# traveller59/spconv

Hardware: AMD Instinct MI355X
Metric: active-voxels/sec fwd+bwd, 3x3x3 SubMConv3d C=64, ~100k voxels/scene (higher is better)
Workload: dtype f16; 1 GPU; SubMConv3d 3x3x3 C=64->64 f16, 100000 uniform voxels/scene in 1600x1280x40 (BASELINE configs[1]), 8 distinct scenes per GPU visited round-robin, rulebook reused via indice_key; voxels_per_gpu=100000, launch=hipgraph, steps_per_replay=8, scenes_rotated=8, mask_sort=False, prewarm_steps=0, parallelism=dp1, ranks_seen=1, tree=unknown

## Files before the change

include/spconv_amd.h:

```cpp
#ifndef SPCONV_AMD_H_
#define SPCONV_AMD_H_

#include <stddef.h>
#include <stdint.h>

#ifdef __cplusplus
extern "C" {
#endif

#define SPX_MAX_NDIM 4
#define SPX_UNION_MAX_OPERANDS 8

typedef void *spx_stream_t;

enum spx_dtype { SPX_F32 = 0, SPX_F16 = 1, SPX_BF16 = 2, SPX_I8 = 3, SPX_F64 = 4 };

enum spx_act { SPX_ACT_NONE = 0, SPX_ACT_RELU = 1, SPX_ACT_SIGMOID = 2, SPX_ACT_LEAKY_RELU = 3 };
#define SPX_OUT_CACHED 0x100
#define SPX_TILE_ORDER 0x200

const char *spx_last_error(void);

int spx_version(void);

int spx_set_option(const char *name_h, int value);

long long spx_launch_count(const char *family_h);

int spx_pad_rows(const void *src, void *dst, long long rows, int src_row_bytes, int dst_row_bytes,
                 spx_stream_t stream);

int spx_conv_out_shape(int ndim, const int *in_shape, const int *ksize, const int *stride,
                       const int *padding, const int *dilation, const int *out_padding,
                       int transposed, int *out_shape);


size_t spx_subm_rulebook_ws_bytes(int n, int kv);

int spx_subm_rulebook(const int32_t *indices, int n, int ndim, int batch_size,
                      const int *spatial_shape, const int *ksize, const int *dilation,
                      int32_t *pair_fwd, int32_t *pair_bwd, uint32_t *mask,
                      int32_t *pair_native, int32_t *num_per_loc,
                      void *ws, size_t ws_bytes, spx_stream_t stream);

size_t spx_conv_rulebook_ws_bytes(int n_in, int ndim, const int *ksize, const int *stride,
                                  const int *dilation, int transposed);

int spx_conv_rulebook_count(const int32_t *indices, int n_in, int ndim, int batch_size,
                            const int *in_shape, const int *out_shape, const int *ksize,
                            const int *stride, const int *padding, const int *dilation,
                            int transposed, void *ws, size_t ws_bytes, int *n_out_h,
                            spx_stream_t stream);

int spx_conv_rulebook_fill(const int32_t *indices, int n_in, int ndim, int batch_size,
                           const int *in_shape, const int *out_shape, const int *ksize,
                           const int *stride, const int *padding, const int *dilation,
                           int transposed, int n_out, int32_t *out_indices,
                           int32_t *pair_fwd, int32_t *pair_bwd, uint32_t *mask_fwd,
                           uint32_t *mask_bwd, int32_t *pair_native, int32_t *num_per_loc,
                           void *ws, size_t ws_bytes, spx_stream_t stream);

int spx_conv_rulebook_static(const int32_t *indices, int n_in, int ndim, int batch_size,
                             const int *in_shape, const int *out_shape, const int *ksize,
                             const int *stride, const int *padding, const int *dilation,
                             int transposed, int n_out_cap, int32_t *out_indices,
                             int32_t *pair_fwd, int32_t *pair_bwd, uint32_t *mask_fwd,
                             uint32_t *mask_bwd, int32_t *pair_native, int32_t *num_per_loc,
                             int32_t *n_out_dev, void *ws, size_t ws_bytes, spx_stream_t stream);

size_t spx_rankmap_bytes(int ndim, int batch_size, const int *shape);
int spx_conv_sorted_ok(int ndim, int batch_size, const int *in_shape, const int *out_shape, const int *ksize,
                       const int *stride, const int *padding, const int *dilation, int transposed);
size_t spx_conv_rulebook_sorted_ws_bytes(int n_in, int ndim, int batch_size, const int *out_shape,
                                         const int *ksize);
int spx_conv_rulebook_count_sorted(const int32_t *indices, int n_in, int ndim, int batch_size,
                                   const int *in_shape, const int *out_shape, const int *ksize,
                                   const int *stride, const int *padding, const int *dilation,
                                   void *rankmap, size_t rankmap_bytes, void *ws, size_t ws_bytes,
                                   int *n_out_h, spx_stream_t stream);
int spx_conv_rulebook_fill_sorted(const int32_t *indices, int n_in, int ndim, int batch_size,
                                  const int *in_shape, const int *out_shape, const int *ksize,
                                  const int *stride, const int *padding, const int *dilation, int n_out,
                                  int32_t *out_indices, int32_t *pair_fwd, int32_t *pair_bwd,
                                  uint32_t *mask_fwd, uint32_t *mask_bwd, int32_t *pair_native,
                                  int32_t *num_per_loc, void *rankmap, size_t rankmap_bytes, void *ws,
                                  size_t ws_bytes, spx_stream_t stream);
int spx_conv_rulebook_static_sorted(const int32_t *indices, int n_in, int ndim, int batch_size,
                                    const int *in_shape, const int *out_shape, const int *ksize,
                                    const int *stride, const int *padding, const int *dilation,
                                    int n_out_cap, int32_t *out_indices, int32_t *pair_fwd,
                                    int32_t *pair_bwd, uint32_t *mask_fwd, uint32_t *mask_bwd,
                                    int32_t *pair_native, int32_t *num_per_loc, int32_t *n_out_dev,
                                    void *rankmap, size_t rankmap_bytes, void *ws, size_t ws_bytes,
                                    spx_stream_t stream);
int spx_rankmap_from_sorted(const int32_t *indices, int n, int ndim, int batch_size, const int *spatial_shape,
                            void *rankmap, size_t rankmap_bytes, int32_t *violation, spx_stream_t stream);
size_t spx_key_argsort_ws_bytes(int n);
int spx_key_argsort(const int32_t *indices, int n, int ndim, int batch_size, const int *spatial_shape, int32_t *order,
                    int32_t *indices_sorted, void *rankmap, size_t rankmap_bytes, int32_t *violation, const void *rows,
                    void *rows_sorted, int row_bytes, void *ws, size_t ws_bytes, spx_stream_t stream);
size_t spx_subm_rulebook_ranked_ws_bytes(int n, int kv);
int spx_subm_rulebook_ranked(const int32_t *indices, int n, int ndim, int batch_size,
                             const int *spatial_shape, const int *ksize, const int *dilation,
                             int32_t *pair_fwd, int32_t *pair_bwd, uint32_t *mask,
                             int32_t *pair_native, int32_t *num_per_loc, const void *rankmap,
                             size_t rankmap_bytes, void *ws, size_t ws_bytes, spx_stream_t stream);

size_t spx_mask_argsort_ws_bytes(int n);
int spx_mask_argsort(const uint32_t *mask, int n, int words, int32_t *argsort,
                     void *ws, size_t ws_bytes, spx_stream_t stream);
int spx_mask_argsort_kv(const uint32_t *mask, int n, int kv, int32_t *argsort, void *ws, size_t ws_bytes,
                        spx_stream_t stream);

int spx_native_to_table(const int32_t *pair_native, const int32_t *num_per_loc, int n_in,
                        int n_dst, int kv, int subm, int inverse, int32_t *table,
                        uint32_t *mask, spx_stream_t stream);
size_t spx_table_to_native_ws_bytes(int n, int kv);
int spx_table_to_native(const int32_t *table, int subm, int kv, int n, int32_t *pair_native,
                        int32_t *num_per_loc, void *ws, size_t ws_bytes, spx_stream_t stream);


size_t spx_igemm_acc_bytes(int n_dst, int cout, int kv);

int spx_igemm_fwd(const void *feat, const void *weight, void *out, const int32_t *pair,
                  const uint32_t *mask, const int32_t *argsort, int tile_order, int n_in, int n_out,
                  int C, int K, int kv, int dtype, int identity_k, const void *bias,
                  int act, float act_alpha, void *ws, size_t ws_bytes,
                  spx_stream_t stream);

int spx_igemm_fwd_stats_slots(int n_out);
int spx_igemm_fwd_stats(const void *feat, const void *weight, void *out, const int32_t *pair,
                        const uint32_t *mask, const int32_t *argsort, int tile_order, int n_in, int n_out, int C,
                        int K, int kv, int dtype, int identity_k, const void *bias, int act,
                        float act_alpha, void *ws, size_t ws_bytes, float *stats, int stats_slots,
                        const int32_t *n_live, int *slots_used_h, spx_stream_t stream);

int spx_igemm_fwd_int8(const void *feat, const void *weight, void *out, const int32_t *pair,
                       const uint32_t *mask, const int32_t *argsort, int n_in, int n_out, int C,
                       int K, int kv, int identity_k, const float *scale, const float *bias,
                       const void *add, float add_scale, int out_dtype, int act, float act_alpha,
                       spx_stream_t stream);

int spx_permute_tables(const int32_t *pair, const uint32_t *mask, const int32_t *order, int kv, int n,
                       int words, int32_t *pair_t, uint32_t *mask_t, spx_stream_t stream);

size_t spx_subm_layout_mcap(int n);
#define SPX_ROWS_LAYOUT 2
#define SPX_DENSE_HINT 0x100
#define SPX_ROWS_LAYOUT_ACT 0x400
#define SPX_SPARSE_HINT 0x800
#define SPX_LAYOUT_HEADER 64
size_t spx_subm_layout_bytes(int n, int kv);
size_t spx_subm_layout_ws_bytes(int n);
int spx_subm_layout(const int32_t *pair_fwd, const uint32_t *mask, int n, int kv, int32_t *layout,
                    void *ws, size_t ws_bytes, spx_stream_t stream);

size_t spx_igemm_dgrad_ws_bytes(int C, int K, int kv, int dtype);

int spx_igemm_dgrad(const void *dout, const void *weight, void *din, const int32_t *pair,
                    const uint32_t *mask, const int32_t *argsort, int tile_order, int n_out, int n_in,
                    int C, int K, int kv, int dtype, int subm, void *ws, size_t ws_bytes,
                    spx_stream_t stream);

size_t spx_igemm_wgrad_ws_bytes(int n_in, int C, int K, int kv);
size_t spx_igemm_wgrad_ws_bytes_dtype(int n_in, int C, int K, int kv, int dtype);

size_t spx_wgrad_plan_bytes(int n_in, int kv);
int spx_wgrad_plan(const int32_t *num_per_loc, int n_in, int kv, int subm, int32_t *plan,
                   spx_stream_t stream);

int spx_igemm_wgrad(const void *feat, const void *dout, void *dw, const int32_t *pair_native,
                    const int32_t *num_per_loc, const int32_t *plan, int n_in, int n_out, int C,
                    int K, int kv, int dtype, int subm, void *ws, size_t ws_bytes,
                    spx_stream_t stream);

size_t spx_igemm_bwd_rows_ws_bytes(int n_in, int C, int K, int kv);
int spx_igemm_bwd_rows(const void *feat, const void *dout, const void *weight_t, void *din, void *dw,
                       const int32_t *table, const uint32_t *mask, int n_in, int n_out, int C, int K,
                       int kv, int mirror, int dtype, void *ws, size_t ws_bytes, spx_stream_t stream);

int spx_igemm_bwd(const void *feat, const void *dout, const void *weight, void *din, void *dw,
                  const int32_t *pair, const uint32_t *mask, const int32_t *argsort, int tile_order,
                  const int32_t *pair_native, const int32_t *num_per_loc, const int32_t *plan,
                  int n_in, int n_out, int C, int K, int kv, int dtype, int subm, void *ws,
                  size_t ws_bytes, spx_stream_t stream);

#define SPX_STAGE2_JOB_BYTES 64
int spx_igemm_bwd_deferred(const void *feat, const void *dout, const void *weight, void *din, void *dw,
                           const int32_t *pair, const uint32_t *mask, const int32_t *argsort, int tile_order,
                           const int32_t *pair_native, const int32_t *num_per_loc, const int32_t *plan,
                           int n_in, int n_out, int C, int K, int kv, int dtype, int subm, void *ws,
                           size_t ws_bytes, spx_stream_t stream, void *stage2_job);
int spx_igemm_wgrad_deferred(const void *feat, const void *dout, void *dw, const int32_t *pair_native,
                             const int32_t *num_per_loc, const int32_t *plan, int n_in, int n_out, int C,
                             int K, int kv, int dtype, int subm, void *ws, size_t ws_bytes,
                             spx_stream_t stream, void *stage2_job);
int spx_wgrad_stage2_batch(const void *jobs, int njobs, spx_stream_t stream);
int spx_stage2_job_retarget(void *stage2_job, void *dw);

int spx_bias_act_inplace(void *out, const void *bias, int n, int K, int dtype, int act,
                         float act_alpha, spx_stream_t stream);


int spx_maxpool_fwd(const void *feat, void *out, const int32_t *pair_fwd, const uint32_t *mask,
                    int n_out, int C, int kv, int dtype, int init_zero, spx_stream_t stream);
int spx_maxpool_bwd(const void *feat, const void *out, const void *dout, void *din,
                    const int32_t *pair_bwd, const uint32_t *mask_bwd, int n_in, int C, int kv,
                    int dtype, spx_stream_t stream);
int spx_avgpool_fwd(const void *feat, void *out, int32_t *count_out, const int32_t *pair_fwd,
                    const uint32_t *mask, int n_out, int C, int kv, int dtype,
                    spx_stream_t stream);
int spx_avgpool_bwd(const void *dout, void *din, const int32_t *count, const int32_t *pair_bwd,
                    const uint32_t *mask_bwd, int n_in, int C, int kv, int dtype,
                    spx_stream_t stream);


size_t spx_point2voxel_ws_bytes(int n_points, int max_voxels);
int spx_point2voxel(const float *points, int n, int nfeat, int ndim, const float *vsize,
                    const float *coors_range, const int *grid_size, int max_voxels, int max_points,
                    int empty_mean, int clear_voxels, float *voxels, int32_t *indices,
                    int32_t *num_per_voxel, long long *pc_voxel_id, int *n_voxels_h, void *ws,
                    size_t ws_bytes, spx_stream_t stream);

size_t spx_point2voxel_static_ws_bytes(int n_cap, int max_voxels, int ndim, int batch_size, const int *grid_size,
                                       int key_order);
int spx_point2voxel_static(const float *points, const int32_t *point_batch, int n_cap, const int32_t *n_points_dev,
                           int nfeat, int ndim, const float *vsize, const float *coors_range, const int *grid_size,
                           int batch_size, int max_voxels, int max_points, int empty_mean, int key_order,
                           float *voxels, int32_t *indices, int32_t *num_per_voxel, long long *pc_voxel_id,
                           int32_t *n_voxels_dev, void *mean_out, int mean_dtype, void *rankmap, size_t rankmap_bytes,
                           void *ws, size_t ws_bytes, spx_stream_t stream);


size_t spx_hash_ws_bytes(int capacity);
int spx_hash_clear(void *table_keys, int capacity, int key_bytes, spx_stream_t stream);
int spx_hash_insert(void *table_keys, void *table_vals, int capacity, int key_bytes, int val_bytes,
                    const void *keys, const void *values, int n, spx_stream_t stream);
int spx_hash_query(void *table_keys, void *table_vals, int capacity, int key_bytes, int val_bytes,
                   const void *keys, void *values_out, unsigned char *is_empty, int n,
                   spx_stream_t stream);
int spx_hash_insert_exist(void *table_keys, void *table_vals, int capacity, int key_bytes,
                          int val_bytes, const void *keys, const void *values,
                          unsigned char *is_empty, int n, spx_stream_t stream);
int spx_hash_assign_arange(void *table_keys, void *table_vals, int capacity, int key_bytes,
                           int val_bytes, void *count_out, void *ws, size_t ws_bytes,
                           spx_stream_t stream);
int spx_hash_items(void *table_keys, void *table_vals, int capacity, int key_bytes, int val_bytes,
                   void *keys_out, void *vals_out, int max_out, void *count_out, void *ws,
                   size_t ws_bytes, spx_stream_t stream);

size_t spx_batchnorm_ws_bytes(int n, int C);
int spx_batchnorm_fwd(const void *x, void *y, int n, int C, int dtype, const void *weight,
                      const void *bias, void *running_mean, void *running_var,
                      long long *num_batches_tracked, int param_dtype, int training, float momentum,
                      float eps, int relu, float *save_mean, float *save_invstd, void *ws,
                      size_t ws_bytes, const int32_t *n_live, spx_stream_t stream);
int spx_batchnorm_fwd_stats(const void *x, void *y, int n, int C, int dtype, const void *weight,
                            const void *bias, void *running_mean, void *running_var,
                            long long *num_batches_tracked, int param_dtype, float momentum, float eps,
                            int relu, float *save_mean, float *save_invstd, const float *stats,
                            int stats_records, const int32_t *n_live, spx_stream_t stream);
int spx_batchnorm_bwd(const void *x, const void *dy, void *dx, int n, int C, int dtype,
                      const void *weight, const void *bias, int param_dtype, const float *mean,
                      const float *invstd, int use_batch_stats, int relu, void *dweight, void *dbias,
                      void *ws, size_t ws_bytes, const int32_t *n_live, spx_stream_t stream);

int spx_batchnorm_local_stats(const void *x, int n, int C, int dtype, const float *stats_in,
                              int stats_in_records, float *record_out, void *ws, size_t ws_bytes,
                              const int32_t *n_live, spx_stream_t stream);
int spx_batchnorm_bwd_sums(const void *x, const void *dy, int n, int C, int dtype, const void *weight,
                           const void *bias, int param_dtype, const float *mean, const float *invstd,
                           int relu, float *sums, void *dweight, void *dbias, void *ws, size_t ws_bytes,
                           const int32_t *n_live, spx_stream_t stream);
int spx_batchnorm_bwd_apply(const void *x, const void *dy, void *dx, int n, int C, int dtype,
                            const void *weight, const void *bias, int param_dtype, const float *mean,
                            const float *invstd, int relu, const float *sums, const float *total_rows,
                            const int32_t *n_live, spx_stream_t stream);

size_t spx_dense_ws_bytes(int ndim, int batch, const int *spatial_h);
int spx_dense_map(const int32_t *indices, int n, const int32_t *n_live, int ndim, int batch,
                  const int *spatial_h, int32_t *map, spx_stream_t stream);
int spx_to_dense(const void *rows, int n, long long row_stride, const int32_t *map, void *out, int C,
                 int elem_bytes, int channels_first, long long fill_bits, int ndim, int batch,
                 const int *spatial_h, spx_stream_t stream);
int spx_dense_gather(const void *dense, const int32_t *map, void *rows, int n, int C, int elem_bytes,
                     int channels_first, int ndim, int batch, const int *spatial_h,
                     spx_stream_t stream);
size_t spx_from_dense_ws_bytes(int ndim, int batch, const int *spatial_h);
int spx_from_dense_count(const void *dense, int C, int elem_bytes, int is_float, int ndim, int batch,
                         const int *spatial_h, void *ws, size_t ws_bytes, int *n_active_h,
                         spx_stream_t stream);
int spx_from_dense_fill(const void *dense, int C, int elem_bytes, int ndim, int batch,
                        const int *spatial_h, const void *ws, size_t ws_bytes, int32_t *indices,
                        void *rows, int32_t *map, spx_stream_t stream);

size_t spx_union_ws_bytes(int ndim, int batch, const int *spatial_h, int T, long long n_total);
int spx_union_count(const int32_t *const *indices_h, const int *n_h, const int32_t *const *n_live_h, int T,
                    int ndim, int batch, const int *spatial_h, void *rankmap, size_t rankmap_bytes, void *ws,
                    size_t ws_bytes, int *result_h, spx_stream_t stream);
int spx_union_fill(const int32_t *const *indices_h, const int *n_h, const int32_t *const *n_live_h, int T,
                   int ndim, int batch, const int *spatial_h, int n_out, int base, int32_t *out_indices,
// ... 16 lines not shown
```

spconv_amd/csrc/common.cpp:

```cpp
#include "common.h"

#include <string.h>

#include <mutex>
#include <string>

namespace spx {
namespace {
thread_local std::string g_error;
}

void set_error(const char *fmt, ...) {
  char buf[1024];
  va_list ap;
  va_start(ap, fmt);
  vsnprintf(buf, sizeof(buf), fmt, ap);
  va_end(ap);
  g_error = buf;
}

namespace {
struct Option {
  char name[48];
  int value;
// ... 27 lines not shown
    v = v * 10 + (*t - '0');
  }
  return v;
}

int instance_slot(const char *key) {
  char buf[96];
  if (strlen(key) >= sizeof(buf)) return -1;
  strcpy(buf, key);
  const char *tok[8];
  int n = 0;
  for (char *c = buf, *start = buf;; ++c) {
    if (*c == '/' || *c == 0) {
      if (n == 8) return -1;
      const bool end = *c == 0;
      *c = 0;
      tok[n++] = start;
      start = c + 1;
      if (end) break;
    }
  }
  const char *fam = tok[0];
  auto is = [&](const char *name, int ntok) { return strcmp(fam, name) == 0 && n == ntok; };
  auto cout_ok = [](int c) { return inst::cout_slot(c) >= 0; };
  if (is("igemm_v4", 7)) {
    const int cout = parse_int(tok[1]), mb = parse_int(tok[2]), dt = parse_dt(tok[3]);
    const int bt = strcmp(tok[4], "bt") == 0 ? 1 : (strcmp(tok[4], "fwd") == 0 ? 0 : -1);
    const int nks = parse_int(tok[5]), pk = parse_int(tok[6]);
    if (!cout_ok(cout) || (mb != 1 && mb != 2) || dt < 0 || bt < 0 || (nks != 1 && nks != 2) || inst::pk_slot(pk) < 0)
      return -1;
    return inst::v4(cout, mb, dt, bt == 1, nks, pk);
  }
  if (is("igemm_v4w", 6)) {
    const int nt = parse_int(tok[1]), dt = parse_dt(tok[2]);
    const int bt = strcmp(tok[3], "bt") == 0 ? 1 : (strcmp(tok[3], "fwd") == 0 ? 0 : -1);
    const int nks = parse_int(tok[4]), pk = parse_int(tok[5]);
    if (nt != 128 || bt < 0 || !inst::v4w_exists(dt, bt == 1, nks, pk)) return -1;
    return inst::v4w(dt, bt == 1, nks, pk);
  }
  if (is("igemm_bwd", 6)) {
    const int cout = parse_int(tok[1]), mb = parse_int(tok[2]), dt = parse_dt(tok[3]);
    const int nks = parse_int(tok[4]), pk = parse_int(tok[5]);
    if (!cout_ok(cout) || (mb != 1 && mb != 2) || dt < 0 || (nks != 1 && nks != 2) || inst::pk_slot(pk) < 0) return -1;
    return inst::bwd(cout, mb, dt, nks, pk);
  }
  if (is("igemm_ws", 2)) return parse_dt(tok[1]) < 0 ? -1 : inst::ws(parse_dt(tok[1]));
  if (is("igemm_bwd_rows", 5)) {
    const int c = parse_int(tok[1]), k = parse_int(tok[2]), dt = parse_dt(tok[3]), w8 = parse_int(tok[4]);
    if ((c != 16 && c != 32) || (k != 16 && k != 32) || dt < 0 || (w8 != 0 && w8 != 1)) return -1;
    return inst::bwd_rows(c, k, dt, w8 == 1);
  }
  if (is("wgrad_tr", 3)) {
    const int dt = parse_dt(tok[1]), sl = parse_int(tok[2]);
    return dt < 0 || inst::sl_slot(sl) < 0 ? -1 : inst::wgrad_tr(dt, sl);
  }
  if (is("wgrad_f32", 1)) return inst::kWgradF32;
  if (is("wgrad_mfma", 2)) return parse_dt(tok[1]) < 0 ? -1 : inst::wgrad_mfma(parse_dt(tok[1]));
  if (is("wgrad_generic", 2)) return parse_dt(tok[1]) < 0 ? -1 : inst::wgrad_generic(parse_dt(tok[1]));
  if (is("generic", 2)) return parse_dt(tok[1]) < 0 ? -1 : inst::generic(parse_dt(tok[1]));
  if (is("gen1", 3)) {
    const int cout = parse_int(tok[1]), dt = parse_dt(tok[2]);
    return !cout_ok(cout) || dt < 0 ? -1 : inst::gen1(cout, dt);
  }
  return -1;
}

std::atomic<long long> *f64_counter(const char *key) {
  if (strcmp(key, "igemm_f64/fwd") == 0) return &g_f64_launches[kF64Fwd];
  if (strcmp(key, "igemm_f64/dgrad") == 0) return &g_f64_launches[kF64Dgrad];
  if (strcmp(key, "wgrad_f64") == 0) return &g_f64_launches[kF64Wgrad];
  if (strcmp(key, "pool/f64") == 0) return &g_f64_launches[kF64Pool];
  return nullptr;
}

std::atomic<long long> *dense_counter(const char *key) {
  static const char *names[kDenseCount] = {"dense/map", "dense/scatter_cl", "dense/scatter_cf", "dense/gather_cl",
                                           "dense/gather_cf", "dense/compact"};
  for (int i = 0; i < kDenseCount; ++i)
    if (strcmp(key, names[i]) == 0) return &g_dense_launches[i];
  return nullptr;
}

std::atomic<long long> *union_counter(const char *key) {
  static const char *names[kUnionCount] = {"union/mark", "union/prefix", "union/claim", "union/fill", "union/add_fwd",
                                           "union/add_bwd"};
  for (int i = 0; i < kUnionCount; ++i)
    if (strcmp(key, names[i]) == 0) return &g_union_launches[i];
  return nullptr;
}

std::atomic<long long> *rulebook_counter(const char *key) {
  static const char *names[kRbCount] = {"subm_probe3", "subm_probe4", "subm_probe5", "subm_mask_pass", "subm_lists",
                                        "native_lists_v1", "conv3/1", "conv3/2", "conv3/4", "conv3/8", "conv_generic",
                                        "conv_lists_v1", "conv_shrunk", "conv_retry", "conv3_shares/1", "conv3_shares/2",
                                        "conv3_shares/4", "conv3_shares/8"};
  if (strncmp(key, "rulebook/", 9) != 0) return nullptr;
  for (int i = 0; i < kRbCount; ++i)
    if (strcmp(key + 9, names[i]) == 0) return &g_rulebook_launches[i];
  return nullptr;
}

std::atomic<long long> *pool_counter(const char *key) {
  static const char *ops[kPoolOps] = {"max_fwd", "max_bwd", "avg_fwd", "avg_bwd"};
  static const char *dts[kPoolDts] = {"f16", "bf16", "f32", "f64", "i8"};
  if (strncmp(key, "pool/", 5) != 0) return nullptr;
  key += 5;
  for (int op = 0; op < kPoolOps; ++op) {
    const size_t n = strlen(ops[op]);
    if (strncmp(key, ops[op], n) != 0 || key[n] != '/') continue;
    const char *rest = key + n + 1;
    for (int dt = 0; dt < kPoolDts; ++dt) {
      const size_t m = strlen(dts[dt]);
      if (strncmp(rest, dts[dt], m) != 0 || rest[m] != '/') continue;
      const char *piece = rest + m + 1;
      if (strcmp(piece, "v") == 0) return &g_pool_launches[pool_slot(op, dt, false)];
      if (strcmp(piece, "s") == 0) return &g_pool_launches[pool_slot(op, dt, true)];
    }
  }
  return nullptr;
}
}

int option_int(const char *name, int dflt) {
  {
    std::lock_guard<std::mutex> lock(g_option_mutex);
    for (int i = 0; i < g_noptions; ++i)
      if (strcmp(g_options[i].name, name) == 0) return g_options[i].value;
  }
  return env_int(name, dflt);
}
}

extern "C" {

int spx_set_option(const char *name_h, int value) {
  SPX_CHECK(name_h && strlen(name_h) < sizeof(spx::Option::name), "bad option name");
  std::lock_guard<std::mutex> lock(spx::g_option_mutex);
  for (int i = 0; i < spx::g_noptions; ++i)
    if (strcmp(spx::g_options[i].name, name_h) == 0) {
      spx::g_options[i].value = value;
      return 0;
    }
  SPX_CHECK(spx::g_noptions < 32, "too many options");
  strcpy(spx::g_options[spx::g_noptions].name, name_h);
  spx::g_options[spx::g_noptions++].value = value;
  return 0;
}

const char *spx_last_error(void) { return spx::g_error.c_str(); }

long long spx_launch_count(const char *family_h) {
  static const char *names[spx::kFamCount] = {"igemm_v4", "igemm_ws", "igemm_bwd", "igemm_bwd_rows", "igemm_i8_stream",
                                              "generic", "wgrad_stage2", "wgrad_stage2_batch", "igemm_f64",
                                              "igemm_v4w"};
  if (!family_h) return -1;
  for (int i = 0; i < spx::kFamCount; ++i)
    if (strcmp(names[i], family_h) == 0) return spx::g_launches[i].load(std::memory_order_relaxed);
  if (std::atomic<long long> *c = spx::f64_counter(family_h)) return c->load(std::memory_order_relaxed);
  if (std::atomic<long long> *c = spx::dense_counter(family_h)) return c->load(std::memory_order_relaxed);
  if (std::atomic<long long> *c = spx::union_counter(family_h)) return c->load(std::memory_order_relaxed);
  if (std::atomic<long long> *c = spx::pool_counter(family_h)) return c->load(std::memory_order_relaxed);
  if (std::atomic<long long> *c = spx::rulebook_counter(family_h)) return c->load(std::memory_order_relaxed);
  const int slot = spx::instance_slot(family_h);
  return slot < 0 ? -1 : spx::g_inst_launches[slot].load(std::memory_order_relaxed);
}

int spx_version(void) { return 1000; }

int spx_conv_out_shape(int ndim, const int *in_shape, const int *ksize, const int *stride,
                       const int *padding, const int *dilation, const int *out_padding,
                       int transposed, int *out_shape) {
  SPX_CHECK(ndim >= 1 && ndim <= SPX_MAX_NDIM, "ndim must be in [1,4], got %d", ndim);
  for (int i = 0; i < ndim; ++i) {
    SPX_CHECK(stride[i] > 0, "stride must be positive");
    if (transposed) {
      SPX_CHECK(ksize[i] != -1, "deconv don't support kernel_size < 0");
      out_shape[i] = (in_shape[i] - 1) * stride[i] - 2 * padding[i] + ksize[i] +
                     (out_padding ? out_padding[i] : 0);
    } else if (ksize[i] == -1) {
      out_shape[i] = 1;
    } else {
      const int num = in_shape[i] + 2 * padding[i] - dilation[i] * (ksize[i] - 1) - 1;
      int q = num / stride[i];
      if (num % stride[i] != 0 && num < 0) --q;
      out_shape[i] = q + 1;
    }
  }
  return 0;
}

}
```

spconv_amd/csrc/common.h:

```cpp
#pragma once
#include <hip/hip_runtime.h>
#include <stdint.h>
#include <stdio.h>
#include <stdarg.h>
#include <stdlib.h>

#include <atomic>

#include "../../include/spconv_amd.h"

namespace spx {

constexpr int kWave = 64;
constexpr int kMaxNdim = SPX_MAX_NDIM;

void set_error(const char *fmt, ...);

inline int env_int(const char *name, int dflt) {
  const char *v = getenv(name);
  return v ? atoi(v) : dflt;
}

int option_int(const char *name, int dflt);

inline size_t align_up(size_t v, size_t a) { return (v + a - 1) / a * a; }
inline int div_up(int a, int b) { return (a + b - 1) / b; }

struct Carver {
  char *base;
  size_t off = 0;
  explicit Carver(void *p) : base(static_cast<char *>(p)) {}
  template <typename T> T *take(size_t count) {
    T *r = reinterpret_cast<T *>(base + off);
    off += align_up(count * sizeof(T), 256);
    return r;
  }
};

#define SPX_CHECK(cond, ...)                 \
  do {                                       \
    if (!(cond)) {                           \
      ::spx::set_error(__VA_ARGS__);         \
      return -1;                             \
    }                                        \
  } while (0)

#define SPX_HIP(expr)                                                         \
  do {                                                                        \
    hipError_t e_ = (expr);                                                   \
    if (e_ != hipSuccess) {                                                   \
      ::spx::set_error("%s failed: %s (%s:%d)", #expr, hipGetErrorString(e_), \
                       __FILE__, __LINE__);                                   \
      return -2;                                                              \
    }                                                                         \
  } while (0)

#define SPX_LAUNCH_CHECK() SPX_HIP(hipGetLastError())

inline hipError_t ensure_dynamic_lds(const void *fn, int bytes, std::atomic<uint64_t> &done) {
  int dev = 0;
  hipError_t e = hipGetDevice(&dev);
  if (e != hipSuccess) return e;
  const uint64_t bit = 1ull << (dev & 63);
  if (done.load(std::memory_order_acquire) & bit) return hipSuccess;
  e = hipFuncSetAttribute(fn, hipFuncAttributeMaxDynamicSharedMemorySize, bytes);
  if (e == hipSuccess) done.fetch_or(bit, std::memory_order_release);
  return e;
}

struct Geom {
  int ndim;
  int batch;
  int in_dims[4];
  int out_dims[4];
  int ksize[4], stride[4], padding[4], dilation[4];
  int kv;
};

inline Geom make_geom(int ndim, int batch, const int *in_dims, const int *out_dims,
                      const int *ksize, const int *stride, const int *padding,
                      const int *dilation) {
  Geom g;
  g.ndim = ndim;
  g.batch = batch;
  const int lead = 4 - ndim;
  g.kv = 1;
  for (int i = 0; i < 4; ++i) {
    const bool pad = i < lead;
    const int j = i - lead;
    g.in_dims[i] = pad ? 1 : in_dims[j];
    g.out_dims[i] = pad ? 1 : out_dims[j];
    g.ksize[i] = pad ? 1 : ksize[j];
    g.stride[i] = pad ? 1 : (stride ? stride[j] : 1);
    g.padding[i] = pad ? 0 : (padding ? padding[j] : 0);
    g.dilation[i] = pad ? 1 : (dilation ? dilation[j] : 1);
    g.kv *= g.ksize[i];
  }
  return g;
}

}

namespace spx {
enum LaunchFamily { kFamV4 = 0, kFamWs, kFamBwdFused, kFamBwdRows, kFamI8Stream, kFamGeneric, kFamStage2, kFamStage2Batch,
                    kFamF64, kFamV4w, kFamCount };
extern std::atomic<long long> g_launches[kFamCount];
inline void count_launch(LaunchFamily f) { g_launches[f].fetch_add(1, std::memory_order_relaxed); }

namespace inst {
constexpr int cout_slot(int c) { return c == 16 ? 0 : c == 32 ? 1 : c == 64 ? 2 : c == 128 ? 3 : c == 256 ? 4 : -1; }
constexpr int pk_slot(int pk) {
  return pk == 1 ? 0 : pk == 2 ? 1 : pk == 4 ? 2 : pk == 8 ? 3 : pk == 16 ? 4 : pk == 32 ? 5 : -1;
}
constexpr int sl_slot(int sl) { return sl == 2 ? 0 : sl == 4 ? 1 : sl == 8 ? 2 : -1; }
constexpr int kCouts = 5, kDts = 4, kPks = 6;
constexpr int kV4 = 0;
constexpr int kBwd = kV4 + kCouts * 2 * kDts * 2 * 2 * kPks;
constexpr int kWs = kBwd + kCouts * 2 * kDts * 2 * kPks;
constexpr int kBwdRows = kWs + kDts;
constexpr int kWgradTr = kBwdRows + 2 * 2 * kDts * 2;
constexpr int kWgradF32 = kWgradTr + kDts * 3;
constexpr int kWgradMfma = kWgradF32 + 1;
constexpr int kWgradGeneric = kWgradMfma + kDts;
constexpr int kGeneric = kWgradGeneric + kDts;
constexpr int kGen1 = kGeneric + kDts;
constexpr int kV4w = kGen1 + kCouts * kDts;
constexpr int kWidePks = 3;
constexpr int kCount = kV4w + kDts * 2 * 2 * kWidePks;

constexpr int v4(int cout, int mb, int dt, bool bt, int nks, int pk) {
  return kV4 + ((((cout_slot(cout) * 2 + (mb - 1)) * kDts + dt) * 2 + (bt ? 1 : 0)) * 2 + (nks - 1)) * kPks + pk_slot(pk);
}
constexpr int bwd(int cout, int mb, int dt, int nks, int pk) {
  return kBwd + (((cout_slot(cout) * 2 + (mb - 1)) * kDts + dt) * 2 + (nks - 1)) * kPks + pk_slot(pk);
}
constexpr int ws(int dt) { return kWs + dt; }
constexpr int bwd_rows(int c, int k, int dt, bool w8) {
  return kBwdRows + (((c == 32 ? 1 : 0) * 2 + (k == 32 ? 1 : 0)) * kDts + dt) * 2 + (w8 ? 1 : 0);
}
constexpr int wgrad_tr(int dt, int sl) { return kWgradTr + dt * 3 + sl_slot(sl); }
constexpr int wgrad_mfma(int dt) { return kWgradMfma + dt; }
constexpr int wgrad_generic(int dt) { return kWgradGeneric + dt; }
constexpr int generic(int dt) { return kGeneric + dt; }
constexpr int gen1(int cout, int dt) { return kGen1 + cout_slot(cout) * kDts + dt; }
constexpr bool v4w_exists(int dt, bool bt, int nks, int pk) {
  return dt >= 0 && dt < kDts && (nks == 1 || nks == 2) && (pk == 1 || ((pk == 2 || pk == 4) && nks == 1 && dt <= 1)) &&
         !(dt == 2 && bt);
}
constexpr int v4w(int dt, bool bt, int nks, int pk) {
  return kV4w + ((dt * 2 + (bt ? 1 : 0)) * 2 + (nks - 1)) * kWidePks + pk_slot(pk);
}
}

extern std::atomic<long long> g_inst_launches[inst::kCount];
template <int I>
inline void count_inst() {
  static_assert(I >= 0 && I < inst::kCount, "instance counter slot");
  g_inst_launches[I].fetch_add(1, std::memory_order_relaxed);
}

enum F64Inst { kF64Fwd = 0, kF64Dgrad, kF64Wgrad, kF64Pool, kF64Count };
extern std::atomic<long long> g_f64_launches[kF64Count];
inline void count_f64(F64Inst i) { g_f64_launches[i].fetch_add(1, std::memory_order_relaxed); }

enum DenseInst { kDenseMap = 0, kDenseScatterCl, kDenseScatterCf, kDenseGatherCl, kDenseGatherCf, kDenseCompact, kDenseCount };
extern std::atomic<long long> g_dense_launches[kDenseCount];
inline void count_dense(DenseInst i) { g_dense_launches[i].fetch_add(1, std::memory_order_relaxed); }

enum UnionInst { kUnionMark = 0, kUnionPrefix, kUnionClaim, kUnionFill, kUnionAddFwd, kUnionAddBwd, kUnionCount };
extern std::atomic<long long> g_union_launches[kUnionCount];
inline void count_union(UnionInst i) { g_union_launches[i].fetch_add(1, std::memory_order_relaxed); }

enum PoolDt { kPoolF16 = 0, kPoolBf16, kPoolF32, kPoolF64, kPoolI8, kPoolDts };
constexpr int kPoolOps = 4, kPoolCount = kPoolOps * kPoolDts * 2;
extern std::atomic<long long> g_pool_launches[kPoolCount];
constexpr int pool_slot(int op, int dt, bool scalar) { return (op * kPoolDts + dt) * 2 + (scalar ? 1 : 0); }
inline void count_pool(int op, int dt, bool scalar) {
  g_pool_launches[pool_slot(op, dt, scalar)].fetch_add(1, std::memory_order_relaxed);
}

enum RulebookPass { kRbSubmProbe3 = 0, kRbSubmProbe4, kRbSubmProbe5, kRbSubmMaskPass, kRbSubmLists, kRbNativeListsV1,
                    kRbConv3_1, kRbConv3_2, kRbConv3_4, kRbConv3_8, kRbConvGeneric, kRbConvListsV1, kRbConvShrunk,
                    kRbConvRetry, kRbShares1, kRbShares2, kRbShares4, kRbShares8, kRbCount };
extern std::atomic<long long> g_rulebook_launches[kRbCount];
inline void count_rulebook(RulebookPass p) { g_rulebook_launches[p].fetch_add(1, std::memory_order_relaxed); }
}

namespace spx {
size_t radix_argsort_ws_bytes(int n);
int radix_argsort(const uint32_t *keys, int n, int nbits, int32_t *order_out, void *ws, hipStream_t s);

}
```

spconv_amd/csrc/igemm.hip:

```cpp
#include <cstring>
#include "igemm_bwd.h"

namespace spx {
namespace {

template <typename T>
__global__ void __launch_bounds__(kThreads)
gather_gemm_generic_kernel(GemmParams p) {
  const long long gid = static_cast<long long>(blockIdx.x) * kThreads + threadIdx.x;
  const long long total = static_cast<long long>(p.n_dst) * p.COUT;
  if (gid >= total) return;
  const int d = static_cast<int>(gid / p.COUT), n = static_cast<int>(gid % p.COUT);
  const T *A = static_cast<const T *>(p.A);
  const T *B = static_cast<const T *>(p.B);
  const int words = (p.kv + 31) / 32;
  float acc = 0.f;
  for (int k = 0; k < p.kv; ++k) {
    if (p.mask && !((p.mask[static_cast<size_t>(d) * words + (k >> 5)] >> (k & 31)) & 1u)) continue;
    const int idx = (k == p.identity_k) ? d : p.pair[static_cast<size_t>(k) * p.n_dst + d];
    if (idx < 0) continue;
    const int kb = p.b_reverse ? p.kv - 1 - k : k;
    const T *a = A + static_cast<size_t>(idx) * p.CIN;
    const T *b = B + static_cast<size_t>(kb) * p.strideK + static_cast<size_t>(n) * p.strideN;
    for (int c = 0; c < p.CIN; ++c) acc = fmaf(load_f(a + c), load_f(b + c * p.strideD), acc);
// ... 10 lines not shown
  const long long gid = static_cast<long long>(blockIdx.x) * kThreads + threadIdx.x;
  if (gid >= total) return;
  float v = load_f(out + gid);
  if (bias) v += load_f(bias + gid % K);
  store_f(out + gid, apply_act(v, act, alpha));
}

bool mfma_ok(int dtype, int cin, int cout, int kv) {
  if (dtype != SPX_F16 && dtype != SPX_BF16 && dtype != SPX_F32) return false;
  if (cin % (dtype == SPX_F32 ? 4 : 8) != 0) return false;
  if (kv > 128) return false;
  if (cout == 16 || cout == 32 || cout == 64 || cout == 128 || cout == 256) return true;
  return wide_cout(cout) && option_int("SPX_WIDE", 1) != 0;
}

int run_gather_gemm_single(const GemmParams &p, int dtype, hipStream_t s);

int run_gather_gemm(const GemmParams &p, int dtype, hipStream_t s) {
  if (p.n_dst == 0) return 0;
  if (p.kv <= 32 || !mfma_ok(dtype, p.CIN, p.COUT, p.kv) || !p.pair) return run_gather_gemm_single(p, dtype, s);
  const int words = div_up(p.kv, 32);
  const bool fits = fits32(p.n_dst, words, 4) &&
                    fits32(p.n_dst, p.COUT, 4) &&
                    v4_ok(p, dtype == SPX_F32 ? 4 : 2, dtype == SPX_F32 ? 4 : 2) && !p.argsort;
  if (!fits || !p.acc) {
    GemmParams q = p;
    q.acc = nullptr;
    return run_gather_gemm_single(q, dtype, s);
  }
  for (int g = 0; g < words; ++g) {
    GemmParams q = p;
    q.kbase = 32 * g;
    q.pair = p.pair + static_cast<size_t>(32 * g) * p.n_dst;
    q.mask = p.mask ? p.mask + g : nullptr;
    q.mask_words = p.mask ? words : 1;
    q.identity_k = (p.identity_k >= 32 * g && p.identity_k < 32 * g + 32) ? p.identity_k - 32 * g : -1;
    q.acc_mode = (g > 0 ? 1 : 0) | (g < words - 1 ? 2 : 0);
    if (int rc = run_gather_gemm_single(q, dtype, s)) return rc;
  }
  return 0;
}

int run_gather_gemm_single(const GemmParams &p, int dtype, hipStream_t s) {
  if (p.n_dst == 0) return 0;
  const bool grouped = p.acc_mode != 0;
  if (dtype == SPX_F32 && mfma_ok(dtype, p.CIN, p.COUT, p.kv) && v4_ok(p, 4, 4) &&
      (p.kv <= 32 || grouped))
    return dispatch_gather_gemm_f32(p, s);
  if (dtype != SPX_F32 && mfma_ok(dtype, p.CIN, p.COUT, p.kv) && (p.kv <= 32 || grouped) &&
      (!wide_cout(p.COUT) || v4_ok(p)))
    return dtype == SPX_BF16 ? dispatch_gather_gemm_bf16(p, s) : dispatch_gather_gemm<false>(p, s);
  if (p.cls) {
    GemmParams q = p;
    drop_rows_layout(q);
    return run_gather_gemm_single(q, dtype, s);
  }
  if (p.tile_order) {
    set_error("tables in tile order are supported by the MFMA kernels only (channel counts / kernel volume)");
    return -1;
  }
  const long long total = static_cast<long long>(p.n_dst) * p.COUT;
  const dim3 grid(static_cast<unsigned>((total + kThreads - 1) / kThreads));
  count_launch(kFamGeneric);
  if (int rc = with_elem_type(dtype, [&](auto t, auto slot) {
        count_inst<inst::generic(decltype(slot)::value)>();
        hipLaunchKernelGGL(gather_gemm_generic_kernel<decltype(t)>, grid, dim3(kThreads), 0, s, p);
      }))
    return rc;
  SPX_LAUNCH_CHECK();
  return 0;
}

GemmParams dgrad_params(const void *dout, const void *weight, void *din, const int32_t *pair,
                        const uint32_t *mask, const int32_t *argsort, int n_out, int n_in, int C,
                        int K, int kv, int subm) {
  GemmParams p{};
  p.A = dout;
  p.B = weight;
  p.out = din;
  p.pair = pair;
  p.mask = mask;
  p.argsort = argsort;
  p.bias = nullptr;
  p.strideK = C;
  p.strideN = 1;
  p.strideD = static_cast<long long>(kv) * C;
  p.n_src = n_out;
  p.n_dst = n_in;
  p.CIN = K;
  p.COUT = C;
  p.kv = kv;
  p.identity_k = subm ? kv / 2 : -1;
  p.b_reverse = subm ? 1 : 0;
  p.act = SPX_ACT_NONE;
  p.act_alpha = 0.f;
  return p;
}

GemmParams fwd_params(const void *feat, const void *weight, void *out, const int32_t *pair, const uint32_t *mask,
                      const int32_t *argsort, const void *bias, int n_in, int n_out, int C, int K, int kv,
                      int identity_k) {
  GemmParams p{};
  p.A = feat;
  p.B = weight;
  p.out = out;
  p.pair = pair;
  p.mask = mask;
  p.argsort = argsort;
  p.bias = bias;
  p.strideK = C;
  p.strideN = static_cast<long long>(kv) * C;
  p.strideD = 1;
  p.n_src = n_in;
  p.n_dst = n_out;
  p.CIN = C;
  p.COUT = K;
  p.kv = kv;
  p.identity_k = identity_k;
  p.b_reverse = 0;
  return p;
}

__global__ void __launch_bounds__(kThreads)
pad_rows_kernel(const uint16_t *__restrict__ src, uint16_t *__restrict__ dst, long long total, int sw, int dw) {
  const long long i = static_cast<long long>(blockIdx.x) * kThreads + threadIdx.x;
  if (i >= total) return;
  const long long r = i / dw;
  const int c = static_cast<int>(i - r * dw);
  dst[i] = c < sw ? src[r * sw + c] : static_cast<uint16_t>(0);
}
}
}

using namespace spx;

extern "C" {

size_t spx_igemm_acc_bytes(int n_dst, int cout, int kv) {
  return kv > 32 ? align_up(static_cast<size_t>(n_dst > 0 ? n_dst : 1) * cout * sizeof(float), 256) : 0;
}

static int igemm_fwd_impl(const void *feat, const void *weight, void *out, const int32_t *pair,
                          const uint32_t *mask, const int32_t *argsort, int tile_order, int n_in, int n_out, int C,
                          int K, int kv, int dtype, int identity_k, const void *bias, int act,
                          float act_alpha, void *ws, size_t ws_bytes, spx_stream_t stream, float *stats,
                          const int32_t *n_live, int *slots_used_h) {
  if (slots_used_h) *slots_used_h = 0;
  SPX_CHECK(C > 0 && K > 0 && kv > 0 && n_in >= 0 && n_out >= 0, "bad sizes");
  if (n_out == 0) return 0;
  SPX_CHECK((feat || n_in == 0) && weight && out, "null tensor pointer");
  SPX_CHECK(pair || kv == 1, "pair table required");
  GemmParams p = fwd_params(feat, weight, out, pair, mask, argsort, bias, n_in, n_out, C, K, kv, identity_k);
  p.dense_hint = (tile_order & SPX_DENSE_HINT) ? 1 : 0;
  apply_rows_layout(p, tile_order & ~SPX_DENSE_HINT);
  p.act = act & 0xff;
  if (act & SPX_OUT_CACHED) p.dbg = 0x400;
  p.act_alpha = act_alpha;
  if (dtype == SPX_F64) return run_gather_gemm_f64(p, false, static_cast<hipStream_t>(stream));
  if (ws && ws_bytes >= spx_igemm_acc_bytes(n_out, K, kv) && kv > 32) p.acc = static_cast<float *>(ws);
  if (stats && kv <= 32 && !bias && p.act == SPX_ACT_NONE) {
    p.stats = stats;
    p.n_live = n_live;
    p.grid_out = slots_used_h;
  }
  return run_gather_gemm(p, dtype, static_cast<hipStream_t>(stream));
}

int spx_igemm_fwd(const void *feat, const void *weight, void *out, const int32_t *pair,
                  const uint32_t *mask, const int32_t *argsort, int tile_order, int n_in, int n_out, int C,
                  int K, int kv, int dtype, int identity_k, const void *bias, int act,
                  float act_alpha, void *ws, size_t ws_bytes, spx_stream_t stream) {
  return igemm_fwd_impl(feat, weight, out, pair, mask, argsort, tile_order, n_in, n_out, C, K, kv, dtype, identity_k,
                        bias, act, act_alpha, ws, ws_bytes, stream, nullptr, nullptr, nullptr);
}

int spx_igemm_fwd_stats_slots(int n_out) {
  return n_out <= 0 ? 0 : div_up(n_out, 64) + div_up(n_out, 256) + 8;
}

int spx_igemm_fwd_stats(const void *feat, const void *weight, void *out, const int32_t *pair,
                        const uint32_t *mask, const int32_t *argsort, int tile_order, int n_in, int n_out, int C,
                        int K, int kv, int dtype, int identity_k, const void *bias, int act,
                        float act_alpha, void *ws, size_t ws_bytes, float *stats, int stats_slots,
                        const int32_t *n_live, int *slots_used_h, spx_stream_t stream) {
  SPX_CHECK(slots_used_h, "slots_used_h is required");
  SPX_CHECK(!stats || stats_slots >= spx_igemm_fwd_stats_slots(n_out), "statistics buffer too small: %d slots < %d",
            stats_slots, spx_igemm_fwd_stats_slots(n_out));
  return igemm_fwd_impl(feat, weight, out, pair, mask, argsort, tile_order, n_in, n_out, C, K, kv, dtype, identity_k,
                        bias, act, act_alpha, ws, ws_bytes, stream, stats, n_live, slots_used_h);
}

int spx_igemm_fwd_int8(const void *feat, const void *weight, void *out, const int32_t *pair,
                       const uint32_t *mask, const int32_t *argsort, int n_in, int n_out, int C,
                       int K, int kv, int identity_k, const float *scale, const float *bias,
                       const void *add, float add_scale, int out_dtype, int act, float act_alpha,
                       spx_stream_t stream) {
  SPX_CHECK(C > 0 && K > 0 && kv > 0 && n_in >= 0 && n_out >= 0, "bad sizes");
  if (n_out == 0) return 0;
  SPX_CHECK((feat || n_in == 0) && weight && out, "null tensor pointer");
  SPX_CHECK(pair || kv == 1, "pair table required");
  SPX_CHECK(C % 16 == 0, "int8 needs in_channels %% 16 == 0, got %d", C);
  SPX_CHECK(K == 16 || K == 32 || K == 64 || K == 128 || K == 256 || wide_cout(K),
            "int8 supports out_channels 16/32/64/128/256 or a multiple of 128 beyond, got %d", K);
  SPX_CHECK(kv <= 32, "int8 supports kernel volumes up to 32, got %d", kv);
  SPX_CHECK(out_dtype == SPX_I8 || out_dtype == SPX_F16 || out_dtype == SPX_BF16 || out_dtype == SPX_F32,
            "bad output dtype %d", out_dtype);
  GemmParams p = fwd_params(feat, weight, out, pair, mask, argsort, bias, n_in, n_out, C, K, kv, identity_k);
  apply_rows_layout(p, (act & SPX_ROWS_LAYOUT_ACT) ? SPX_ROWS_LAYOUT : ((act & SPX_TILE_ORDER) ? 1 : 0));
  const bool hinted = p.cls && (act & SPX_SPARSE_HINT);
  if (hinted) p.app_rows = ((act >> 16) & 0xffff) * 64;
  p.act = act & 0xff;
  p.act_alpha = act_alpha;
  p.scale = scale;
  p.add = add;
  p.add_scale = add_scale;
  p.out_dtype = out_dtype;
  const int oes = out_dtype == SPX_I8 ? 1 : (out_dtype == SPX_F32 ? 4 : 2);
  SPX_CHECK(v4_ok(p, 1, oes), "tensor too large for 32-bit buffer offsets");
  hipStream_t s = static_cast<hipStream_t>(stream);
  return launch_gather_gemm_int8(p, p.tile_order || hinted, s);
}

size_t spx_igemm_dgrad_ws_bytes(int C, int K, int kv, int dtype) {
  (void)C; (void)K; (void)kv; (void)dtype;
  return 0;
}

int spx_igemm_dgrad(const void *dout, const void *weight, void *din, const int32_t *pair,
                    const uint32_t *mask, const int32_t *argsort, int tile_order, int n_out, int n_in, int C,
                    int K, int kv, int dtype, int subm, void *ws, size_t ws_bytes,
                    spx_stream_t stream) {
  if (n_in == 0) return 0;
  SPX_CHECK((dout || n_out == 0) && weight && din, "null tensor pointer");
  SPX_CHECK(pair || kv == 1, "pair table required");
  GemmParams p = dgrad_params(dout, weight, din, pair, mask, argsort, n_out, n_in, C, K, kv, subm);
  p.dense_hint = (tile_order & SPX_DENSE_HINT) ? 1 : 0;
  apply_rows_layout(p, tile_order & ~SPX_DENSE_HINT);
  if (dtype == SPX_F64) return run_gather_gemm_f64(p, true, static_cast<hipStream_t>(stream));
  if (ws && ws_bytes >= spx_igemm_acc_bytes(n_in, C, kv) && kv > 32) p.acc = static_cast<float *>(ws);
  return run_gather_gemm(p, dtype, static_cast<hipStream_t>(stream));
}

static int igemm_bwd_impl(const void *feat, const void *dout, const void *weight, void *din, void *dw,
                          const int32_t *pair, const uint32_t *mask, const int32_t *argsort, int tile_order,
                          const int32_t *pair_native, const int32_t *num_per_loc, const int32_t *plan,
                          int n_in, int n_out, int C, int K, int kv, int dtype, int subm, void *ws,
                          size_t ws_bytes, spx_stream_t stream, void *stage2_job) {
  hipStream_t s = static_cast<hipStream_t>(stream);
  if (n_in == 0 || n_out == 0) {
    SPX_CHECK(dw && C > 0 && K > 0 && kv > 0, "null tensor pointer");
    SPX_HIP(hipMemsetAsync(dw, 0, static_cast<size_t>(K) * kv * C * elem_bytes(dtype), s));
    if (n_in > 0) {
      SPX_CHECK(din, "null tensor pointer");
      SPX_HIP(hipMemsetAsync(din, 0, static_cast<size_t>(n_in) * C * elem_bytes(dtype), s));
    }
    return 0;
  }
  SPX_CHECK(feat && dout && weight && din && dw && ws, "null tensor pointer");
  SPX_CHECK(pair_native && num_per_loc, "Native pair lists and counts are required");
  SPX_CHECK(pair || kv == 1, "pair table required");
  if (dtype == SPX_F64) {
    SPX_CHECK(!stage2_job, "float64 backward has no deferred second stage (use spx_igemm_bwd)");
    SPX_CHECK(ws_bytes >= wgrad_f64_ws_bytes(n_in, C, K, kv),
              "workspace too small for the float64 weight gradient (spx_igemm_wgrad_ws_bytes_dtype)");
    if (spx_igemm_dgrad(dout, weight, din, pair, mask, argsort, tile_order, n_out, n_in, C, K, kv, dtype, subm,
                        nullptr, 0, stream))
      return -2;
    return wgrad_f64(feat, dout, dw, pair_native, num_per_loc, n_in, C, K, kv, subm, ws, ws_bytes, s);
  }
  SPX_CHECK(ws_bytes >= spx_igemm_wgrad_ws_bytes(n_in, C, K, kv), "workspace too small");
  GemmParams p = dgrad_params(dout, weight, din, pair, mask, argsort, n_out, n_in, C, K, kv, subm);
  p.dense_hint = (tile_order & SPX_DENSE_HINT) ? 1 : 0;
  apply_rows_layout(p, tile_order & ~SPX_DENSE_HINT);
  const int es = dtype == SPX_F32 ? 4 : 2, lanes = 16 / es;
  const bool fusable = (dtype == SPX_F16 || dtype == SPX_BF16 || dtype == SPX_F32) && C % lanes == 0 &&
                       K % lanes == 0 && mfma_ok(dtype, p.CIN, p.COUT, kv) && kv <= 32 && p.COUT <= 128 &&
                       v4_ok(p, es, es) && wgrad_rows_fit(n_in, n_out, C, K, es) && wgrad_lists_fit(n_in, kv) &&
                       n_in > 0 && n_out > 0;
  if (!fusable) {
    if (spx_igemm_dgrad(dout, weight, din, pair, mask, argsort, tile_order, n_out, n_in, C, K, kv, dtype, subm,
                        nullptr, 0, stream))
      return -2;
    return igemm_wgrad_impl(feat, dout, dw, pair_native, num_per_loc, plan, n_in, n_out, C, K, kv, dtype,
                            subm, ws, ws_bytes, stream, stage2_job);
  }
  plan = wgrad_plan_or_build(plan, num_per_loc, n_in, kv, subm, ws, ws_bytes, stream);
  if (!plan) return -2;
  const Wgrad2Params q = wgrad2_params(feat, dout, ws, pair_native, num_per_loc, plan, n_in, n_out, C, K, kv, subm);
  const int ntile = q.tiles_c * q.tiles_k;
  const int rc = dtype == SPX_F32 ? dispatch_bwd_f32(p, q, q.G * ntile, s)
                                  : (dtype == SPX_BF16 ? dispatch_bwd_bf16(p, q, q.G * ntile, s)
                                                       : dispatch_bwd<0>(p, q, q.G * ntile, s));
  if (rc) return rc;
  return launch_reduce2(q, dw, dtype, ntile, s, stage2_job);
}

int spx_igemm_bwd(const void *feat, const void *dout, const void *weight, void *din, void *dw,
                  const int32_t *pair, const uint32_t *mask, const int32_t *argsort, int tile_order,
                  const int32_t *pair_native, const int32_t *num_per_loc, const int32_t *plan,
                  int n_in, int n_out, int C, int K, int kv, int dtype, int subm, void *ws,
                  size_t ws_bytes, spx_stream_t stream) {
  return igemm_bwd_impl(feat, dout, weight, din, dw, pair, mask, argsort, tile_order, pair_native, num_per_loc, plan, n_in,
                        n_out, C, K, kv, dtype, subm, ws, ws_bytes, stream, nullptr);
}

int spx_igemm_bwd_deferred(const void *feat, const void *dout, const void *weight, void *din, void *dw,
                           const int32_t *pair, const uint32_t *mask, const int32_t *argsort, int tile_order,
                           const int32_t *pair_native, const int32_t *num_per_loc, const int32_t *plan,
                           int n_in, int n_out, int C, int K, int kv, int dtype, int subm, void *ws,
                           size_t ws_bytes, spx_stream_t stream, void *stage2_job) {
  SPX_CHECK(stage2_job, "stage2_job is required");
  SPX_CHECK(dtype != SPX_F64, "float64 backward has no deferred second stage (use spx_igemm_bwd)");
  memset(stage2_job, 0, SPX_STAGE2_JOB_BYTES);
  return igemm_bwd_impl(feat, dout, weight, din, dw, pair, mask, argsort, tile_order, pair_native, num_per_loc, plan, n_in,
                        n_out, C, K, kv, dtype, subm, ws, ws_bytes, stream, stage2_job);
}

int spx_bias_act_inplace(void *out, const void *bias, int n, int K, int dtype, int act,
                         float act_alpha, spx_stream_t stream) {
  hipStream_t s = static_cast<hipStream_t>(stream);
  const long long total = static_cast<long long>(n) * K;
  if (total == 0) return 0;
  if (dtype == SPX_F64) return bias_act_f64(out, bias, n, K, act, act_alpha, s);
  const dim3 grid(static_cast<unsigned>((total + kThreads - 1) / kThreads));
  if (int rc = with_elem_type(dtype, [&](auto t, auto) {
        using T = decltype(t);
        hipLaunchKernelGGL(bias_act_kernel<T>, grid, dim3(kThreads), 0, s, static_cast<T *>(out),
                           static_cast<const T *>(bias), total, K, act, act_alpha);
      }))
    return rc;
  SPX_LAUNCH_CHECK();
  return 0;
}

int spx_pad_rows(const void *src, void *dst, long long rows, int src_row_bytes, int dst_row_bytes,
                 spx_stream_t stream) {
  SPX_CHECK(src_row_bytes > 0 && dst_row_bytes >= src_row_bytes && src_row_bytes % 2 == 0 && dst_row_bytes % 2 == 0,
            "row sizes must be even, destination rows at least as long as source rows");
  if (rows <= 0) return 0;
  SPX_CHECK(src && dst, "null tensor pointer");
  const long long total = rows * (dst_row_bytes / 2);
  hipLaunchKernelGGL(pad_rows_kernel, dim3(static_cast<unsigned>((total + kThreads - 1) / kThreads)), dim3(kThreads), 0,
                     static_cast<hipStream_t>(stream), static_cast<const uint16_t *>(src), static_cast<uint16_t *>(dst),
                     total, src_row_bytes / 2, dst_row_bytes / 2);
  SPX_LAUNCH_CHECK();
  return 0;
}

#ifdef SPX_TIMELINE
int spx_debug_timeline(unsigned long long *dst_h) {
  SPX_HIP(hipDeviceSynchronize());
  SPX_HIP(hipMemcpyFromSymbol(dst_h, HIP_SYMBOL(g_timeline), sizeof(unsigned long long) * kTlMaxWg * kTlSlots));
  return 0;
}
#endif

}
```

spconv_amd/csrc/igemm_bwd.h:

```cpp
#pragma once
#include "igemm_v4.h"

namespace spx {
namespace {

constexpr int kWT = 64;

constexpr int kW2MaxG = 1024;
constexpr int kW2J = 128;
constexpr int kW2Rec = 8;
constexpr int kXcds = 8;


__host__ __device__ inline int plan2_wg(int w) { return 8 + kW2Rec * w; }
__host__ __device__ inline int plan2_kf(int G) { return 8 + kW2Rec * G; }
__host__ __device__ inline int plan2_seg(int G, int kv) { return 8 + kW2Rec * G + kv + 1; }
__host__ __device__ inline int plan2_red(int G, int kv) {
  return (plan2_seg(G, kv) + 3 * (G + kv) + 3) & ~3;
}

__device__ __forceinline__ int wtr_x(int row) { return ((row >> 1) & 1) | (((row >> 3) & 1) << 1); }
__device__ __forceinline__ int wtr_slot(int row, int sl) {
  return row * 128 + ((((sl >> 1) ^ wtr_x(row)) << 5) | ((sl & 1) << 4));
}

typedef short s16x4 __attribute__((ext_vector_type(4)));

__device__ __forceinline__ uint4 wtr_frag(const char *stage, int row0, int lrow, int gran) {
  const int r = row0 + (lrow >> 2);
  const char *a0 = stage + r * 128 + ((gran ^ wtr_x(r)) << 5) + ((lrow & 3) << 3);
  const int r1 = r + 4;
  const char *a1 = stage + r1 * 128 + ((gran ^ wtr_x(r1)) << 5) + ((lrow & 3) << 3);
  typedef __attribute__((address_space(3))) s16x4 lds_s16x4;
  const s16x4 lo = __builtin_amdgcn_ds_read_tr16_b64_v4i16(
      (lds_s16x4 *)(__attribute__((address_space(3))) char *)a0);
  const s16x4 hi = __builtin_amdgcn_ds_read_tr16_b64_v4i16(
      (lds_s16x4 *)(__attribute__((address_space(3))) char *)a1);
  const uint2 l2 = __builtin_bit_cast(uint2, lo), h2 = __builtin_bit_cast(uint2, hi);
  return make_uint4(l2.x, l2.y, h2.x, h2.y);
}

template <bool BF16, int STAGES, int SL = 8>
__device__ __forceinline__ void wgrad_tr_body(const Wgrad2Params &p, int block) {
  extern __shared__ __attribute__((aligned(16))) char smem[];
  constexpr int TILE_B = kW2J * 128;
  constexpr int RQ = SL / 2;
  constexpr int RSTEP = 2 * kW2J / SL;
  constexpr int RA = RQ < 2 ? 2 : RQ;
  const int tid = threadIdx.x, lane = tid & 63, wave = tid >> 6;
  const int lrow = lane & 15, lgrp = lane >> 4;
  const int wk = wave >> 1, wc = wave & 1;
  const int ntile = p.tiles_k * p.tiles_c;
  const int wb = block / ntile, tile = block - wb * ntile;
  const int w = p.xcd_order ? p.plan2[plan2_wg(wb) + 5] : wb;
  const int kk0 = (tile / p.tiles_c) * kWT, c0 = (tile % p.tiles_c) * kWT;
  const int32_t *__restrict__ rec = p.plan2 + plan2_wg(w);
  const int32_t *__restrict__ segs = p.plan2 + plan2_seg(p.G, p.kv);
  const int seg_lo = rec[0], nseg = rec[1];
  const bool live = kk0 + wk * 32 < p.K && c0 + wc * 32 < p.C;
  SPX_STAMP(0);

  const uint32_t rowD = static_cast<uint32_t>(p.K) * 2u, rowF = static_cast<uint32_t>(p.C) * 2u;
  const __amdgpu_buffer_rsrc_t rD = make_rsrc(p.dout, static_cast<uint32_t>(p.n_out) * rowD);
  const __amdgpu_buffer_rsrc_t rF = make_rsrc(p.feat, static_cast<uint32_t>(p.n_in) * rowF);
  const uint32_t list_bytes = (static_cast<uint32_t>(p.kv) + 1u) * static_cast<uint32_t>(p.n_in) * 4u;
  const uint32_t out_list = static_cast<uint32_t>(p.kv) * static_cast<uint32_t>(p.n_in) * 4u;

  const int slot = tid & (SL - 1), r0 = tid / SL;
  const uint32_t dcol = kk0 + slot * 8 < p.K ? static_cast<uint32_t>(kk0 + slot * 8) * 2u : kOob;
  const uint32_t fcol = c0 + slot * 8 < p.C ? static_cast<uint32_t>(c0 + slot * 8) * 2u : kOob;
  constexpr int W_ROWS = 64 / SL;
  const int wl_idx = lane & 31;
  const int wl_row = (64 * wave) / SL + (wl_idx % W_ROWS) + RSTEP * (wl_idx / W_ROWS);
  const uint32_t wl_list = (lane >> 5) ? out_list : 0u;
  const int rsub = lane / SL;
  int lds_w[RA];
#pragma unroll
  for (int q = 0; q < RQ; ++q) lds_w[q] = wtr_slot(r0 + RSTEP * q, slot);
  if constexpr (SL < 8) {
    for (int o = tid * 16; o < STAGES * 2 * TILE_B; o += kThreads * 16)
      *reinterpret_cast<u32x4 *>(smem + o) = u32x4{0u, 0u, 0u, 0u};
    __syncthreads();
  }

  for (int si = 0; si < nseg; ++si) {
    int k, begin, end;
    if (si == 0) {
      k = rec[2];
      begin = rec[3];
      end = rec[4];
    } else {
      k = segs[3 * (seg_lo + si)];
      begin = segs[3 * (seg_lo + si) + 1];
      end = segs[3 * (seg_lo + si) + 2];
    }
    const bool identity = p.subm && k == p.kv / 2;
    const __amdgpu_buffer_rsrc_t rW = make_rsrc(p.native + static_cast<size_t>(k) * p.n_in, list_bytes);

    f32x4 acc[2][2];
#pragma unroll
    for (int a = 0; a < 2; ++a)
#pragma unroll
      for (int b = 0; b < 2; ++b) acc[a][b] = f32x4{0.f, 0.f, 0.f, 0.f};

    uint32_t wd = 0;
    u32x4 dv[RA], fv[RA];
    auto load_words = [&](int base) __attribute__((always_inline)) {
      const int j = base + wl_row;
      if (identity) {
        wd = static_cast<uint32_t>(j);
      } else {
        const uint32_t vo = j < end ? static_cast<uint32_t>(j) * 4u + wl_list : kOob;
        wd = __builtin_amdgcn_raw_buffer_load_b32(rW, vo, 0, SPX_AUX_TABLE);
      }
    };
    auto load_rows = [&](int base) __attribute__((always_inline)) {
#pragma unroll
      for (int q = 0; q < RQ; ++q) {
        const uint32_t iq = static_cast<uint32_t>(
            __builtin_amdgcn_ds_bpermute((q * W_ROWS + rsub) * 4, static_cast<int>(wd)));
        const uint32_t oq = static_cast<uint32_t>(
            __builtin_amdgcn_ds_bpermute((32 + q * W_ROWS + rsub) * 4, static_cast<int>(wd)));
        const bool ok = base + r0 + RSTEP * q < end;
        dv[q] = __builtin_amdgcn_raw_buffer_load_b128(rD, ok ? (oq * rowD + dcol) | (dcol & kOob) : kOob, 0, 0);
        fv[q] = __builtin_amdgcn_raw_buffer_load_b128(rF, ok ? (iq * rowF + fcol) | (fcol & kOob) : kOob, 0, 0);
      }
    };
    load_words(begin);
    load_rows(begin);
    load_words(begin + kW2J);
    if (si == 0) SPX_STAMP(1);
    int stage = 0;
    for (int base = begin; base < end; base += kW2J, stage ^= (STAGES - 1)) {
      char *sD = smem + stage * (2 * TILE_B);
      char *sF = sD + TILE_B;
      if (STAGES == 1) __syncthreads();
#pragma unroll
      for (int q = 0; q < RQ; ++q) {
        *reinterpret_cast<u32x4 *>(sD + lds_w[q]) = dv[q];
        *reinterpret_cast<u32x4 *>(sF + lds_w[q]) = fv[q];
      }
      __syncthreads();
      load_rows(base + kW2J);
      load_words(base + 2 * kW2J);
      if (live)
#pragma unroll
      for (int ks = 0; ks < kW2J / 32; ++ks) {
        const int row0 = ks * 32 + lgrp * 8;
        uint4 fa[2], fb[2];
#pragma unroll
        for (int a = 0; a < 2; ++a) fa[a] = wtr_frag(sD, row0, lrow, wk * 2 + a);
#pragma unroll
        for (int b = 0; b < 2; ++b) fb[b] = wtr_frag(sF, row0, lrow, wc * 2 + b);
#pragma unroll
        for (int a = 0; a < 2; ++a)
#pragma unroll
          for (int b = 0; b < 2; ++b) acc[a][b] = mfma16<BF16>(fa[a], fb[b], acc[a][b]);
      }
    }
    if (si == nseg - 1) SPX_STAMP(4);
    float *dst = p.partial + (static_cast<size_t>(seg_lo + si) * ntile + tile) * (kWT * kWT);
#pragma unroll
    for (int a = 0; a < 2; ++a)
#pragma unroll
      for (int b = 0; b < 2; ++b)
#pragma unroll
        for (int e = 0; e < 4; ++e) {
          const int kk = wk * 32 + a * 16 + lgrp * 4 + e;
          const int c = wc * 32 + b * 16 + lrow;
          if (SPX_AUX_OUT) __builtin_nontemporal_store(acc[a][b][e], &dst[kk * kWT + c]);
          else dst[kk * kWT + c] = acc[a][b][e];
        }
    __syncthreads();
  }
  SPX_STAMP(6);
#ifdef SPX_TIMELINE
  asm volatile("s_waitcnt vmcnt(0)" ::: "memory");
  SPX_STAMP(7);
#endif
}

constexpr int kW3J = 64;
constexpr int kW3Stride = 80;

__device__ __forceinline__ void wgrad_f32_body(const Wgrad2Params &p, int block) {
  extern __shared__ __attribute__((aligned(16))) char smem[];
  float *sD = reinterpret_cast<float *>(smem);
  float *sF = sD + kW3J * kW3Stride;
  const int tid = threadIdx.x, lane = tid & 63, wave = tid >> 6;
  const int lrow = lane & 15, lgrp = lane >> 4;
  const int wk = wave >> 1, wc = wave & 1;
  const int ntile = p.tiles_k * p.tiles_c;
  const int w = block / ntile, tile = block - w * ntile;
  const int kk0 = (tile / p.tiles_c) * kWT, c0 = (tile % p.tiles_c) * kWT;
  const int32_t *__restrict__ rec = p.plan2 + plan2_wg(w);
  const int32_t *__restrict__ segs = p.plan2 + plan2_seg(p.G, p.kv);
  const int seg_lo = rec[0], nseg = rec[1];
  const uint32_t rowD = static_cast<uint32_t>(p.K) * 4u, rowF = static_cast<uint32_t>(p.C) * 4u;
  const __amdgpu_buffer_rsrc_t rD = make_rsrc(p.dout, static_cast<uint32_t>(p.n_out) * rowD);
  const __amdgpu_buffer_rsrc_t rF = make_rsrc(p.feat, static_cast<uint32_t>(p.n_in) * rowF);
  const uint32_t list_bytes = static_cast<uint32_t>(p.n_in) * 4u;
  const int slot = tid & 15, r0 = tid >> 4;
  const uint32_t dcol = kk0 + slot * 4 < p.K ? static_cast<uint32_t>(kk0 + slot * 4) * 4u : kOob;
  const uint32_t fcol = c0 + slot * 4 < p.C ? static_cast<uint32_t>(c0 + slot * 4) * 4u : kOob;

  for (int si = 0; si < nseg; ++si) {
    int k, begin, end;
    if (si == 0) {
      k = rec[2];
      begin = rec[3];
      end = rec[4];
    } else {
      k = segs[3 * (seg_lo + si)];
      begin = segs[3 * (seg_lo + si) + 1];
      end = segs[3 * (seg_lo + si) + 2];
    }
    const bool identity = p.subm && k == p.kv / 2;
    const __amdgpu_buffer_rsrc_t rIn =
        make_rsrc(p.native + static_cast<size_t>(k) * p.n_in, list_bytes);
    const __amdgpu_buffer_rsrc_t rOut =
        make_rsrc(p.native + static_cast<size_t>(p.kv + k) * p.n_in, list_bytes);
    f32x4 acc[2][2];
#pragma unroll
    for (int a = 0; a < 2; ++a)
#pragma unroll
      for (int b = 0; b < 2; ++b) acc[a][b] = f32x4{0.f, 0.f, 0.f, 0.f};
    u32x4 dv[4], fv[4];
    auto load_rows = [&](int base) __attribute__((always_inline)) {
#pragma unroll
      for (int q = 0; q < 4; ++q) {
        const int j = base + r0 + 16 * q;
        const bool ok = j < end;
        uint32_t ii = static_cast<uint32_t>(j), oi = static_cast<uint32_t>(j);
        if (!identity) {
          const uint32_t vo = ok ? static_cast<uint32_t>(j) * 4u : kOob;
          ii = __builtin_amdgcn_raw_buffer_load_b32(rIn, vo, 0, 0);
          oi = __builtin_amdgcn_raw_buffer_load_b32(rOut, vo, 0, 0);
        }
        dv[q] = __builtin_amdgcn_raw_buffer_load_b128(rD, ok ? (oi * rowD + dcol) | (dcol & kOob) : kOob, 0, 0);
        fv[q] = __builtin_amdgcn_raw_buffer_load_b128(rF, ok ? (ii * rowF + fcol) | (fcol & kOob) : kOob, 0, 0);
      }
    };
    load_rows(begin);
    for (int base = begin; base < end; base += kW3J) {
      __syncthreads();
#pragma unroll
      for (int q = 0; q < 4; ++q) {
        *reinterpret_cast<u32x4 *>(sD + (r0 + 16 * q) * kW3Stride + slot * 4) = dv[q];
        *reinterpret_cast<u32x4 *>(sF + (r0 + 16 * q) * kW3Stride + slot * 4) = fv[q];
      }
      __syncthreads();
      load_rows(base + kW3J);
#pragma unroll 4
      for (int ks = 0; ks < kW3J / 4; ++ks) {
        const int row = (ks * 4 + lgrp) * kW3Stride;
        float fa[2], fb[2];
#pragma unroll
        for (int a = 0; a < 2; ++a) fa[a] = sD[row + wk * 32 + a * 16 + lrow];
#pragma unroll
        for (int b = 0; b < 2; ++b) fb[b] = sF[row + wc * 32 + b * 16 + lrow];
#pragma unroll
        for (int a = 0; a < 2; ++a)
#pragma unroll
          for (int b = 0; b < 2; ++b)
            acc[a][b] = __builtin_amdgcn_mfma_f32_16x16x4f32(fa[a], fb[b], acc[a][b], 0, 0, 0);
      }
    }
    float *dst = p.partial + (static_cast<size_t>(seg_lo + si) * ntile + tile) * (kWT * kWT);
#pragma unroll
    for (int a = 0; a < 2; ++a)
#pragma unroll
      for (int b = 0; b < 2; ++b)
#pragma unroll
        for (int e = 0; e < 4; ++e) {
          const int kk = wk * 32 + a * 16 + lgrp * 4 + e;
          const int c = wc * 32 + b * 16 + lrow;
          if (SPX_AUX_OUT) __builtin_nontemporal_store(acc[a][b][e], &dst[kk * kWT + c]);
          else dst[kk * kWT + c] = acc[a][b][e];
        }
    __syncthreads();
  }
}

template <int COUT, int MB, int DT, int NKS = 2, int PK = 1>
__global__ void __launch_bounds__(kThreads, COUT <= 64 ? 4 : 2)
igemm_bwd_kernel(const void *argA, const void *argB, const uint32_t *arg_mask,
                 const int32_t *arg_argsort, const int32_t *arg_pair, int n_dst, int n_src, int CIN,
                 int kv, int identity_k, int b_reverse, GemmRest rest, int n_dgrad, Wgrad2Params wp) {
  const int nw = n_dgrad < 0 ? ~n_dgrad : 0;
  const int b = static_cast<int>(blockIdx.x);
  const bool is_dgrad = n_dgrad < 0 ? b >= nw : b < n_dgrad;
  if (is_dgrad) {
    GemmParams p;
    unpack_gemm_args(p, argA, argB, arg_mask, arg_argsort, arg_pair, n_dst, n_src, CIN, kv,
                     identity_k, b_reverse, rest);
    p.xcd_rot = (rest.dbg & 0x100) ? 0 : (nw & 7);
    p.app_budget = kAppBudget;
    igemm_v4_body<COUT, MB, DT, true, NKS, PK>(p, n_dgrad < 0 ? b - nw : b);
  } else {
    if constexpr (DT == 3) wgrad_f32_body(wp, n_dgrad < 0 ? b : b - n_dgrad);
    else wgrad_tr_body<DT == 1, 1>(wp, n_dgrad < 0 ? b : b - n_dgrad);
  }
}

template <int COUT, int MB, int DT = 0>
constexpr size_t bwd_smem_bytes() {
  const size_t a = v4_smem_bytes<COUT, MB>();
  const size_t b = DT == 3 ? 2 * static_cast<size_t>(kW3J) * kW3Stride * sizeof(float)
                           : 2 * static_cast<size_t>(kW2J) * 128;
  return a > b ? a : b;
}

template <int COUT, int MB, int DT>
int launch_bwd(const GemmParams &p, const Wgrad2Params &q, int n_wgrad_blocks, hipStream_t s) {
  const int napp = p.cls ? layout_app_tiles(p.n_dst, 64 * MB) : 0;
  const int n_dgrad = div_up(p.n_dst, 64 * MB) + napp;
  GemmRest rr = rest_of(p);
  rr.napp = p.cls ? napp : -1;
  constexpr int wgrad_first = 1;
  GemmParams pl = p;
  pl.lpt = p.tile_order && n_dgrad + n_wgrad_blocks > 1024;
  count_launch(kFamBwdFused);
#define SPX_LAUNCH_BWD(NKSV, PKV)                                                                                  \
  do {                                                                                                               \
    count_inst<inst::bwd(COUT, MB, DT, NKSV, PKV)>();                                                                \
    hipLaunchKernelGGL((igemm_bwd_kernel<COUT, MB, DT, NKSV, PKV>), dim3(n_dgrad + n_wgrad_blocks), dim3(kThreads),  \
                       (bwd_smem_bytes<COUT, MB, DT>()), s, p.A, p.B, p.mask, p.argsort, p.pair, p.n_dst,           \
                       p.n_src, p.CIN, p.kv, p.identity_k, v4_flags(pl), rr,                                        \
                       wgrad_first ? ~n_wgrad_blocks : n_dgrad, q);                                                 \
  } while (0)
  const int pk = v4_pack(p, DT, DT == 3 ? 4 : 2, true);
  if constexpr (DT == 0 || DT == 1) {
    if (pk == 32) SPX_LAUNCH_BWD(2, 32);
    else if (pk == 16) SPX_LAUNCH_BWD(2, 16);
    else if (pk == 8) SPX_LAUNCH_BWD(2, 8);
    else if (pk == 4) SPX_LAUNCH_BWD(1, 4);
    else if (pk == 2) SPX_LAUNCH_BWD(1, 2);
    else if (p.CIN * 2 <= 64) SPX_LAUNCH_BWD(1, 1);
    else SPX_LAUNCH_BWD(2, 1);
  } else {
    if (p.CIN * (DT == 3 ? 4 : 2) <= 64) SPX_LAUNCH_BWD(1, 1);
    else SPX_LAUNCH_BWD(2, 1);
  }
#undef SPX_LAUNCH_BWD
  SPX_LAUNCH_CHECK();
  return 0;
}

template <int DT>
int dispatch_bwd(const GemmParams &p, const Wgrad2Params &q, int nwb, hipStream_t s) {
  switch (p.COUT) {
    case 16: return launch_bwd<16, 2, DT>(p, q, nwb, s);
    case 32: return launch_bwd<32, 2, DT>(p, q, nwb, s);
    case 64: return launch_bwd<64, 2, DT>(p, q, nwb, s);
    case 128: return launch_bwd<128, 2, DT>(p, q, nwb, s);
  }
  return -1;
}

}
}
```

spconv_amd/csrc/igemm_defs.h:

```cpp
#pragma once
#include "common.h"

#include <stdlib.h>
#include <type_traits>
#include <utility>

#ifndef SPX_AUX_TABLE
#define SPX_AUX_TABLE 0
#endif
#ifndef SPX_WD
#define SPX_WD 2
#endif
#ifndef SPX_AUX_OUT
#define SPX_AUX_OUT 2
#endif

namespace spx {

struct GemmParams {
  const void *A;
  const void *B;
  void *out;
  const int32_t *pair;
  const uint32_t *mask;
  const int32_t *argsort;
  const void *bias;
  long long strideK, strideN, strideD;
  int n_src, n_dst, CIN, COUT, kv;
  int identity_k;
  int b_reverse;
  int tile_order;
  int kbase, mask_words;
  float *acc;
  int acc_mode;
  int act;
  float act_alpha;
  const float *scale;
  const void *add;
  float add_scale;
  int out_dtype;
  int dbg;
  int xcd_rot;
  int lpt;
  const int32_t *cls;
  const uint32_t *mask_rows;
  int app_rows;
  int app_budget;
  int dense_hint;
  float *stats;
  const int32_t *n_live;
  int *grid_out;
  int n0;
};

constexpr int kAppBudget = 64;
constexpr int kLayoutMinRows = 32768;
__host__ __device__ inline int layout_mcap(int n) { return ((n / 4 + 63) & ~63) + 256; }
__host__ __device__ inline int layout_app_tiles(int n, int tm) { return (n / 4 + tm - 1) / tm; }

inline void apply_rows_layout(GemmParams &p, int tile_order) {
  p.cls = nullptr;
  p.mask_rows = nullptr;
  p.app_rows = 0;
  p.app_budget = 0;
  if (tile_order == SPX_ROWS_LAYOUT && p.argsort && p.pair && p.mask) {
    const int32_t *blob = p.argsort;
    const size_t npad = (static_cast<size_t>(p.n_dst) + 63) & ~static_cast<size_t>(63);
    p.cls = blob;
    p.mask_rows = p.mask;
    p.mask = reinterpret_cast<const uint32_t *>(blob + SPX_LAYOUT_HEADER);
    p.argsort = blob + SPX_LAYOUT_HEADER + npad;
    p.tile_order = 0;
  } else {
    p.tile_order = (tile_order == 1 && p.argsort) ? 1 : 0;
    if (tile_order == SPX_ROWS_LAYOUT) p.argsort = nullptr;
  }
}

inline void drop_rows_layout(GemmParams &p) {
  if (!p.cls) return;
  p.mask = p.mask_rows;
  p.argsort = nullptr;
  p.tile_order = 0;
  p.cls = nullptr;
}

struct GemmRest {
  void *out;
  const void *bias;
  long long strideK, strideN, strideD;
  int COUT, act;
  float act_alpha;
  const float *scale;
  const void *add;
  float add_scale;
  int out_dtype;
  int dbg;
  float *acc;
  int acc_mode;
  int napp;
  float *stats;
  const int32_t *n_live;
};

__device__ __forceinline__ float row16_sum(float x) {
  x += __builtin_bit_cast(float, __builtin_amdgcn_update_dpp(0, __builtin_bit_cast(int, x), 0x128, 0xf, 0xf, false));
  x += __builtin_bit_cast(float, __builtin_amdgcn_update_dpp(0, __builtin_bit_cast(int, x), 0x124, 0xf, 0xf, false));
  x += __builtin_bit_cast(float, __builtin_amdgcn_update_dpp(0, __builtin_bit_cast(int, x), 0x122, 0xf, 0xf, false));
  x += __builtin_bit_cast(float, __builtin_amdgcn_update_dpp(0, __builtin_bit_cast(int, x), 0x121, 0xf, 0xf, false));
  return x;
}

template <int COUT>
__device__ __forceinline__ void bn_record_store(float *__restrict__ stats, int rec, int nrec, int c, float n, float m,
                                                float m2) {
  const size_t g = static_cast<size_t>(nrec);
  stats[static_cast<size_t>(c) * g + rec] = n;
  stats[(static_cast<size_t>(COUT) + c) * g + rec] = m;
  stats[(2 * static_cast<size_t>(COUT) + c) * g + rec] = m2;
}

template <int ROUND>
__device__ __forceinline__ float bn_rounded(float v) {
  if constexpr (ROUND == 1) v = static_cast<float>(static_cast<_Float16>(v));
  if constexpr (ROUND == 2) {
    uint32_t u = __builtin_bit_cast(uint32_t, v);
    u += 0x7fffu + ((u >> 16) & 1u);
    v = __builtin_bit_cast(float, u & 0xffff0000u);
  }
  return v;
}

template <int COUT, int CPL, int MB, int NWAVES, int ROUND, typename Acc>
__device__ __forceinline__ void wg_bn_stats(const Acc (&acc)[CPL / 4][MB], const int (&grow)[MB], int n_live,
                                            float *lds, float *__restrict__ stats, int rec, int nrec) {
  const int tid = threadIdx.x, lane = tid & 63, wave = tid >> 6, lrow = lane & 15, lgrp = lane >> 4;
  constexpr int W = 2 * COUT + 1;
  bool ok[MB];
  int rows = 0;
#pragma unroll
  for (int mb = 0; mb < MB; ++mb) {
    ok[mb] = grow[mb] >= 0 && grow[mb] < n_live;
    rows += ok[mb] ? 1 : 0;
  }
  const float cnt = row16_sum(static_cast<float>(rows));
  const float inv = cnt > 0.f ? 1.f / cnt : 0.f;
#pragma unroll
  for (int nb = 0; nb < CPL / 4; ++nb)
#pragma unroll
    for (int e = 0; e < 4; ++e) {
      float a = 0.f;
#pragma unroll
      for (int mb = 0; mb < MB; ++mb) a += ok[mb] ? bn_rounded<ROUND>(acc[nb][mb][e]) : 0.f;
      const float mean = row16_sum(a) * inv;
      float b = 0.f;
#pragma unroll
      for (int mb = 0; mb < MB; ++mb) {
        const float d = bn_rounded<ROUND>(acc[nb][mb][e]) - mean;
        b += ok[mb] ? d * d : 0.f;
      }
      b = row16_sum(b);
      if (lrow == 0) {
        lds[wave * W + lgrp * CPL + nb * 4 + e] = mean;
        lds[wave * W + COUT + lgrp * CPL + nb * 4 + e] = b;
      }
    }
  if (lane == 0) lds[wave * W + 2 * COUT] = cnt;
  __syncthreads();
  if (tid < COUT) {
    float n = 0.f, m = 0.f, m2 = 0.f;
#pragma unroll
    for (int w = 0; w < NWAVES; ++w) {
      const float nb = lds[w * W + 2 * COUT];
      if (nb > 0.f) {
        const float tot = n + nb, d = lds[w * W + tid] - m;
        m += d * (nb / tot);
        m2 += lds[w * W + COUT + tid] + d * d * (n * nb / tot);
        n = tot;
      }
    }
    bn_record_store<COUT>(stats, rec, nrec, tid, n, m, m2);
  }
}

template <int COUT>
__device__ __forceinline__ void wg_bn_stats_empty(float *__restrict__ stats, int rec, int nrec) {
  if (threadIdx.x < COUT) bn_record_store<COUT>(stats, rec, nrec, threadIdx.x, 0.f, 0.f, 0.f);
}

struct Wgrad2Params {
  const void *feat;
  const void *dout;
  float *partial;
  const int32_t *native;
  const int32_t *num;
  const int32_t *plan2;
  int n_in, n_out, C, K, kv, subm, tiles_c, tiles_k, G;
  int xcd_order;
};

// ... 265 lines not shown
```

spconv_amd/csrc/igemm_v4.h:

```cpp
#pragma once
#include "igemm_defs.h"

namespace spx {
namespace {

#ifdef SPX_TIMELINE
constexpr int kTlSlots = 8, kTlMaxWg = 8192;
__device__ unsigned long long g_timeline[kTlMaxWg * kTlSlots];
#define SPX_STAMP(i)                                                                     \
  do {                                                                                   \
    if (threadIdx.x == 0 && blockIdx.x < kTlMaxWg)                                       \
      g_timeline[blockIdx.x * kTlSlots + (i)] = __builtin_amdgcn_s_memtime();            \
  } while (0)
#else
#define SPX_STAMP(i) do {} while (0)
#endif




template <int COUT, int MB, int DT, bool BT, int NKS = 2, int PK = 1, bool WIDE = false>
__device__ __forceinline__ void igemm_v4_body(const GemmParams &p, int block);
__device__ __forceinline__ void unpack_gemm_args(GemmParams &p, const void *argA, const void *argB,
                                                 const uint32_t *arg_mask, const int32_t *arg_argsort,
                                                 const int32_t *arg_pair, int n_dst, int n_src, int CIN,
                                                 int kv, int identity_k, int b_reverse,
                                                 const GemmRest &rest);

template <int COUT, int MB, int DT, bool BT, int NKS = 2, int PK = 1>
__global__ void __launch_bounds__(kThreads)
igemm_v4_kernel(const void *argA, const void *argB, const uint32_t *arg_mask,
                const int32_t *arg_argsort, const int32_t *arg_pair, int n_dst, int n_src, int CIN,
                int kv, int identity_k, int b_reverse, GemmRest rest) {
  GemmParams p;
  unpack_gemm_args(p, argA, argB, arg_mask, arg_argsort, arg_pair, n_dst, n_src, CIN, kv, identity_k,
                   b_reverse, rest);
  igemm_v4_body<COUT, MB, DT, BT, NKS, PK>(p, blockIdx.x);
}

__device__ __forceinline__ void unpack_gemm_args(GemmParams &p, const void *argA, const void *argB,
                                                 const uint32_t *arg_mask, const int32_t *arg_argsort,
                                                 const int32_t *arg_pair, int n_dst, int n_src, int CIN,
                                                 int kv, int identity_k, int b_reverse,
                                                 const GemmRest &rest) {
  p.A = argA;
  p.B = argB;
  p.mask = arg_mask;
  p.argsort = arg_argsort;
  p.pair = arg_pair;
  p.n_dst = n_dst;
  p.n_src = n_src;
  p.CIN = CIN;
  p.kv = kv;
  p.identity_k = identity_k;
  p.b_reverse = b_reverse & 1;
  p.tile_order = (b_reverse >> 1) & 1;
  p.mask_words = ((b_reverse >> 2) & 3) + 1;
  p.kbase = (b_reverse >> 4) & 127;
  p.lpt = (b_reverse >> 11) & 1;
  p.acc = rest.acc;
  p.acc_mode = rest.acc_mode;
  p.out = rest.out;
  p.bias = rest.bias;
  p.strideK = rest.strideK;
  p.strideN = rest.strideN;
  p.strideD = rest.strideD;
  p.COUT = rest.COUT;
  p.act = rest.act;
  p.act_alpha = rest.act_alpha;
  p.scale = rest.scale;
  p.add = rest.add;
  p.add_scale = rest.add_scale;
  p.out_dtype = rest.out_dtype;
  p.dbg = rest.dbg;
  p.xcd_rot = 0;
  p.stats = rest.stats;
  p.n_live = rest.n_live;
  p.app_rows = rest.napp;
  p.app_budget = 0;
  p.cls = nullptr;
  if ((b_reverse >> 12) & 1) {
    const size_t npad = (static_cast<size_t>(n_dst) + 63) & ~static_cast<size_t>(63);
    p.cls = arg_argsort - npad - SPX_LAYOUT_HEADER;
  }
}

template <int COUT, int MB>
__device__ __forceinline__ void i8_epilogue(const GemmParams &p, i32x4 (&acc)[COUT / 16][MB], const int (&grow)[MB],
                                            int lgrp, const float *lds_sb, int ldo = COUT, int n0 = 0) {
  constexpr int NB = COUT / 16, CPL = NB * 4;
  const int oes = p.out_dtype == SPX_I8 ? 1 : (p.out_dtype == SPX_F32 ? 4 : 2);
  const __amdgpu_buffer_rsrc_t rO =
      make_rsrc(p.out, static_cast<uint32_t>(p.n_dst) * static_cast<uint32_t>(ldo * oes));
  const __amdgpu_buffer_rsrc_t rAdd =
      make_rsrc(p.add, p.add ? static_cast<uint32_t>(p.n_dst) * ldo : 0u);
  uint32_t rowoff[MB];
  uint32_t addw[MB][CPL / 4];
#pragma unroll
  for (int mb = 0; mb < MB; ++mb) {
    rowoff[mb] = grow[mb] < 0 ? kOob : static_cast<uint32_t>(grow[mb]) * ldo + n0 + lgrp * CPL;
    load_dwords<CPL / 4>(addw[mb], rAdd, rowoff[mb]);
  }
#pragma unroll
  for (int nb = 0; nb < NB; ++nb) {
    const float4 sc4 = *reinterpret_cast<const float4 *>(lds_sb + lgrp * CPL + nb * 4);
    const float4 bv4 = *reinterpret_cast<const float4 *>(lds_sb + COUT + lgrp * CPL + nb * 4);
    const float sc[4] = {sc4.x, sc4.y, sc4.z, sc4.w}, bv[4] = {bv4.x, bv4.y, bv4.z, bv4.w};
#pragma unroll
    for (int mb = 0; mb < MB; ++mb) {
      float v[4];
#pragma unroll
      for (int e = 0; e < 4; ++e) {
        float prod = static_cast<float>(acc[nb][mb][e]) * sc[e];
        asm volatile("" : "+v"(prod));
        v[e] = prod + bv[e];
      }
      if (p.add) {
#pragma unroll
        for (int e = 0; e < 4; ++e) {
          const int a8 = static_cast<int>(static_cast<int8_t>((addw[mb][nb] >> (e * 8)) & 0xff));
          float prod = static_cast<float>(a8) * p.add_scale;
          asm volatile("" : "+v"(prod));
          v[e] += prod;
        }
      }
      if (p.act == SPX_ACT_RELU) {
#pragma unroll
        for (int e = 0; e < 4; ++e) v[e] = v[e] > 0.f ? v[e] : 0.f;
      } else if (p.act != SPX_ACT_NONE) {
#pragma unroll
        for (int e = 0; e < 4; ++e) v[e] = apply_act(v[e], p.act, p.act_alpha);
      }
      if (p.out_dtype == SPX_I8) {
        int q[4];
#pragma unroll
        for (int e = 0; e < 4; ++e)
          q[e] = static_cast<int>(__builtin_amdgcn_fmed3f(__builtin_rintf(v[e]), -128.f, 127.f));
        typedef short s16x2 __attribute__((ext_vector_type(2)));
        const uint32_t p01 = __builtin_bit_cast(uint32_t, __builtin_amdgcn_cvt_pk_i16(q[0], q[1]));
        const uint32_t p23 = __builtin_bit_cast(uint32_t, __builtin_amdgcn_cvt_pk_i16(q[2], q[3]));
        const uint32_t word = __builtin_amdgcn_perm(p23, p01, 0x06040200u);
        addw[mb][nb] = word;
      } else if (p.out_dtype == SPX_F32) {
        uint32_t d[4];
#pragma unroll
        for (int e = 0; e < 4; ++e) d[e] = __builtin_bit_cast(uint32_t, v[e]);
        store_dwords<4, SPX_AUX_OUT>(d, rO, rowoff[mb] == kOob ? kOob : (rowoff[mb] + nb * 4) * 4u);
      } else {
        uint32_t d[2];
#pragma unroll
        for (int q = 0; q < 2; ++q)
          d[q] = p.out_dtype == SPX_BF16 ? pack2<true>(v[2 * q], v[2 * q + 1])
                                         : pack2<false>(v[2 * q], v[2 * q + 1]);
        store_dwords<2, SPX_AUX_OUT>(d, rO, rowoff[mb] == kOob ? kOob : (rowoff[mb] + nb * 4) * 2u);
      }
    }
  }
  if (p.out_dtype == SPX_I8) {
#pragma unroll
    for (int mb = 0; mb < MB; ++mb) store_dwords<CPL / 4, SPX_AUX_OUT>(addw[mb], rO, rowoff[mb]);
  }

}

template <int COUT, int MB, int DT, bool BT, int NKS, int PK, bool WIDE>
__device__ __forceinline__ void igemm_v4_body(const GemmParams &p, int block) {
  constexpr bool BF16 = DT == 1, I8 = DT == 2, F32 = DT == 3;
  constexpr bool XK = PK >= 8;
  constexpr int PP = XK ? PK / 8 : PK;
  constexpr int T = PP * (XK ? 2 : 1);
  static_assert(PK == 1 || (!I8 && !F32 && (XK ? NKS == 2 : NKS == 1)), "offset packing: 16-bit operands");
  static_assert(PP == 1 || PP == 2 || PP == 4, "offsets per piece");
  constexpr int ES = I8 ? 1 : (F32 ? 4 : 2);
  static_assert(!(I8 && BT), "int8 is forward only");
  constexpr int NB = COUT / 16;
  const int ldo = WIDE ? p.COUT : COUT;
  const int n0 = WIDE ? p.n0 : 0;
  constexpr int TM = 64 * MB;
  constexpr int BROWS = !BT ? (COUT + 31) / 32 : (F32 ? (COUT + 31) / 32 : 2 * ((COUT + 63) / 64));
  constexpr int BA = BROWS < 2 ? 2 : BROWS;
  constexpr int B_BYTES = COUT * kRowBytes;
  constexpr int CPL = NB * 4;
  extern __shared__ __attribute__((aligned(16))) char smem[];
  uint32_t *lds_mask = reinterpret_cast<uint32_t *>(smem + 2 * B_BYTES);
  float *lds_sb = reinterpret_cast<float *>(smem + 2 * B_BYTES + 64);

  SPX_STAMP(0);
  const int tid = threadIdx.x, lane = tid & 63, wave = tid >> 6;
  const int ntiles = (p.n_dst + TM - 1) / TM;
  const int napp = p.cls ? (p.app_rows >= 0 ? p.app_rows : layout_app_tiles(p.n_dst, TM)) : 0;
  const bool app = block < napp;
  int app_m = 0;
  int tile = 0;
  int pos[MB];
  if (app) {
    typedef const int32_t __attribute__((address_space(4))) *cptr_t;
    const int cls = *(cptr_t)(p.cls);
    app_m = *(cptr_t)(p.cls + 1);
    if (!cls) {
      if constexpr (!I8 && !BT && !WIDE) if (p.stats) wg_bn_stats_empty<COUT>(p.stats, block, static_cast<int>(gridDim.x));
      return;
    }
    const int groups = p.app_budget > 0 ? min(napp, p.app_budget) : napp;
    const int h = min(TM, (((app_m + groups - 1) / groups) + 15) & ~15);
    if (block * h >= app_m) {
      if constexpr (!I8 && !BT && !WIDE) if (p.stats) wg_bn_stats_empty<COUT>(p.stats, block, static_cast<int>(gridDim.x));
      return;
    }
#pragma unroll
    for (int mb = 0; mb < MB; ++mb) {
      const int blk = mb * (kThreads / 64) + (threadIdx.x >> 6);
      const int q = block * h + blk * 16 + (threadIdx.x & 15);
      pos[mb] = (blk * 16 < h && q < app_m) ? q : -1;
    }
    tile = block;
  } else {
    const int bid = block - napp;
    const int rot = (p.xcd_rot + napp) & 7;
    tile = (p.tile_order && p.lpt) ? ntiles - 1 - bid : (rot ? xcd_tile_rot(bid, ntiles, rot) : xcd_tile(bid, ntiles));
#pragma unroll
    for (int mb = 0; mb < MB; ++mb) {
      const int t = tile * TM + ((threadIdx.x >> 6) * MB + mb) * 16 + (threadIdx.x & 15);
      pos[mb] = t < p.n_dst ? t : -1;
    }
  }
  const int mcap = layout_mcap(p.n_dst);
  const int32_t *order_app = p.argsort;
  const uint32_t *maskp = app ? reinterpret_cast<const uint32_t *>(order_app + mcap) : p.mask;
  const int32_t *pairp = app ? order_app + 2 * static_cast<size_t>(mcap) : p.pair;
  const int tbl_rows = app ? mcap : p.n_dst;
  const int lrow = lane & 15, lgrp = lane >> 4;
  const int slot = tid & 7, r0 = tid >> 3;
  constexpr int GL = 4 / PP;
  const int ga = lgrp / GL;
  auto swzB = [](int row, int sl) __attribute__((always_inline)) {
    const int x = ((row >> 1) & 1) | (((row / CPL) & 3) << 1);
    return row * kRowBytes + ((sl ^ x) << 4);
  };
  const uint32_t rowB = static_cast<uint32_t>(p.CIN) * ES;
  const int nchunk = (static_cast<int>(rowB) + kRowBytes - 1) / kRowBytes;
  const bool cfull = (rowB & (kRowBytes - 1)) == 0;

  const uint32_t a_bytes = static_cast<uint32_t>(p.n_src) * rowB;
  const uint32_t w_bytes = static_cast<uint32_t>(p.COUT) * p.kv * rowB;
  const uint32_t pair_bytes = static_cast<uint32_t>(tbl_rows) * 4u;

  const int32_t *olist = (app || !p.cls) ? p.argsort : nullptr;
  const bool by_row = olist && !app && !p.tile_order;
  const __amdgpu_buffer_rsrc_t rO = make_rsrc(olist, olist ? pair_bytes : 0u);
  int glist[MB];
  uint32_t goff[MB];
#pragma unroll
  for (int mb = 0; mb < MB; ++mb) {
    goff[mb] = pos[mb] < 0 ? kOob : static_cast<uint32_t>(pos[mb]) * 4u;
    glist[mb] = static_cast<int>(__builtin_amdgcn_raw_buffer_load_b32(rO, goff[mb], 0, SPX_AUX_TABLE));
  }
  if (by_row) {
#pragma unroll
    for (int mb = 0; mb < MB; ++mb) goff[mb] = pos[mb] < 0 ? kOob : static_cast<uint32_t>(glist[mb]) * 4u;
    asm volatile("" ::: "memory");
  }
  const __amdgpu_buffer_rsrc_t rM = make_rsrc(maskp, maskp ? pair_bytes * p.mask_words : 0u);
  uint32_t mraw[MB];
#pragma unroll
  for (int mb = 0; mb < MB; ++mb)
    mraw[mb] = __builtin_amdgcn_raw_buffer_load_b32(rM, goff[mb] == kOob ? kOob : goff[mb] * p.mask_words, 0, SPX_AUX_TABLE);
  __builtin_amdgcn_sched_barrier(0);
  int grow[MB];
#pragma unroll
  for (int mb = 0; mb < MB; ++mb) grow[mb] = pos[mb] < 0 ? -1 : (olist ? glist[mb] : pos[mb]);

  const int ctail = static_cast<int>(rowB) - (nchunk - 1) * kRowBytes;
  constexpr int AK = NKS < 2 ? 2 : NKS;
  uint32_t aoff[AK], aoff_tail[AK];
#pragma unroll
  for (int ks = 0; ks < NKS; ++ks) {
    const int c = T == 1 ? ks * 64 + lgrp * 16
                         : (lgrp % GL) * 16;
    aoff[ks] = static_cast<uint32_t>(c);
    aoff_tail[ks] = c < ctail ? 0u : kOob;
  }
  uint32_t boff[BA], boff_tail[BA];
  int bgrp[BA];
  if constexpr (!BT) {
#pragma unroll
    for (int j = 0; j < BROWS; ++j) {
      const int n = r0 + 32 * j;
      const int sl = T == 1 ? slot : slot % GL;
      const uint32_t o = static_cast<uint32_t>(n0 + n) * static_cast<uint32_t>(p.strideN) * ES + sl * 16u;
      bgrp[j] = T == 1 ? 0 : slot / GL;
      boff[j] = (n < COUT && (T == 1 || XK || slot < 4)) ? o : kOob;
      boff_tail[j] = sl * 16 < ctail ? 0u : kOob;
    }
  } else {
#pragma unroll
    for (int j = 0; j < BROWS; ++j) {
      const int d = F32 ? r0 : 2 * r0 + (j & 1);
      const int n = F32 ? j * 32 + slot * 4 : (j >> 1) * 64 + slot * 8;
      const int dl = T == 1 ? d : d % (8 * GL);
      const uint32_t o = (static_cast<uint32_t>(dl) * static_cast<uint32_t>(p.strideD) + n0 + n) * ES;
      bgrp[j] = T == 1 ? 0 : (d / (8 * GL)) & 7;
      boff[j] = (n < COUT && (T == 1 || XK || d < 32)) ? o : kOob;
      boff_tail[j] = dl * ES < ctail ? 0u : kOob;
    }
  }

  int idxr[2][MB][AK];
  uint32_t identr[2] = {0u, 0u};
  u32x4 areg[2][MB][AK];
  constexpr int WD = (!I8 && !F32 && COUT <= 64) ? SPX_WD : 1;
  u32x4 breg[2][BA];

  auto lane_k = [&](const StepIt &it, int ks) __attribute__((always_inline)) {
    int km = it.k;
    if constexpr (T > 1) {
      const int g = (XK ? ks * PP : 0) + ga;
      const int kg = step_k(it, g < 1 ? 1 : g);
// ... 101 lines not shown
                                     : __builtin_amdgcn_perm(od, ev, 0x05040100u);
          if (COUT >= 64 * (jj + 1) || n < COUT)
            *reinterpret_cast<uint32_t *>(ldsB + swzB(n, r0 >> 2) + (r0 & 3) * 4) = v;
        }
      }
    }
  };

  using Set0 = std::integral_constant<int, 0>;
  using Set1 = std::integral_constant<int, 1>;
  const bool spec = p.identity_k >= 0;
  StepIt it0;
  it0.k = p.identity_k;
  it0.chunk = 0;
  it0.rest = 0;
  it0.kx = ~0ull;
  __builtin_amdgcn_sched_barrier(0);
  load_b(it0, Set0{});
  identr[0] = 0xffffffffu;
#pragma unroll
  for (int mb = 0; mb < MB; ++mb) idxr[0][mb][0] = idxr[0][mb][1] = 0;
  load_a(it0, Set0{});
  __builtin_amdgcn_sched_barrier(0);
  SPX_STAMP(1);
  uint32_t wm = 0;
#pragma unroll
  for (int mb = 0; mb < MB; ++mb) wm |= mraw[mb];
  if (!maskp) wm = 0xffffffffu;
  wm |= __shfl_xor(wm, 1, 64);
  wm |= __shfl_xor(wm, 2, 64);
  wm |= __shfl_xor(wm, 4, 64);
  wm |= __shfl_xor(wm, 8, 64);
  const uint32_t wavemask =
      __builtin_amdgcn_readfirstlane(wm) | (spec ? (1u << p.identity_k) : 0u);
  if (lane == 0) lds_mask[wave] = wm;
  if (spec) store_b(smem, Set0{});
  if constexpr (I8) {
    const float *bias_f = static_cast<const float *>(p.bias);
    for (int c = tid; c < 2 * COUT; c += kThreads)
      lds_sb[c] = c < COUT ? (p.scale ? p.scale[n0 + c] : 1.f) : (bias_f ? bias_f[n0 + c - COUT] : 0.f);
  }
  __syncthreads();
  SPX_STAMP(2);
  if (p.cls && !app) {
#pragma unroll
    for (int mb = 0; mb < MB; ++mb)
      if (mraw[mb] == 0u) grow[mb] = -1;
  }
  uint32_t tilemask = lds_mask[0] | lds_mask[1] | lds_mask[2] | lds_mask[3];
  tilemask = __builtin_amdgcn_readfirstlane(tilemask);
  if (p.kv - p.kbase < 32) tilemask &= (1u << (p.kv - p.kbase)) - 1u;
  if (spec) {
    it0.rest = tilemask & ~(1u << p.identity_k);
  } else {
    it0 = step_begin<T>(tilemask);
    load_b(it0, Set0{});
    load_idx(it0, Set0{});
    load_a(it0, Set0{});
    store_b(smem, Set0{});
    __syncthreads();
  }
  StepIt it1 = step_next<T>(it0, nchunk);
  StepIt it2 = step_next<T>(it1, nchunk);

  using acc_t = typename std::conditional<I8, i32x4, f32x4>::type;
  acc_t acc[NB][MB];
#pragma unroll
  for (int nb = 0; nb < NB; ++nb)
#pragma unroll
    for (int mb = 0; mb < MB; ++mb) acc[nb][mb] = acc_t{0, 0, 0, 0};

  auto compute = [&](const StepIt &it, auto SET) __attribute__((always_inline)) {
    constexpr int S = decltype(SET)::value;
    uint32_t stepbits = it.k >= 0 ? 1u << it.k : 0u;
    if constexpr (T > 1) {
#pragma unroll
      for (int g = 1; g < T; ++g) {
        const int kg = step_k(it, g);
        stepbits |= kg >= 0 ? 1u << kg : 0u;
      }
    }
    if (wavemask & stepbits) {
      const char *cur = smem + S * B_BYTES;
      const int ksteps = XK ? 2 : (min(kRowBytes, static_cast<int>(rowB) - it.chunk * kRowBytes) + 63) >> 6;
#pragma unroll
      for (int ks = 0; ks < NKS; ++ks) {
        if (ks < ksteps) {
#pragma unroll
          for (int nb = 0; nb < NB; ++nb) {
            const uint4 fa = *reinterpret_cast<const uint4 *>(
                cur + swzB((lrow >> 2) * CPL + nb * 4 + (lrow & 3), ks * 4 + lgrp));
#pragma unroll
            for (int mb = 0; mb < MB; ++mb) {
              if (SPX_ABL(p, 3)) acc[nb][mb][0] += static_cast<decltype(acc[nb][mb][0] + 0)>(fa.x ^ areg[S][mb][ks][0]);
              else acc[nb][mb] = mfma_step<DT>(fa, __builtin_bit_cast(uint4, areg[S][mb][ks]), acc[nb][mb]);
            }
          }
        }
      }
    }
  };

  load_idx(it1, Set1{});
  __builtin_amdgcn_sched_barrier(0);
  using WSetA = std::integral_constant<int, (WD == 2 ? 1 : 0)>;
  load_b(it1, WSetA{});
  __builtin_amdgcn_sched_barrier(0);
  load_idx(it2, Set0{});
  __builtin_amdgcn_sched_barrier(0);
  compute(it0, Set0{});
  __builtin_amdgcn_sched_barrier(0);
  load_a(it1, Set1{});
  store_b(smem + B_BYTES, WSetA{});
  {
    const StepIt it3 = step_next<T>(it2, nchunk);
    load_b(it2, Set0{});
    if constexpr (WD == 2) load_b(it3, Set1{});
    __builtin_amdgcn_sched_barrier(0);
    load_idx(it3, Set1{});
    __builtin_amdgcn_sched_barrier(0);
    load_a(it2, Set0{});
    it0 = it1;
    it1 = it2;
    it2 = it3;
  }

  auto step = [&](auto SET) __attribute__((always_inline)) {
    constexpr int S = decltype(SET)::value;
    if (!SPX_ABL(p, 2)) __syncthreads();
    using WSetN = std::integral_constant<int, (WD == 2 ? 1 - S : 0)>;
    if (!SPX_ABL(p, 1) && !SPX_ABL(p, 2)) store_b(smem + (1 - S) * B_BYTES, WSetN{});
    compute(it0, SET);
    const StepIt it3 = step_next<T>(it2, nchunk);
    if (!SPX_ABL(p, 1) && !SPX_ABL(p, 2)) {
      if constexpr (WD == 2) load_b(it3, WSetN{});
      else load_b(it2, WSetN{});
    }
    __builtin_amdgcn_sched_barrier(0);
    load_idx(it3, std::integral_constant<int, 1 - S>{});
    __builtin_amdgcn_sched_barrier(0);
    load_a(it2, SET);
    it0 = it1;
    it1 = it2;
    it2 = it3;
  };
  SPX_STAMP(3);
  while (it0.k >= 0) {
    step(Set1{});
    step(Set0{});
  }
  SPX_STAMP(4);

  if constexpr (!I8) {
    const bool plain = p.bias == nullptr && p.act == SPX_ACT_NONE;
    const __amdgpu_buffer_rsrc_t rO = make_rsrc(p.out, static_cast<uint32_t>(p.n_dst) * (ldo * ES));
    float bv[CPL];
#pragma unroll
    for (int q = 0; q < CPL; ++q) bv[q] = 0.f;
    if (p.bias) {
#pragma unroll
      for (int q = 0; q < CPL; ++q) {
        if constexpr (F32) bv[q] = static_cast<const float *>(p.bias)[n0 + lgrp * CPL + q];
        else bv[q] = to_float<BF16>(static_cast<const uint16_t *>(p.bias)[n0 + lgrp * CPL + q]);
      }
    }
    if (p.acc_mode) {
      const __amdgpu_buffer_rsrc_t rS = make_rsrc(p.acc, static_cast<uint32_t>(p.n_dst) * (ldo * 4));
#pragma unroll
      for (int mb = 0; mb < MB; ++mb) {
        const uint32_t so = grow[mb] < 0 ? kOob : static_cast<uint32_t>(grow[mb]) * (ldo * 4) + (n0 + lgrp * CPL) * 4;
        uint32_t prev[CPL];
        if (p.acc_mode & 1) load_dwords<CPL>(prev, rS, so);
#pragma unroll
        for (int nb = 0; nb < NB; ++nb)
#pragma unroll
          for (int e = 0; e < 4; ++e) {
            if (p.acc_mode & 1) acc[nb][mb][e] += __builtin_bit_cast(float, prev[nb * 4 + e]);
            prev[nb * 4 + e] = __builtin_bit_cast(uint32_t, static_cast<float>(acc[nb][mb][e]));
          }
        if (p.acc_mode & 2) store_dwords<CPL>(prev, rS, so);
      }
      if (p.acc_mode & 2) return;
    }
#pragma unroll
    for (int mb = 0; mb < MB; ++mb) {
      uint32_t d[F32 ? CPL : CPL / 2];
#pragma unroll
      for (int nb = 0; nb < NB; ++nb) {
#pragma unroll
        for (int h = 0; h < 2; ++h) {
          float v0 = acc[nb][mb][2 * h], v1 = acc[nb][mb][2 * h + 1];
          if (!plain) {
            v0 = apply_act(v0 + bv[nb * 4 + 2 * h], p.act, p.act_alpha);
            v1 = apply_act(v1 + bv[nb * 4 + 2 * h + 1], p.act, p.act_alpha);
          }
          if constexpr (F32) {
            d[nb * 4 + 2 * h] = __builtin_bit_cast(uint32_t, v0);
            d[nb * 4 + 2 * h + 1] = __builtin_bit_cast(uint32_t, v1);
          } else {
            d[nb * 2 + h] = pack2<BF16>(v0, v1);
          }
        }
      }
      const uint32_t vo = grow[mb] < 0 ? kOob
                                       : static_cast<uint32_t>(grow[mb]) * (ldo * ES) + (n0 + lgrp * CPL) * ES;
      if (p.dbg & 0x400) store_dwords<(F32 ? CPL : CPL / 2)>(d, rO, vo);
      else store_dwords<(F32 ? CPL : CPL / 2), 2>(d, rO, vo);
    }
    if constexpr (!BT && !WIDE) {
      if (p.stats) {
        const int st_live = p.n_live ? *p.n_live : 0x7fffffff;
        __syncthreads();
        wg_bn_stats<COUT, CPL, MB, kThreads / 64, (F32 ? 0 : (BF16 ? 2 : 1))>(
            acc, grow, st_live, reinterpret_cast<float *>(smem), p.stats, block, static_cast<int>(gridDim.x));
      }
    }
  } else {
    i8_epilogue<COUT, MB>(p, acc, grow, lgrp, lds_sb, ldo, n0);
  }
  SPX_STAMP(6);
#ifdef SPX_TIMELINE
  asm volatile("s_waitcnt vmcnt(0)" ::: "memory");
  SPX_STAMP(7);
#endif
}

template <int COUT, int MB, int DT = 0>
constexpr size_t v4_smem_bytes() {
  return 2 * static_cast<size_t>(COUT) * kRowBytes + 64 + (DT == 2 ? 2 * static_cast<size_t>(COUT) * 4 : 0);
}

int v4_flags(const GemmParams &p) {
  const int words = p.mask_words > 0 ? p.mask_words : 1;
  return p.b_reverse | (p.tile_order << 1) | ((words - 1) << 2) | (p.kbase << 4) | ((p.lpt ? 1 : 0) << 11) |
         ((p.cls ? 1 : 0) << 12);
}

bool v4_ok(const GemmParams &p, int es = 2, int out_es = 2) {
  const unsigned long long abytes = static_cast<unsigned long long>(p.n_src) * p.CIN * es;
  const unsigned long long pbytes = static_cast<unsigned long long>(p.n_dst) * 4ull;
  const unsigned long long wbytes = static_cast<unsigned long long>(p.COUT) * p.kv * p.CIN * es;
  const unsigned long long obytes = static_cast<unsigned long long>(p.n_dst) * p.COUT * out_es;
  return abytes < 0x7fff0000ull && pbytes < 0x7fff0000ull && wbytes < 0x7fff0000ull &&
         obytes < 0x7fff0000ull;
}

template <int COUT, int MB, int DT>
int launch_v4(const GemmParams &p, hipStream_t s);
GemmRest rest_of(const GemmParams &p);

inline int v4_pack(const GemmParams &p, int DT, int es, bool fused_bwd = false) {
  const int mode = option_int("SPX_PK", 1);
  if ((DT != 0 && DT != 1) || !p.pair || mode == 0) return 1;
  if (static_cast<unsigned long long>(p.n_dst) * 4ull * 32ull >= 0x7fff0000ull) return 1;
  const int rb = p.CIN * es;
  const bool both = mode == 3 || (mode == 1 && fused_bwd);
  if (both) return rb <= 16 ? 32 : (rb <= 32 ? 16 : (rb <= 64 ? 8 : 1));
  return rb <= 16 ? 4 : (rb <= 32 ? 2 : 1);
}

template <int COUT, int MB, int DT>
int launch_v4(const GemmParams &p, hipStream_t s) {
  const int ntiles = div_up(p.n_dst, 64 * MB);
  const int napp = p.cls ? (p.app_rows > 0 ? div_up(p.app_rows, 64 * MB) : layout_app_tiles(p.n_dst, 64 * MB)) : 0;
  GemmParams q = p;
  q.lpt = p.tile_order && ntiles > ((DT == 2 || COUT > 64) ? 512 : 1024);
  GemmRest r = rest_of(p);
  r.napp = p.cls ? napp : -1;
  constexpr int es = DT == 2 ? 1 : (DT == 3 ? 4 : 2);
  const bool half = p.CIN * es <= 64;
  const int pk = v4_pack(p, DT, es);
  count_launch(kFamV4);
#define SPX_LAUNCH_V4(BTV, NKSV, PKV)                                                                \
  do {                                                                                                 \
    count_inst<inst::v4(COUT, MB, DT, BTV, NKSV, PKV)>();                                              \
    hipLaunchKernelGGL((igemm_v4_kernel<COUT, MB, DT, BTV, NKSV, PKV>), dim3(napp + ntiles), dim3(kThreads), \
                       (v4_smem_bytes<COUT, MB, DT>()), s, p.A, p.B, p.mask, p.argsort, p.pair, p.n_dst,  \
                       p.n_src, p.CIN, p.kv, p.identity_k, v4_flags(q), r);                            \
  } while (0)
  if (p.grid_out) *p.grid_out = (p.stats && DT != 2 && p.strideD == 1 && !p.acc_mode) ? napp + ntiles : 0;
  if (DT == 2 || p.strideD == 1) {
    if constexpr (DT == 0 || DT == 1) {
      if (pk == 32) SPX_LAUNCH_V4(false, 2, 32);
      else if (pk == 16) SPX_LAUNCH_V4(false, 2, 16);
      else if (pk == 8) SPX_LAUNCH_V4(false, 2, 8);
      else if (pk == 4) SPX_LAUNCH_V4(false, 1, 4);
      else if (pk == 2) SPX_LAUNCH_V4(false, 1, 2);
      else if (half) SPX_LAUNCH_V4(false, 1, 1);
      else SPX_LAUNCH_V4(false, 2, 1);
    } else {
      if (half) SPX_LAUNCH_V4(false, 1, 1);
      else SPX_LAUNCH_V4(false, 2, 1);
    }
  } else if constexpr (DT != 2) {
    if constexpr (DT == 0 || DT == 1) {
      if (pk == 32) SPX_LAUNCH_V4(true, 2, 32);
      else if (pk == 16) SPX_LAUNCH_V4(true, 2, 16);
      else if (pk == 8) SPX_LAUNCH_V4(true, 2, 8);
      else if (pk == 4) SPX_LAUNCH_V4(true, 1, 4);
      else if (pk == 2) SPX_LAUNCH_V4(true, 1, 2);
      else if (half) SPX_LAUNCH_V4(true, 1, 1);
      else SPX_LAUNCH_V4(true, 2, 1);
    } else {
      if (half) SPX_LAUNCH_V4(true, 1, 1);
      else SPX_LAUNCH_V4(true, 2, 1);
    }
  }
#undef SPX_LAUNCH_V4
  SPX_LAUNCH_CHECK();
  return 0;
}

inline GemmRest rest_of(const GemmParams &p) {
  GemmRest r{};
  r.out = p.out;
  r.bias = p.bias;
  r.strideK = p.strideK;
  r.strideN = p.strideN;
  r.strideD = p.strideD;
  r.COUT = p.COUT;
  r.act = p.act;
  r.act_alpha = p.act_alpha;
  r.scale = p.scale;
  r.add = p.add;
  r.add_scale = p.add_scale;
  r.out_dtype = p.out_dtype;
  constexpr int dbg = 0;
  r.dbg = dbg | p.dbg;
  r.acc = p.acc;
  r.acc_mode = p.acc_mode;
  r.napp = -1;
  r.stats = p.stats;
  r.n_live = p.n_live;
  return r;
}

template <int COUT>
__device__ __forceinline__ void i8_centre_stream(const GemmParams &p, int first, int stride) {
  constexpr int NB = COUT / 16, CPL = NB * 4, B_BYTES = COUT * kRowBytes, TM = 64;
  extern __shared__ __attribute__((aligned(16))) char smem[];
  float *lds_sb = reinterpret_cast<float *>(smem + 2 * B_BYTES + 64);
  const int tid = threadIdx.x, lane = tid & 63, wave = tid >> 6;
  const int lrow = lane & 15, lgrp = lane >> 4;
  const int slot = tid & 7, r0 = tid >> 3;
  auto swzB = [](int row, int sl) __attribute__((always_inline)) {
    const int x = ((row >> 1) & 1) | (((row / CPL) & 3) << 1);
    return row * kRowBytes + ((sl ^ x) << 4);
  };
  const uint32_t rowB = static_cast<uint32_t>(p.CIN);
  {
    const uint32_t w_bytes = static_cast<uint32_t>(p.COUT) * p.kv * rowB;
    const __amdgpu_buffer_rsrc_t rW = make_rsrc(p.B, w_bytes);
    const uint32_t so = static_cast<uint32_t>(p.identity_k) * static_cast<uint32_t>(p.strideK);
#pragma unroll
    for (int j = 0; j < (COUT + 31) / 32; ++j) {
      const int n = r0 + 32 * j;
      if (n < COUT) {
        const uint32_t o = static_cast<uint32_t>(n) * static_cast<uint32_t>(p.strideN) + slot * 16u;
        const u32x4 v = __builtin_amdgcn_raw_buffer_load_b128(rW, slot * 16u < rowB ? o : kOob, so, 0);
        *reinterpret_cast<u32x4 *>(smem + swzB(n, slot)) = v;
      }
    }
    const float *bias_f = static_cast<const float *>(p.bias);
    for (int c = tid; c < 2 * COUT; c += kThreads)
      lds_sb[c] = c < COUT ? (p.scale ? p.scale[c] : 1.f) : (bias_f ? bias_f[c - COUT] : 0.f);
  }
  __syncthreads();
  const int ntiles = (p.n_dst + TM - 1) / TM;
  const __amdgpu_buffer_rsrc_t rA = make_rsrc(p.A, static_cast<uint32_t>(p.n_src) * rowB);
  const __amdgpu_buffer_rsrc_t rM = make_rsrc(p.mask, static_cast<uint32_t>(p.n_dst) * 4u);
  const int nks = rowB > 64u ? 2 : 1;
  uint32_t aoff[2];
#pragma unroll
  for (int ks = 0; ks < 2; ++ks) {
    const uint32_t c = static_cast<uint32_t>(ks * 64 + lgrp * 16);
    aoff[ks] = c < rowB ? c : kOob;
  }
  auto load_tile = [&](int t, u32x4 (&a)[2], uint32_t &m, int &row) __attribute__((always_inline)) {
    row = t * TM + wave * 16 + lrow;
    const bool ok = t < ntiles && row < p.n_dst;
    m = __builtin_amdgcn_raw_buffer_load_b32(rM, ok ? static_cast<uint32_t>(row) * 4u : kOob, 0, SPX_AUX_TABLE);
    const uint32_t base = ok ? static_cast<uint32_t>(row) * rowB : kOob;
#pragma unroll
    for (int ks = 0; ks < 2; ++ks)
      a[ks] = __builtin_amdgcn_raw_buffer_load_b128(rA, min(base + aoff[ks], kOob) | (aoff[ks] & kOob), 0, 0);
  };
  u32x4 a_cur[2], a_nxt[2];
  uint32_t m_cur, m_nxt;
  int row_cur, row_nxt;
  int t = first;
  load_tile(t, a_cur, m_cur, row_cur);
  while (t < ntiles) {
    const int tn = t + stride;
    load_tile(tn, a_nxt, m_nxt, row_nxt);
    i32x4 acc[NB][1];
#pragma unroll
    for (int nb = 0; nb < NB; ++nb) acc[nb][0] = i32x4{0, 0, 0, 0};
#pragma unroll
    for (int ks = 0; ks < 2; ++ks) {
      if (ks < nks) {
#pragma unroll
        for (int nb = 0; nb < NB; ++nb) {
          const uint4 fa = *reinterpret_cast<const uint4 *>(
              smem + swzB((lrow >> 2) * CPL + nb * 4 + (lrow & 3), ks * 4 + lgrp));
          acc[nb][0] = mfma_step<2>(fa, __builtin_bit_cast(uint4, a_cur[ks]), acc[nb][0]);
        }
      }
    }
    const int grow[1] = {(row_cur < p.n_dst && m_cur != 0u) ? row_cur : -1};
    i8_epilogue<COUT, 1>(p, acc, grow, lgrp, lds_sb);
#pragma unroll
    for (int ks = 0; ks < 2; ++ks) a_cur[ks] = a_nxt[ks];
    m_cur = m_nxt;
    row_cur = row_nxt;
    t = tn;
  }
}

template <int COUT>
__global__ void __launch_bounds__(kThreads, 4)
igemm_i8_sparse_kernel(const void *argA, const void *argB, const uint32_t *arg_mask,
                       const int32_t *arg_argsort, const int32_t *arg_pair, int n_dst, int n_src, int CIN,
                       int kv, int identity_k, int b_reverse, GemmRest rest) {
  GemmParams p;
  unpack_gemm_args(p, argA, argB, arg_mask, arg_argsort, arg_pair, n_dst, n_src, CIN, kv, identity_k, b_reverse, rest);
  const int napp = p.app_rows;
  const int block = static_cast<int>(blockIdx.x), nmain = static_cast<int>(gridDim.x) - napp;
  if (block < napp) {
    igemm_v4_body<COUT, 1, 2, false, 2>(p, block);
    return;
  }
  typedef const int32_t __attribute__((address_space(4))) *cptr_t;
  if (*(cptr_t)(p.cls) == 1) {
// ... 69 lines not shown
```

spconv_amd/pytorch/_gemm.py:

```python
from __future__ import annotations

import contextlib
import ctypes
import functools
import os
import threading
from typing import Optional

import numpy as np
import torch

from spconv_amd import _lib
from spconv_amd.pytorch._rulebook import (_MFMA_COUT, _ROWS_LAYOUT, Activation, _dtype_code, _int_repr, _on_device, _ptr,
                                          _require_gpu, _stream, _with_dense_hint, _ws)

_OUT_CACHED = 0x100
_TILE_ORDER = 0x200
_ROWS_LAYOUT_ACT = 0x400
_SPARSE_HINT = 0x800
_out_policy = threading.local()


@contextlib.contextmanager
def output_stays_cached():
    prev = getattr(_out_policy, "cached", False)
    _out_policy.cached = True
    try:
        yield
    finally:
        _out_policy.cached = prev


_stats_req = threading.local()


class StatsSink:
    __slots__ = ("n_live", "records", "count", "rows", "channels")

    def __init__(self):
        self.n_live, self.records, self.count, self.rows, self.channels = None, None, 0, 0, 0


@contextlib.contextmanager
def collect_bn_stats():
    sink = StatsSink()
    prev = getattr(_stats_req, "sink", None)
    _stats_req.sink = sink
    try:
        yield sink
    finally:
        _stats_req.sink = prev


def current_stats_sink() -> Optional[StatsSink]:
    return getattr(_stats_req, "sink", None)


def _check_feat(features: torch.Tensor, filters: torch.Tensor):
    _require_gpu(features, "features")
    if features.dtype != filters.dtype:
        raise TypeError(f"features ({features.dtype}) and filters ({filters.dtype}) must share a dtype")
    if features.dtype in (torch.int8, torch.qint8):
        raise NotImplementedError("int8 tensors go through implicit_gemm / igemm_fwd_int8 "
                                  "(inference only, like the reference)")


_OUT_CODES = {torch.int8: _lib.DTYPE_I8, torch.float16: _lib.DTYPE_F16,
              torch.bfloat16: _lib.DTYPE_BF16, torch.float32: _lib.DTYPE_F32}


@_on_device
def igemm_fwd_int8(features: torch.Tensor, filters: torch.Tensor, pair: torch.Tensor,
                   mask: Optional[torch.Tensor], argsort: Optional[torch.Tensor], n_out: int,
                   identity_k: int = -1, scale: Optional[torch.Tensor] = None,
                   bias: Optional[torch.Tensor] = None, add: Optional[torch.Tensor] = None,
                   add_scale: float = 0.0, out_dtype: torch.dtype = torch.int8,
                   act_type: int = Activation.None_, act_alpha: float = 0.0,
                   tile_order: int = 0, sparse_hint: bool = False, hint_rows: int = 0) -> torch.Tensor:
    _require_gpu(features, "features")
    L = _lib.load()
    features = _int_repr(features).contiguous()
    filters = _int_repr(filters).contiguous()
    if features.dtype != torch.int8 or filters.dtype != torch.int8:
        raise TypeError("igemm_fwd_int8 needs int8 features and filters")
    K0, C0 = filters.shape[0], filters.shape[-1]
    kv = filters.numel() // (K0 * C0)
    assert features.shape[1] == C0, "channel size mismatch"
    C, K = _padded_ck(torch.int8, "fwd", C0, K0, kv)
    features, filters = _pad_last(features, C), _pad_first(_pad_last(filters, C), K)
    out = torch.empty((n_out, K), dtype=out_dtype, device=features.device)
    f32 = lambda t: None if t is None else t.to(device=features.device, dtype=torch.float32).contiguous()
    scale, bias = f32(scale), f32(bias)
    if K != K0:
        scale = None if scale is None else torch.nn.functional.pad(scale.reshape(-1), (0, K - K0), value=1.0)
        bias = None if bias is None else torch.nn.functional.pad(bias.reshape(-1), (0, K - K0))
    if add is not None:
        add = _int_repr(add).contiguous()
        assert add.dtype == torch.int8 and tuple(add.shape) == (n_out, K0)
        add = _pad_last(add, K)
    if sparse_hint and int(tile_order) == _ROWS_LAYOUT:
        known = getattr(argsort, "_spx_heavy", None)
        if known is None:
            sparse_hint, hint_rows = False, 0
        else:
            hint_rows = max(int(hint_rows), int(known))
    _lib.check(L.spx_igemm_fwd_int8(features.data_ptr(), filters.data_ptr(), out.data_ptr(), _ptr(pair),
                                    _ptr(mask), _ptr(argsort), features.shape[0], n_out, C, K, kv,
                                    identity_k, _ptr(scale), _ptr(bias), _ptr(add), float(add_scale),
                                    _OUT_CODES[out_dtype],
                                    int(act_type) | (0 if argsort is None else
                                                     {0: 0, 1: _TILE_ORDER, 2: _ROWS_LAYOUT_ACT}[int(tile_order)])
                                    | ((_SPARSE_HINT | (min(65535, -(-int(hint_rows) // 64)) << 16)) if sparse_hint else 0),
                                    float(act_alpha), _stream(features)))
    return out if K == K0 else out[:, :K0].contiguous()


def _lane_mult(dtype: torch.dtype) -> int:
    return 4 if dtype == torch.float32 else 16 if dtype == torch.int8 else 8


_WIDE_TILE = 128


def _round_cout(c: int) -> int:
    for v in _MFMA_COUT:
        if c <= v:
            return v
    return -(-c // _WIDE_TILE) * _WIDE_TILE


def _pad_last(t: torch.Tensor, to: int) -> torch.Tensor:
    if t.shape[-1] == to:
        return t
    if (t.is_cuda and t.is_contiguous() and t.element_size() in (2, 4) and t.numel() > 0
            and not (torch.is_grad_enabled() and t.requires_grad)
            and not t.is_quantized):
        out = torch.empty(t.shape[:-1] + (to,), dtype=t.dtype, device=t.device)
        es = t.element_size()
        with torch.cuda.device(t.device):
            _lib.check(_lib.load().spx_pad_rows(t.data_ptr(), out.data_ptr(), t.numel() // t.shape[-1],
                                                t.shape[-1] * es, to * es, _stream(t)))
        return out
    return torch.nn.functional.pad(t, (0, to - t.shape[-1]))


def _pad_first(t: torch.Tensor, to: int) -> torch.Tensor:
    if t.shape[0] == to:
        return t
    pad = [0, 0] * (t.ndim - 1) + [0, to - t.shape[0]]
    return torch.nn.functional.pad(t, pad)


@functools.lru_cache(maxsize=None)
def _padded_ck(dtype: torch.dtype, role: str, C0: int, K0: int, kv: int):
    if dtype == torch.float64:
        return C0, K0
    lane = _lane_mult(dtype)
    if role == "wgrad":
        return -(-C0 // lane) * lane, -(-K0 // lane) * lane
    red, out = (C0, K0) if role == "fwd" else (K0, C0)
    width = _round_cout(out) if (kv <= 128 or dtype == torch.int8) else out
    red = -(-red // lane) * lane
    return (red, width) if role == "fwd" else (width, red)


@_on_device
def igemm_fwd(features: torch.Tensor, filters: torch.Tensor, pair: torch.Tensor,
              mask: Optional[torch.Tensor], argsort: Optional[torch.Tensor], n_out: int,
              identity_k: int = -1, bias: Optional[torch.Tensor] = None,
              act_type: int = Activation.None_, act_alpha: float = 0.0,
              tile_order: int = 0) -> torch.Tensor:
    _check_feat(features, filters)
    L = _lib.load()
    K0, C0 = filters.shape[0], filters.shape[-1]
    assert features.shape[1] == C0, "channel size mismatch"
    kv = filters.numel() // (K0 * C0)
    C, K = _padded_ck(features.dtype, "fwd", C0, K0, kv)
    if C != C0 or K != K0:
        features, filters = _pad_last(features, C), _pad_first(_pad_last(filters, C), K)
        bias = None if bias is None else _pad_last(bias, K)
    features, filters = features.contiguous(), filters.contiguous()
    out = torch.empty((n_out, K), dtype=features.dtype, device=features.device)
    if bias is not None:
        bias = bias.to(features.dtype).contiguous()
    f64 = features.dtype == torch.float64
    head = (features.data_ptr(), filters.data_ptr(), out.data_ptr(), _ptr(pair), _ptr(mask), _ptr(argsort),
            int(tile_order) if f64 else _with_dense_hint(int(tile_order), argsort, mask), features.shape[0], n_out, C, K,
            kv, _dtype_code(features), identity_k)
    if f64:
        _lib.check(L.spx_igemm_fwd(*head, _ptr(bias), int(act_type), float(act_alpha), None, 0, _stream(features)))
        return out
    ws = _ws(L.spx_igemm_acc_bytes(n_out, K, kv), features.device) if kv > 32 else None
    act = int(act_type) | (_OUT_CACHED if getattr(_out_policy, "cached", False) else 0)
    sink = getattr(_stats_req, "sink", None)
    if (sink is not None and sink.records is None and bias is None and int(act_type) == Activation.None_
            and K == K0 and K <= _MFMA_COUT[-1] and kv <= 32 and n_out > 0):
        slots = int(L.spx_igemm_fwd_stats_slots(n_out))
        records = torch.empty((3 * K * slots,), dtype=torch.float32, device=features.device)
        used = ctypes.c_int(0)
        _lib.check(L.spx_igemm_fwd_stats(*head, None, act, float(act_alpha), None, 0, records.data_ptr(), slots,
                                         _ptr(sink.n_live), ctypes.byref(used), _stream(features)))
        if used.value > 0:
            sink.records, sink.count, sink.rows, sink.channels = records, int(used.value), n_out, K
        return out
    _lib.check(L.spx_igemm_fwd(*head, _ptr(bias), act, float(act_alpha), _ptr(ws), 0 if ws is None else ws.numel(),
                               _stream(features)))
    return out if K == K0 else out[:, :K0].contiguous()


@_on_device
def igemm_dgrad(out_bp: torch.Tensor, filters: torch.Tensor, pair: torch.Tensor,
                mask: Optional[torch.Tensor], argsort: Optional[torch.Tensor], n_in: int,
                subm: bool, tile_order: int = 0) -> torch.Tensor:
    _check_feat(out_bp, filters)
    L = _lib.load()
    K0, C0 = filters.shape[0], filters.shape[-1]
    kv = filters.numel() // (K0 * C0)
    C, K = _padded_ck(out_bp.dtype, "dgrad", C0, K0, kv)
    if C != C0 or K != K0:
        out_bp, filters = _pad_last(out_bp, K), _pad_first(_pad_last(filters, C), K)
    out_bp, filters = out_bp.contiguous(), filters.contiguous()
    din = torch.empty((n_in, C), dtype=out_bp.dtype, device=out_bp.device)
    code = _dtype_code(out_bp)
    ws = None if code == _lib.DTYPE_F64 else _ws(max(L.spx_igemm_dgrad_ws_bytes(C, K, kv, code),
                                                     L.spx_igemm_acc_bytes(n_in, C, kv)), out_bp.device)
    _lib.check(L.spx_igemm_dgrad(out_bp.data_ptr(), filters.data_ptr(), din.data_ptr(), _ptr(pair),
                                 _ptr(mask), _ptr(argsort), _with_dense_hint(int(tile_order), argsort, mask), out_bp.shape[0],
                                 n_in, C, K, kv, code,
                                 int(subm), _ptr(ws), 0 if ws is None else ws.numel(), _stream(out_bp)))
    return din if C == C0 else din[:, :C0].contiguous()


@_on_device
def wgrad_plan(num_per_loc: torch.Tensor, n_in: int, kv: int, subm: bool) -> torch.Tensor:
    L = _lib.load()
    plan = torch.empty((L.spx_wgrad_plan_bytes(n_in, kv) // 4,), dtype=torch.int32,
                       device=num_per_loc.device)
    _lib.check(L.spx_wgrad_plan(num_per_loc.data_ptr(), n_in, kv, int(subm), plan.data_ptr(),
                                _stream(num_per_loc)))
    return plan


_WGRAD_MAX_KV = 128


def _wgrad_in_groups(features, out_bp, filters_shape, native, num_per_loc, subm: bool, kv: int):
    K0, C0 = filters_shape[0], filters_shape[-1]
    n_in = native.shape[2]
    counts = num_per_loc.to(torch.int32).clone()
    if subm:
        centre = kv // 2
        counts[centre] = n_in
        counts[centre + 1:] = num_per_loc[:kv - centre - 1].flip(0)
    dw = torch.empty((K0, kv, C0), dtype=features.dtype, device=features.device)
    for kbase in range(0, kv, _WGRAD_MAX_KV):
        g = min(_WGRAD_MAX_KV, kv - kbase)
        part = igemm_wgrad(features, out_bp, (K0, g, C0), native[:, kbase:kbase + g].contiguous(),
                           counts[kbase:kbase + g].contiguous(), False, None)
        dw[:, kbase:kbase + g] = part
    return dw.view(tuple(filters_shape))


@_on_device
def igemm_wgrad(features: torch.Tensor, out_bp: torch.Tensor, filters_shape, native: torch.Tensor,
                num_per_loc: torch.Tensor, subm: bool,
                plan: Optional[torch.Tensor] = None) -> torch.Tensor:
    _require_gpu(features, "features")
    L = _lib.load()
    K0, C0 = filters_shape[0], filters_shape[-1]
    kv = int(np.prod(filters_shape)) // (K0 * C0)
    if kv > _WGRAD_MAX_KV:
        return _wgrad_in_groups(features, out_bp, filters_shape, native, num_per_loc, subm, kv)
    C, K = _padded_ck(features.dtype, "wgrad", C0, K0, kv)
    f64 = features.dtype == torch.float64
    features = _pad_last(features, C).contiguous()
    out_bp = _pad_last(out_bp, K).contiguous()
    n_in = native.shape[2]
    shape = (K,) + tuple(filters_shape[1:-1]) + (C,)
    dw = torch.empty(shape, dtype=features.dtype, device=features.device)
    ws = _ws(L.spx_igemm_wgrad_ws_bytes_dtype(n_in, C, K, kv, _lib.DTYPE_F64) if f64
             else L.spx_igemm_wgrad_ws_bytes(n_in, C, K, kv), features.device)
    _lib.check(L.spx_igemm_wgrad(features.data_ptr(), out_bp.data_ptr(), dw.data_ptr(),
                                 native.data_ptr(), num_per_loc.data_ptr(), _ptr(plan), n_in,
                                 out_bp.shape[0], C, K, kv, _dtype_code(features), int(subm),
                                 ws.data_ptr(), ws.numel(), _stream(features)))
    return dw if (C == C0 and K == K0) else dw[:K0, ..., :C0].contiguous()


_WGRAD_DEFER = os.environ.get("SPCONV_AMD_WGRAD_DEFER", "1") != "0"
_STAGE2_JOB_BYTES = 64
_defer_depth = [0]
_defer_passes = {}
_defer_lock = threading.Lock()


class deferred_wgrad:

    def __enter__(self):
        _defer_depth[0] += 1
        return self

    def __exit__(self, *exc):
        _defer_depth[0] -= 1
        if _defer_depth[0] == 0 and _defer_passes:
            with _defer_lock:
                _defer_passes.clear()
        return False


def _flush_deferred(task_id: int) -> None:
    with _defer_lock:
        st = _defer_passes.pop(task_id, None)
    if not st or not st["jobs"]:
        return
    L = _lib.load()
    by_dev = {}
    for job, param, _keep in st["jobs"]:
        g = param.grad
        if g is not None:
            if not (g.is_contiguous() and g.shape == param.shape and g.dtype == param.dtype):
                raise RuntimeError("deferred weight gradient: .grad of a weight has another layout than the weight")
            L.spx_stage2_job_retarget(job, g.data_ptr())
        by_dev.setdefault(param.device, []).append(job)
    for dev, jobs in by_dev.items():
        blob = b"".join(j.raw for j in jobs)
        with torch.cuda.device(dev):
            _lib.check(L.spx_wgrad_stage2_batch(blob, len(jobs), torch._C._cuda_getCurrentRawStream(dev.index)))


def _defer_state(filters: torch.Tensor):
    if not (_WGRAD_DEFER and _defer_depth[0] > 0 and filters.is_cuda):
        return None
    if not (filters.is_leaf and filters.requires_grad and filters.grad is None and filters.is_contiguous()):
        return None
    if filters._backward_hooks or getattr(filters, "_post_accumulate_grad_hooks", None):
        return None
    task = torch._C._current_graph_task_id()
    if task < 0:
        return None
    with _defer_lock:
        st = _defer_passes.get(task)
        if st is None:
            try:
                torch.autograd.Variable._execution_engine.queue_callback(lambda t=task: _flush_deferred(t))
            except RuntimeError:
                return None
            st = _defer_passes[task] = {"jobs": [], "seen": set()}
        key = filters.data_ptr()
        again = key in st["seen"]
        st["seen"].add(key)
    if again:
        _flush_deferred(task)
        return None
    return st


@_on_device
def bias_act_inplace(out: torch.Tensor, bias: Optional[torch.Tensor], act_type: int,
                     act_alpha: float = 0.0) -> torch.Tensor:
    L = _lib.load()
    if bias is not None:
        bias = bias.to(out.dtype).contiguous()
    _lib.check(L.spx_bias_act_inplace(out.data_ptr(), _ptr(bias), out.shape[0], out.shape[1],
                                      _dtype_code(out), int(act_type), float(act_alpha),
                                      _stream(out)))
    return out
```

spconv_amd/pytorch/_rulebook.py:

```python
from __future__ import annotations

import collections
import ctypes
import functools
import math
import os
import weakref
from typing import NamedTuple, Optional

import torch

from spconv_amd import _lib
from spconv_amd.pytorch.core import Rulebook

_DTYPES = {torch.float32: _lib.DTYPE_F32, torch.float16: _lib.DTYPE_F16,
           torch.bfloat16: _lib.DTYPE_BF16, torch.float64: _lib.DTYPE_F64}


class Activation:
    None_ = _lib.ACT_NONE
    ReLU = _lib.ACT_RELU
    Sigmoid = _lib.ACT_SIGMOID
    LeakyReLU = _lib.ACT_LEAKY_RELU

# ... 111 lines not shown

def _build_conv(L, indices, batch_size, spatial_shape, out_shape, ksize, stride, padding, dilation, transpose,
                need_native, num_out_act_bound, static_num_out, in_key_order: bool, stream) -> Rulebook:
    dev = indices.device
    n_in, ndim = indices.shape[0], indices.shape[1] - 1
    kv = _kv(ksize)
    i32 = dict(dtype=torch.int32, device=dev)
    static = static_num_out > 0
    head = (indices.data_ptr(), n_in, ndim, batch_size, _lib.ints(spatial_shape), _lib.ints(out_shape), _lib.ints(ksize),
            _lib.ints(stride), _lib.ints(padding), _lib.ints(dilation))
    n_out_dev = None
    if in_key_order:
        count, fill, fill_static = (L.spx_conv_rulebook_count_sorted, L.spx_conv_rulebook_fill_sorted,
                                    L.spx_conv_rulebook_static_sorted)
        cells = torch.empty((L.spx_rankmap_bytes(ndim, batch_size, _lib.ints(out_shape)) // 4,), **i32)
        ws = _ws(L.spx_conv_rulebook_sorted_ws_bytes(n_in, ndim, batch_size, _lib.ints(out_shape), _lib.ints(ksize)), dev)
        tail = (cells.data_ptr(), cells.numel() * 4, ws.data_ptr(), ws.numel())
        if static:
            n_out_dev = torch.empty((4,), **i32)
    else:
        count, fill, fill_static = L.spx_conv_rulebook_count, L.spx_conv_rulebook_fill, L.spx_conv_rulebook_static
        head += (int(transpose),)
        ws = _ws(L.spx_conv_rulebook_ws_bytes(n_in, ndim, _lib.ints(ksize), _lib.ints(stride), _lib.ints(dilation),
                                              int(transpose)), dev)
        tail = (ws.data_ptr(), ws.numel())
    if static:
        n_out = int(static_num_out)
    else:
        n_out_c = ctypes.c_int(0)
        _lib.check(count(*head, *tail, ctypes.byref(n_out_c), stream))
        n_out = int(n_out_c.value)
        if n_out == 0:
            raise ValueError(_POINT_VANISH_MSG.format(spatial_shape, ksize, stride, padding, dilation))
        if 0 < num_out_act_bound < n_out:
            n_out = int(num_out_act_bound)
    words = (kv + 31) // 32
    out_indices = torch.empty((n_out, ndim + 1), **i32)
    pair_fwd = torch.empty((kv, n_out), **i32)
    pair_bwd = torch.empty((kv, n_in), **i32)
    mask_fwd = torch.empty((n_out, words), **i32)
    mask_bwd = torch.empty((n_in, words), **i32)
    if static and not in_key_order:
        n_out_dev = torch.empty((2,), **i32)
    native = torch.empty((2, kv, n_in), **i32) if need_native else None
    num = torch.empty((kv,), **i32) if need_native else None
    outs = (out_indices, pair_fwd, pair_bwd, mask_fwd, mask_bwd, native, num)
    out_ptrs = tuple(_ptr(t) for t in outs)
    if static:
        _lib.check(fill_static(*head, n_out, *out_ptrs, n_out_dev.data_ptr(), *tail, stream))
    else:
        _lib.check(fill(*head, n_out, *out_ptrs, *tail, stream))
    rb = Rulebook(*outs, n_in, n_out, kv, False)
    rb.n_out_dev = n_out_dev
    if static and in_key_order:
        rb.n_out_dev, rb.out_n_live_dev = n_out_dev[:2], n_out_dev[2:3]
    if in_key_order:
        rb.rankmap = cells
        _tag_rank_map(outs[0], cells, batch_size, out_shape, n_out)
    return rb


class RankMap(NamedTuple):
    cells: torch.Tensor
    batch_size: int
    shape: tuple
    rows: int
    version: Optional[int] = None
    ptr: Optional[int] = None


def _tag_rank_map(indices: torch.Tensor, cells: torch.Tensor, batch_size: int, shape, rows: int) -> None:
    indices._spx_rankmap = RankMap(cells, batch_size, tuple(int(v) for v in shape), rows,
                                   indices._version, indices.data_ptr())


def _rankmap_of(indices: torch.Tensor, batch_size: int, spatial_shape, n: int, kv: int):
    rm = getattr(indices, "_spx_rankmap", None)
    if rm is None or not (1 < kv <= 128) or n > (4 << 20):
        return None
    cells, bs, shape, rows = rm[:4]
    if bs != batch_size or shape != tuple(int(v) for v in spatial_shape) or rows != n or cells.device != indices.device:
        return None
    if len(rm) >= 6 and (rm[4] != indices._version or rm[5] != indices.data_ptr()):
        indices._spx_rankmap = None
        return None
    return cells


_RANKMAP_MAX_CELLS_PER_ROW = float(os.environ.get("SPCONV_AMD_RANKMAP_MAX_CELLS_PER_ROW", "4096"))
_SORTED_MAX_SCRATCH = 1 << 30


def _rankmap_fits(nbytes: int, cells: int, n: int) -> bool:
    return (0 < nbytes <= _SORTED_MAX_SCRATCH and n > 0
            and not (_RANKMAP_MAX_CELLS_PER_ROW > 0 and cells > _RANKMAP_MAX_CELLS_PER_ROW * n))


@_on_device
def attach_rank_map(indices: torch.Tensor, batch_size: int, spatial_shape, check: bool = True,
                    violation: Optional[torch.Tensor] = None) -> bool:
    _require_gpu(indices, "indices")
    assert indices.dtype == torch.int32 and indices.ndim == 2 and indices.is_contiguous()
    L = _lib.load()
    n, ndim = indices.shape[0], indices.shape[1] - 1
    nbytes = int(L.spx_rankmap_bytes(ndim, batch_size, _lib.ints(spatial_shape)))
    if not _rankmap_fits(nbytes, _cells(batch_size, spatial_shape), n):
        return False
    i32 = dict(dtype=torch.int32, device=indices.device)
    cells_t = torch.empty((nbytes // 4,), **i32)
    bad = torch.empty((1,), **i32) if check else violation
    _lib.check(L.spx_rankmap_from_sorted(indices.data_ptr(), n, ndim, batch_size, _lib.ints(spatial_shape),
                                         cells_t.data_ptr(), nbytes, _ptr(bad), _stream(indices)))
    if check and int(bad.item()) != 0:
        return False
    _tag_rank_map(indices, cells_t, batch_size, spatial_shape, n)
    return True


@_on_device
def key_argsort(indices: torch.Tensor, batch_size: int, spatial_shape, want_indices: bool = True,
                rank_map: bool = False, violation: Optional[torch.Tensor] = None, rows: Optional[torch.Tensor] = None):
    _require_gpu(indices, "indices")
    assert indices.dtype == torch.int32 and indices.ndim == 2 and indices.is_contiguous()
    cells = _cells(batch_size, spatial_shape)
    if cells > 0xffe00000:
        return None
    L = _lib.load()
    n, ndim = indices.shape[0], indices.shape[1] - 1
    order = torch.empty((n,), dtype=torch.int32, device=indices.device)
    out = torch.empty_like(indices) if (want_indices or rank_map) else None
    cells_t = None
    if rank_map:
        nbytes = int(L.spx_rankmap_bytes(ndim, batch_size, _lib.ints(spatial_shape)))
        if _rankmap_fits(nbytes, cells, n):
            cells_t = torch.empty((nbytes // 4,), dtype=torch.int32, device=indices.device)
    ws = _ws(L.spx_key_argsort_ws_bytes(n), indices.device)
    rows_sorted, row_bytes = None, 0
    if rows is not None:
        assert rows.is_cuda and rows.is_contiguous() and rows.shape[0] == n
        row_bytes = (rows.numel() // max(n, 1)) * rows.element_size()
        assert row_bytes % 4 == 0, "rows carried by the sort: row size must be a multiple of 4 bytes"
        rows_sorted = torch.empty_like(rows)
    _lib.check(L.spx_key_argsort(indices.data_ptr(), n, ndim, int(batch_size), _lib.ints(spatial_shape),
                                 order.data_ptr(), _ptr(out), _ptr(cells_t), 0 if cells_t is None else cells_t.numel() * 4,
                                 _ptr(violation), _ptr(rows), _ptr(rows_sorted), row_bytes,
                                 ws.data_ptr(), ws.numel(), _stream(indices)))
    if cells_t is not None:
        _tag_rank_map(out, cells_t, batch_size, spatial_shape, n)
    return (order, out) if rows is None else (order, out, rows_sorted)


_ROWS_LAYOUT = 2
_DENSE_HINT = 0x100
_WS_MIN_ROWS = 98304
_CLASS_SLOTS = 1024
_class_ring = {}
_PRED_ATTR = "_spx_dense_pred"
_CLS0_ATTR = "_spx_class0_pred"
_LAYOUT_MIN_ROWS = 32768


def _pred_get(key) -> bool:
    return bool(getattr(key, _PRED_ATTR, False)) if key is not None else False


def _dense_rule(cls, heavy: int, n: int) -> bool:
    return (not cls) and n >= _WS_MIN_ROWS and 4 * heavy >= 3 * n


def _predict(key, cls, heavy: int, n: int) -> None:
    if key is None:
        return
    try:
        object.__setattr__(key, _PRED_ATTR, _dense_rule(cls, heavy, n))
        if heavy > 0:
            object.__setattr__(key, _CLS0_ATTR, (not cls) and 4 * heavy >= n)
    except (AttributeError, TypeError):
        pass


def _set_class(rb: Rulebook, cls=None, heavy: int = 0, predict: bool = True) -> None:
    rb.sparse_class, rb.heavy_rows = (None if cls is None else bool(cls)), heavy
    carrier = rb.layout if rb.layout is not None else rb.mask_fwd
    if cls is None:
        carrier._spx_dense = _pred_get(rb.pred_key)
        return
    carrier._spx_dense, carrier._spx_heavy = _dense_rule(cls, heavy, rb.n_out), heavy
    if predict:
        _predict(rb.pred_key, cls, heavy, rb.n_out)


class _ClassRequest:
    __slots__ = ("ring", "slot", "token", "event", "key", "n", "rb", "done")

    def resolve(self) -> bool:
        if self.done or self.ring[2][self.slot] is not self.token:
            self.done = True
            return True
        if not self.event.query():
            return False
        cls, heavy = (int(v) for v in self.ring[0][self.slot])
        self.done = True
        rb = self.rb()
        if rb is not None and rb.layout is not None:
            _set_class(rb, cls, heavy)
        else:
            _predict(self.key, cls, heavy, self.n)
        return True


_class_pending = collections.deque()


def _request_class(rb: Rulebook) -> None:
    blob = rb.layout
    rb._class_req = None
    if blob is None:
        return
    capturing = torch.cuda.is_current_stream_capturing()
    if not capturing:
        while _class_pending and _class_pending[0].resolve():
            _class_pending.popleft()
        if len(_class_pending) > 64:
            _class_pending.popleft()
    _set_class(rb)
    if capturing:
        return
    ring = _class_ring.get(blob.device.index)
    if ring is None:
        ring = [torch.zeros((_CLASS_SLOTS, 2), dtype=torch.int32).pin_memory(), 0, [None] * _CLASS_SLOTS]
        _class_ring[blob.device.index] = ring
    host, slot = ring[0], ring[1]
    ring[1] = (slot + 1) % _CLASS_SLOTS
    req = _ClassRequest()
    req.ring, req.slot, req.token, req.done = ring, slot, object(), False
    req.key, req.n, req.rb = rb.pred_key, rb.n_out, weakref.ref(rb)
    ring[2][slot] = req.token
    host[slot].copy_(blob[:2], non_blocking=True)
    req.event = torch.cuda.Event()
    req.event.record()
    rb._class_req = req
    _class_pending.append(req)


def poll_class(rb: Optional[Rulebook]) -> None:
    if rb is None or rb.layout is None or rb.sparse_class is not None:
        return
    req = rb._class_req
    if req is not None and not torch.cuda.is_current_stream_capturing() and req.resolve():
        rb._class_req = None


def _with_dense_hint(tile_order: int, argsort, mask=None) -> int:
    if tile_order == _ROWS_LAYOUT and getattr(argsort, "_spx_dense", False):
        return tile_order | _DENSE_HINT
    if tile_order == 0 and argsort is None and getattr(mask, "_spx_dense", False):
        return _DENSE_HINT
    return tile_order


def sparse_neighbourhoods(rb: Rulebook) -> bool:
    if rb.sparse_class is not None:
        return rb.sparse_class
    if rb.layout is not None:
        head = rb.layout[:2].tolist()
        _set_class(rb, head[0], int(head[1]), predict=False)
        rb._class_req = None
    elif rb.subm and 1 < rb.kv <= 32 and rb.n_out >= _LAYOUT_MIN_ROWS and rb.mask_fwd is not None:
        centre = 1 << (rb.kv // 2)
        rb.sparse_class = float((rb.mask_fwd.view(-1) != centre).float().mean().item()) < 0.25
    else:
        rb.sparse_class = False
    return rb.sparse_class




@_on_device
def rows_layout(rb: Rulebook) -> None:
    L = _lib.load()
    n, kv = rb.n_out, rb.kv
    dev = rb.pair_fwd.device
    blob = torch.empty((L.spx_subm_layout_bytes(n, kv) // 4,), dtype=torch.int32, device=dev)
    ws = _ws(L.spx_subm_layout_ws_bytes(n), dev)
    _lib.check(L.spx_subm_layout(rb.pair_fwd.data_ptr(), rb.mask_fwd.data_ptr(), n, kv, blob.data_ptr(),
                                 ws.data_ptr(), ws.numel(), _stream(rb.pair_fwd)))
    rb.layout = blob
    _request_class(rb)


def layout_views(rb: Rulebook):
    n, kv, blob = rb.n_out, rb.kv, rb.layout
    npad = (n + 63) // 64 * 64
    mcap = int(_lib.load().spx_subm_layout_mcap(n))
    o = 64 + npad
    return (blob[:5], blob[64:64 + n], blob[o:o + mcap], blob[o + mcap:o + 2 * mcap],
            blob[o + 2 * mcap:o + (2 + kv) * mcap].view(kv, mcap))


def sort_rulebook(rb: Rulebook) -> None:
    L = _lib.load()
    for which in (("fwd",) if rb.subm else ("fwd", "bwd")):
        pair, mask = (rb.pair_fwd, rb.mask_fwd) if which == "fwd" else (rb.pair_bwd, rb.mask_bwd)
        if pair is None or mask is None or mask.shape[1] != 1 or pair.shape[1] == 0:
            continue
        order = mask_argsort(mask, rb.kv)
        pair_t, mask_t = torch.empty_like(pair), torch.empty_like(mask)
        with torch.cuda.device(pair.device):
            _lib.check(L.spx_permute_tables(pair.data_ptr(), mask.data_ptr(), order.data_ptr(), pair.shape[0],
                                            pair.shape[1], mask.shape[1], pair_t.data_ptr(), mask_t.data_ptr(),
                                            _stream(pair)))
        if which == "fwd":
            rb.argsort_fwd = order
        else:
            rb.argsort_bwd = order
        rb.sorted_tables[which] = (pair_t, mask_t)


def tables_of(rb: Rulebook, which: str, cout: int = 64):
    pair, mask, order = ((rb.pair_fwd, rb.mask_fwd, rb.argsort_fwd) if which == "fwd"
                         else (rb.pair_bwd, rb.mask_bwd, rb.argsort_bwd))
    if rb.kv > 32:
        return pair, mask, None, 0
    st = rb.sorted_tables.get(which)
    if order is not None and st is not None:
        return st[0], st[1], order, 1
    if order is None and which == "fwd" and rb.subm and rb.layout is not None:
        poll_class(rb)
        return pair, mask, rb.layout, _ROWS_LAYOUT
    return pair, mask, order, 0


@_on_device
def mask_argsort(mask: torch.Tensor, kv: int = 0) -> torch.Tensor:
    L = _lib.load()
    n, words = mask.shape
    out = torch.empty((n,), dtype=torch.int32, device=mask.device)
    ws = _ws(L.spx_mask_argsort_ws_bytes(n), mask.device)
    if 1 <= int(kv) <= 32 and words == 1:
        _lib.check(L.spx_mask_argsort_kv(mask.data_ptr(), n, int(kv), out.data_ptr(), ws.data_ptr(), ws.numel(),
                                         _stream(mask)))
    else:
        _lib.check(L.spx_mask_argsort(mask.data_ptr(), n, words, out.data_ptr(), ws.data_ptr(),
                                      ws.numel(), _stream(mask)))
    return out


def attach_rulebook(t: torch.Tensor, rb: Rulebook) -> torch.Tensor:
    t._spx_rulebook = weakref.ref(rb)
    return t


def rulebook_of(t: torch.Tensor) -> Optional[Rulebook]:
    ref = getattr(t, "_spx_rulebook", None)
    return ref() if ref is not None else None


def _table_from_native(indice_pairs: torch.Tensor, indice_pair_num: torch.Tensor, n_dst: int,
                       subm: bool, inverse: bool):
    L = _lib.load()
    kv, n_in = indice_pairs.shape[1], indice_pairs.shape[2]
    table = torch.empty((kv, n_dst), dtype=torch.int32, device=indice_pairs.device)
    mask = torch.empty((n_dst, (kv + 31) // 32), dtype=torch.int32, device=indice_pairs.device)
    _lib.check(L.spx_native_to_table(indice_pairs.data_ptr(), indice_pair_num.data_ptr(), n_in,
                                     n_dst, kv, int(subm), int(inverse), table.data_ptr(),
                                     mask.data_ptr(), _stream(indice_pairs)))
    return table, mask


def _native_from_table(table: torch.Tensor, subm: bool):
    L = _lib.load()
    kv, n = table.shape
    native = torch.empty((2, kv, n), dtype=torch.int32, device=table.device)
    num = torch.empty((kv,), dtype=torch.int32, device=table.device)
    ws = _ws(L.spx_table_to_native_ws_bytes(n, kv), table.device)
    _lib.check(L.spx_table_to_native(table.data_ptr(), int(subm), kv, n, native.data_ptr(),
                                     num.data_ptr(), ws.data_ptr(), ws.numel(), _stream(table)))
    return native, num
```

spconv_amd/pytorch/ops.py:

```python
from __future__ import annotations

import ctypes
import os
from typing import List, Optional, Tuple

import numpy as np
import torch

from spconv_amd import _lib
from spconv_amd.constants import SPCONV_DO_SORT
from spconv_amd.pytorch.core import ConvAlgo, Rulebook
from spconv_amd.pytorch._rulebook import (
    _CLS0_ATTR, _DTYPES, _LAYOUT_MIN_ROWS, _MFMA_COUT, _ROWS_LAYOUT, _SORTED_MAX_SCRATCH, Activation, _build_conv,
    _build_subm, _cells, _dtype_code, _int_repr, _kv, _native_from_table, _on_device, _pred_get, _ptr, _rankmap_of,
    _require_gpu, _set_class, _stream, _table_from_native, _with_dense_hint, _ws, attach_rank_map, attach_rulebook,
    get_conv_output_size, get_deconv_output_size, key_argsort, layout_views, mask_argsort, poll_class, rows_layout,
    rulebook_of, sort_rulebook, sparse_neighbourhoods, tables_of)
from spconv_amd.pytorch._gemm import (
    _STAGE2_JOB_BYTES, _WGRAD_MAX_KV, StatsSink, _check_feat, _defer_lock, _defer_passes, _defer_state, _lane_mult,
    bias_act_inplace, collect_bn_stats, current_stats_sink, deferred_wgrad, igemm_dgrad, igemm_fwd, igemm_fwd_int8,
    igemm_wgrad, output_stays_cached, wgrad_plan)
from spconv_amd.pytorch._union import sparse_union

BN_EPILOGUE = os.environ.get("SPCONV_AMD_BN_EPILOGUE", "1") != "0"
_LAYOUT_SKIP = os.environ.get("SPCONV_AMD_LAYOUT_SKIP", "1") != "0"
_SORTED_MAX_CELLS_PER_ROW = float(os.environ.get("SPCONV_AMD_SORTED_MAX_CELLS_PER_ROW", "512"))


def _sorted_pays(n_in: int, batch_size: int, out_shape) -> bool:
    cells = _cells(batch_size, out_shape)
    return _SORTED_MAX_CELLS_PER_ROW <= 0 or (cells <= _SORTED_MAX_CELLS_PER_ROW * max(n_in, 1)
                                              and cells * 1.25 <= _SORTED_MAX_SCRATCH)


@_on_device
def build_rulebook(indices: torch.Tensor, batch_size: int, spatial_shape: List[int],
                   ksize: List[int], stride: List[int], padding: List[int],
                   dilation: List[int], out_padding: List[int], subm: bool = False,
                   transpose: bool = False, need_bwd_table: bool = False,
                   do_sort=False, need_native: bool = True,
                   num_out_act_bound: int = -1, static_num_out: int = 0,
                   pred_key=None, out_order: str = "first_seen") -> Tuple[Rulebook, List[int]]:
    _require_gpu(indices, "indices")
    assert indices.dtype == torch.int32 and indices.ndim == 2
    L = _lib.load()
    indices = indices.contiguous()
    n_in, ndim = indices.shape[0], indices.shape[1] - 1
    kv = _kv(ksize)
    words = (kv + 31) // 32
    if subm:
        out_shape = list(spatial_shape)
    elif transpose:
        out_shape = get_deconv_output_size(spatial_shape, ksize, stride, padding, dilation, out_padding)
    else:
        out_shape = get_conv_output_size(spatial_shape, ksize, stride, padding, dilation)
    if any(x <= 0 for x in out_shape):
        raise ValueError(f"your out spatial shape {out_shape} reach zero!!! input shape: {spatial_shape}")
    stream = _stream(indices)
    in_key_order = False
    if subm:
        rb = _build_subm(L, indices, batch_size, spatial_shape, ksize, dilation, need_native, need_bwd_table, stream)
    else:
        if out_order not in ("first_seen", "sorted"):
            raise ValueError(f"out_order must be 'first_seen' or 'sorted', got {out_order!r}")
        in_key_order = bool(out_order == "sorted" and n_in > 0
                            and L.spx_conv_sorted_ok(ndim, batch_size, _lib.ints(spatial_shape), _lib.ints(out_shape),
                                                     _lib.ints(ksize), _lib.ints(stride), _lib.ints(padding),
                                                     _lib.ints(dilation), int(transpose))
                            and _sorted_pays(n_in, batch_size, out_shape))
        rb = _build_conv(L, indices, batch_size, spatial_shape, out_shape, ksize, stride, padding, dilation, transpose,
                         need_native, num_out_act_bound, static_num_out, in_key_order, stream)
    rb.set_geometry(indices, spatial_shape, out_shape, batch_size, pred_key)
    if not subm and static_num_out > 0 and not in_key_order:
        do_sort = False
    elif in_key_order:
        do_sort = do_sort is True
    if do_sort in ("layout", "auto"):
        if subm and 1 < kv <= 32 and n_in >= _LAYOUT_MIN_ROWS:
            if (_LAYOUT_SKIP and torch.cuda.is_current_stream_capturing()
                    and bool(getattr(pred_key, _CLS0_ATTR, False))):
                _set_class(rb)
            else:
                rows_layout(rb)
    elif do_sort and words == 1:
        sort_rulebook(rb)
    return rb, out_shape


def get_indice_pairs(indices: torch.Tensor, batch_size: int, spatial_shape: List[int],
                     algo: ConvAlgo, ksize: List[int], stride: List[int], padding: List[int],
                     dilation: List[int], out_padding: List[int], subm: bool = False,
                     transpose: bool = False, num_out_act_bound: int = -1):
    rb, _ = build_rulebook(indices, batch_size, spatial_shape, ksize, stride, padding, dilation,
                           out_padding, subm, transpose, num_out_act_bound=num_out_act_bound)
    return rb.out_indices, attach_rulebook(rb.pair_native, rb), rb.num_per_loc


def get_indice_pairs_implicit_gemm(indices: torch.Tensor, batch_size: int,
                                   spatial_shape: List[int], algo: ConvAlgo, ksize: List[int],
                                   stride: List[int], padding: List[int], dilation: List[int],
                                   out_padding: List[int], subm: bool = False,
                                   transpose: bool = False, is_train: bool = True, alloc=None,
                                   timer=None, num_out_act_bound: int = -1,
                                   direct_table: bool = True, do_sort: bool = SPCONV_DO_SORT):
    if algo not in (ConvAlgo.MaskImplicitGemm, ConvAlgo.MaskSplitImplicitGemm):
        raise ValueError(f"get_indice_pairs_implicit_gemm builds the masked implicit-GEMM tables; algo {algo} "
                         f"(ConvAlgo.Native) goes through get_indice_pairs")
    kv = _kv(ksize)
    rb, _ = build_rulebook(indices, batch_size, spatial_shape, ksize, stride, padding, dilation,
                           out_padding, subm, transpose, need_bwd_table=subm and is_train,
                           do_sort=do_sort if kv <= 32 else False, num_out_act_bound=num_out_act_bound)
    masks = [np.array([0xffffffff], dtype=np.uint32)]
    arg_fwd = rb.argsort_fwd if rb.argsort_fwd is not None else torch.arange(
        rb.n_out, dtype=torch.int32, device=indices.device)
    pair_fwd = attach_rulebook(rb.pair_fwd, rb)
    if subm:
        pair_bwd = rb.pair_bwd if (is_train and rb.pair_bwd is not None) else torch.Tensor()
        return (rb.out_indices, rb.num_per_loc, pair_fwd, pair_bwd, [rb.mask_fwd], [], [arg_fwd],
                [], masks)
    arg_bwd = rb.argsort_bwd if rb.argsort_bwd is not None else torch.arange(
        rb.n_in, dtype=torch.int32, device=indices.device)
    return (rb.out_indices, rb.num_per_loc, pair_fwd, rb.pair_bwd, [rb.mask_fwd], [rb.mask_bwd],
            [arg_fwd], [arg_bwd], masks)


@_on_device
def igemm_bwd(features: torch.Tensor, out_bp: torch.Tensor, filters: torch.Tensor,
              table: torch.Tensor, mask: Optional[torch.Tensor], argsort: Optional[torch.Tensor],
              native: torch.Tensor, num_per_loc: torch.Tensor, subm: bool,
              plan: Optional[torch.Tensor] = None, need_din: bool = True,
              tile_order: int = 0, dense_rows: bool = False, lists=None):
    _check_feat(out_bp, filters)
    K0, C0 = filters.shape[0], filters.shape[-1]
    m = _lane_mult(out_bp.dtype)
    kvf = filters.numel() // (K0 * C0)
    if ((_BWD_ROWS is True or (_BWD_ROWS == "auto" and dense_rows))
            and out_bp.dtype in (torch.float16, torch.bfloat16) and K0 in (16, 32) and C0 in (16, 32)
            and kvf <= 27 and table is not None and mask is not None and mask.shape[1] == 1
            and (argsort is None or tile_order == _ROWS_LAYOUT) and tile_order != 1):
        return _igemm_bwd_rows(features, out_bp, filters, table, mask, subm, need_din, K0, C0, kvf)
    if native is None:
        native, num_per_loc, plan = lists()
    if (not need_din or K0 % m or C0 not in _MFMA_COUT or kvf > 32
            or out_bp.dtype == torch.float64):
        din = igemm_dgrad(out_bp, filters, table, mask, argsort, features.shape[0], subm,
                          tile_order=tile_order) if need_din else None
        return din, igemm_wgrad(features, out_bp, filters.shape, native, num_per_loc, subm, plan)
    L = _lib.load()
    features = features.contiguous()
    out_bp = out_bp.contiguous()
    st = _defer_state(filters)
    filters_leaf = filters
    filters = filters.contiguous()
    K, C = filters.shape[0], filters.shape[-1]
    kv = filters.numel() // (K * C)
    n_in = features.shape[0]
    din = torch.empty((n_in, C), dtype=out_bp.dtype, device=out_bp.device)
    dw = torch.empty_like(filters)
    ws = _ws(L.spx_igemm_wgrad_ws_bytes(native.shape[2], C, K, kv), features.device)
    args = (features.data_ptr(), out_bp.data_ptr(), filters.data_ptr(), din.data_ptr(), dw.data_ptr(), _ptr(table),
            _ptr(mask), _ptr(argsort), int(tile_order), native.data_ptr(), num_per_loc.data_ptr(), _ptr(plan), n_in,
            out_bp.shape[0], C, K, kv, _dtype_code(out_bp), int(subm), ws.data_ptr(), ws.numel(), _stream(out_bp))
    if st is not None:
        job = ctypes.create_string_buffer(_STAGE2_JOB_BYTES)
        _lib.check(L.spx_igemm_bwd_deferred(*args, job))
        with _defer_lock:
            st["jobs"].append((job, filters_leaf, (ws, plan, native, num_per_loc)))
        return din, dw
    _lib.check(L.spx_igemm_bwd(*args))
    return din, dw


_BWD_ROWS = {"0": False, "1": True}.get(os.environ.get("SPCONV_AMD_BWD_ROWS", "auto"), "auto")
_BWD_ROWS_OCC = float(os.environ.get("SPCONV_AMD_BWD_ROWS_OCC", "0.003"))


def rows_backward_expected(dtype: torch.dtype, cin: int, cout: int, kv: int, n_rows: int, batch_size: int,
                           dims) -> bool:
    if (_BWD_ROWS is False or dtype not in (torch.float16, torch.bfloat16) or cin not in (16, 32) or cout not in (16, 32)
            or kv > 27):
        return False
    return _BWD_ROWS is True or n_rows >= _BWD_ROWS_OCC * _cells(batch_size, dims)


def _dense_rows(rb: Optional[Rulebook], n_rows: int, which: str) -> bool:
    dims = None if rb is None else (rb.out_shape if which == "fwd" else rb.in_shape)
    return bool(dims) and n_rows >= _BWD_ROWS_OCC * _cells(rb.batch_size, dims)


@_on_device
def _igemm_bwd_rows(features, out_bp, filters, table, mask, subm, need_din, K, C, kv):
    L = _lib.load()
    features, out_bp = features.contiguous(), out_bp.contiguous()
    n_in = features.shape[0]
    wt = filters.reshape(K, kv, C).permute(1, 2, 0).contiguous()
    din = torch.empty((n_in, C), dtype=out_bp.dtype, device=out_bp.device) if need_din else None
    dw = torch.empty_like(filters)
    ws = _ws(L.spx_igemm_bwd_rows_ws_bytes(n_in, C, K, kv), features.device)
    _lib.check(L.spx_igemm_bwd_rows(features.data_ptr(), out_bp.data_ptr(), wt.data_ptr(), _ptr(din), dw.data_ptr(),
                                    table.data_ptr(), mask.data_ptr(), n_in, out_bp.shape[0], C, K, kv, int(subm),
                                    _dtype_code(out_bp), ws.data_ptr(), ws.numel(), _stream(out_bp)))
    return din, dw


def _plan_of(rb: Optional[Rulebook]) -> Optional[torch.Tensor]:
    if rb is None or rb.pair_native is None or rb.kv > _WGRAD_MAX_KV:
        return None
    if rb.wgrad_plan is None:
        rb.wgrad_plan = wgrad_plan(rb.num_per_loc, rb.n_in, rb.kv, rb.subm)
    return rb.wgrad_plan


def record_voxel_count_(buf: torch.Tensor, rb: Rulebook, rows: int) -> None:
    if rb.n_out_dev is not None:
        buf.copy_(torch.maximum(buf, rb.n_out_dev[:1].to(buf.dtype).reshape(buf.shape)))
    else:
        buf.clamp_(min=int(rows))


def maximum_value_int_(ten: torch.Tensor, value: int) -> torch.Tensor:
    return ten.clamp_(min=int(value))


def fused_indice_conv(features, filters, bias, indice_pairs, indice_pair_num, num_activate_out,
                      inverse, subm):
    raise NotImplementedError


def indice_conv(features: torch.Tensor, filters: torch.Tensor, indice_pairs: torch.Tensor,
                indice_pair_num: torch.Tensor, num_activate_out: int, inverse: bool = False,
                subm: bool = False, algo: ConvAlgo = ConvAlgo.Native, timer=None,
                bias: Optional[torch.Tensor] = None, act_alpha: float = 0.0,
                act_beta: float = 0.0, act_type: int = Activation.None_) -> torch.Tensor:
    _check_feat(features, filters)
    rb: Optional[Rulebook] = rulebook_of(indice_pairs)
    kv = indice_pairs.shape[1]
    argsort, tile_order = None, 0
    if rb is not None and not inverse:
        table, mask, argsort, tile_order = tables_of(rb, "fwd", filters.shape[0])
    elif rb is not None and inverse and rb.pair_bwd is not None:
        table, mask, argsort, tile_order = tables_of(rb, "bwd", filters.shape[0])
    else:
        table, mask = _table_from_native(indice_pairs, indice_pair_num, num_activate_out, subm, inverse)
    return igemm_fwd(features, filters, table, mask, argsort, num_activate_out,
                     kv // 2 if subm else -1, bias, act_type, act_alpha, tile_order=tile_order)


def indice_conv_backward(features: torch.Tensor, filters: torch.Tensor, out_bp: torch.Tensor,
                         indice_pairs: torch.Tensor, indice_pair_num: torch.Tensor,
                         inverse: bool = False, subm: bool = False,
                         algo: ConvAlgo = ConvAlgo.Native, timer=None, need_din: bool = True):
    _check_feat(features, filters)
    rb: Optional[Rulebook] = rulebook_of(indice_pairs)
    n_in = features.shape[0]
    argsort, tile_order, which = None, 0, None
    if rb is not None:
        which = "fwd" if (subm or inverse) else "bwd"
        table, mask, argsort, tile_order = tables_of(rb, which, filters.shape[-1])
    else:
        table, mask = _table_from_native(indice_pairs, indice_pair_num, n_in, subm, (not subm) and (not inverse))
    if rb is not None and not inverse and not rb.has_native:
        return igemm_bwd(features, out_bp, filters, table, mask, argsort, None, None, subm, None, need_din,
                         tile_order=tile_order, dense_rows=_dense_rows(rb, n_in, which),
                         lists=lambda: (rb.pair_native, rb.num_per_loc, _plan_of(rb)))
    native = indice_pairs if (rb is None or indice_pairs.shape[2] > 0 or rb.n_in == 0) else rb.pair_native
    if rb is not None and indice_pair_num.numel() != rb.kv:
        indice_pair_num = rb.num_per_loc
    if inverse:
        native = rb.native_swapped() if rb is not None else torch.stack(
            [indice_pairs[1], indice_pairs[0]]).contiguous()
    plan = _plan_of(rb)
    if native.shape[2] == n_in or not need_din:
        return igemm_bwd(features, out_bp, filters, table, mask, argsort, native, indice_pair_num,
                         subm, plan, need_din, tile_order=tile_order,
                         dense_rows=_dense_rows(rb, n_in, which) if rb is not None else False)
    return (igemm_dgrad(out_bp, filters, table, mask, argsort, n_in, subm, tile_order=tile_order),
            igemm_wgrad(features, out_bp, filters.shape, native, indice_pair_num, subm, plan))


def implicit_gemm(features: torch.Tensor, filters: torch.Tensor, pair_fwd: torch.Tensor,
                  pair_mask_fwd_splits: List[torch.Tensor],
                  mask_argsort_fwd_splits: List[torch.Tensor], num_activate_out: int,
                  masks: List[np.ndarray], is_train: bool, is_subm: bool, timer=None,
                  fp32_accum: Optional[bool] = None, bias: Optional[torch.Tensor] = None,
                  act_alpha: float = 0.0, act_beta: float = 0.0,
                  act_type: int = Activation.None_, output_scale: float = 1.0,
                  scale: Optional[torch.Tensor] = None, output_add: Optional[torch.Tensor] = None,
                  output_add_scale: float = 0.0, output_dtype: Optional[torch.dtype] = None):
    mask = pair_mask_fwd_splits[0] if pair_mask_fwd_splits else None
    rb: Optional[Rulebook] = rulebook_of(pair_fwd)
    argsort, tile_order = (rb.argsort_fwd if rb is not None else None), 0
    kv = pair_fwd.shape[0]
    if rb is not None and pair_fwd is rb.pair_fwd:
        pair_fwd, mask, argsort, tile_order = tables_of(rb, "fwd", filters.shape[0])
    if features.dtype in (torch.int8, torch.qint8):
        assert not is_train, "int8 is inference only"
        out_dt = torch.int8 if output_dtype in (None, torch.int8, torch.qint8) else output_dtype
        beta = output_add_scale / output_scale if output_add is not None else 0.0
        out = igemm_fwd_int8(features, filters, pair_fwd, mask, argsort, num_activate_out,
                             kv // 2 if is_subm else -1, scale, bias, output_add, beta, out_dt,
                             act_type, act_alpha, tile_order=tile_order,
                             sparse_hint=rb is not None and rb.sparse_class is True,
                             hint_rows=rb.heavy_rows if rb is not None else 0)
        if out_dt == torch.int8 and features.is_quantized:
            out = torch._make_per_tensor_quantized_tensor(out, float(output_scale), 0)
        return out, None, -1
    if scale is not None or output_add is not None:
        raise NotImplementedError("scale / output_add belong to the int8 path")
    out = igemm_fwd(features, filters, pair_fwd, mask, argsort, num_activate_out,
                    kv // 2 if is_subm else -1, bias, act_type, act_alpha, tile_order=tile_order)
    return out, None, -1


def implicit_gemm_backward(features: torch.Tensor, filters: torch.Tensor, out_bp: torch.Tensor,
# ... 149 lines not shown
```

Measured before the change: 4.118 billion voxels/s.

## Add centre-tile fast path for sparse SubM rows layout and double-buffer wgrad loads

Adds a sparse-seen flag that Python sets when the rulebook is classified as sparse under the rows layout, and passes it to the kernels. When the flag is set, the forward and fused backward launch a centre-tile body for C=64 f16/bf16 tiles, meant to cheaply handle tiles past the app rows that have only the centre (identity) offset. The single-stage wgrad loop now double-buffers its index words and rows, uses constant-address-space plan pointers, and stores partials through buffer stores, to hide gather latency. The centre path depends on a correct sparse classification and adds more template instantiations and register pressure.

```diff
diff --git a/include/spconv_amd.h b/include/spconv_amd.h
--- a/include/spconv_amd.h
+++ b/include/spconv_amd.h
@@ -147,6 +147,7 @@
 size_t spx_subm_layout_mcap(int n);
 #define SPX_ROWS_LAYOUT 2
 #define SPX_DENSE_HINT 0x100
+#define SPX_SPARSE_SEEN 0x200
 #define SPX_ROWS_LAYOUT_ACT 0x400
 #define SPX_SPARSE_HINT 0x800
 #define SPX_LAYOUT_HEADER 64
diff --git a/spconv_amd/csrc/common.cpp b/spconv_amd/csrc/common.cpp
--- a/spconv_amd/csrc/common.cpp
+++ b/spconv_amd/csrc/common.cpp
@@ -203,7 +203,7 @@
 long long spx_launch_count(const char *family_h) {
   static const char *names[spx::kFamCount] = {"igemm_v4", "igemm_ws", "igemm_bwd", "igemm_bwd_rows", "igemm_i8_stream",
                                               "generic", "wgrad_stage2", "wgrad_stage2_batch", "igemm_f64",
-                                              "igemm_v4w"};
+                                              "igemm_v4w", "igemm_centre"};
   if (!family_h) return -1;
   for (int i = 0; i < spx::kFamCount; ++i)
     if (strcmp(names[i], family_h) == 0) return spx::g_launches[i].load(std::memory_order_relaxed);
diff --git a/spconv_amd/csrc/common.h b/spconv_amd/csrc/common.h
--- a/spconv_amd/csrc/common.h
+++ b/spconv_amd/csrc/common.h
@@ -103,7 +103,7 @@
 
 namespace spx {
 enum LaunchFamily { kFamV4 = 0, kFamWs, kFamBwdFused, kFamBwdRows, kFamI8Stream, kFamGeneric, kFamStage2, kFamStage2Batch,
-                    kFamF64, kFamV4w, kFamCount };
+                    kFamF64, kFamV4w, kFamCentre, kFamCount };
 extern std::atomic<long long> g_launches[kFamCount];
 inline void count_launch(LaunchFamily f) { g_launches[f].fetch_add(1, std::memory_order_relaxed); }
 
diff --git a/spconv_amd/csrc/igemm.hip b/spconv_amd/csrc/igemm.hip
--- a/spconv_amd/csrc/igemm.hip
+++ b/spconv_amd/csrc/igemm.hip
@@ -186,7 +186,8 @@
   SPX_CHECK(pair || kv == 1, "pair table required");
   GemmParams p = fwd_params(feat, weight, out, pair, mask, argsort, bias, n_in, n_out, C, K, kv, identity_k);
   p.dense_hint = (tile_order & SPX_DENSE_HINT) ? 1 : 0;
-  apply_rows_layout(p, tile_order & ~SPX_DENSE_HINT);
+  p.sparse_seen = (tile_order & SPX_SPARSE_SEEN) ? 1 : 0;
+  apply_rows_layout(p, tile_order & ~(SPX_DENSE_HINT | SPX_SPARSE_SEEN));
   p.act = act & 0xff;
   if (act & SPX_OUT_CACHED) p.dbg = 0x400;
   p.act_alpha = act_alpha;
@@ -269,7 +270,8 @@
   SPX_CHECK(pair || kv == 1, "pair table required");
   GemmParams p = dgrad_params(dout, weight, din, pair, mask, argsort, n_out, n_in, C, K, kv, subm);
   p.dense_hint = (tile_order & SPX_DENSE_HINT) ? 1 : 0;
-  apply_rows_layout(p, tile_order & ~SPX_DENSE_HINT);
+  p.sparse_seen = (tile_order & SPX_SPARSE_SEEN) ? 1 : 0;
+  apply_rows_layout(p, tile_order & ~(SPX_DENSE_HINT | SPX_SPARSE_SEEN));
   if (dtype == SPX_F64) return run_gather_gemm_f64(p, true, static_cast<hipStream_t>(stream));
   if (ws && ws_bytes >= spx_igemm_acc_bytes(n_in, C, kv) && kv > 32) p.acc = static_cast<float *>(ws);
   return run_gather_gemm(p, dtype, static_cast<hipStream_t>(stream));
@@ -305,7 +307,8 @@
   SPX_CHECK(ws_bytes >= spx_igemm_wgrad_ws_bytes(n_in, C, K, kv), "workspace too small");
   GemmParams p = dgrad_params(dout, weight, din, pair, mask, argsort, n_out, n_in, C, K, kv, subm);
   p.dense_hint = (tile_order & SPX_DENSE_HINT) ? 1 : 0;
-  apply_rows_layout(p, tile_order & ~SPX_DENSE_HINT);
+  p.sparse_seen = (tile_order & SPX_SPARSE_SEEN) ? 1 : 0;
+  apply_rows_layout(p, tile_order & ~(SPX_DENSE_HINT | SPX_SPARSE_SEEN));
   const int es = dtype == SPX_F32 ? 4 : 2, lanes = 16 / es;
   const bool fusable = (dtype == SPX_F16 || dtype == SPX_BF16 || dtype == SPX_F32) && C % lanes == 0 &&
                        K % lanes == 0 && mfma_ok(dtype, p.CIN, p.COUT, kv) && kv <= 32 && p.COUT <= 128 &&
diff --git a/spconv_amd/csrc/igemm_bwd.h b/spconv_amd/csrc/igemm_bwd.h
--- a/spconv_amd/csrc/igemm_bwd.h
+++ b/spconv_amd/csrc/igemm_bwd.h
@@ -54,8 +54,11 @@
   const int wb = block / ntile, tile = block - wb * ntile;
   const int w = p.xcd_order ? p.plan2[plan2_wg(wb) + 5] : wb;
   const int kk0 = (tile / p.tiles_c) * kWT, c0 = (tile % p.tiles_c) * kWT;
-  const int32_t *__restrict__ rec = p.plan2 + plan2_wg(w);
-  const int32_t *__restrict__ segs = p.plan2 + plan2_seg(p.G, p.kv);
+  typedef const int32_t __attribute__((address_space(4))) *cptr_t;
+  typedef const int32_t *__restrict__ rptr_t;
+  using plan_ptr_t = typename std::conditional<STAGES == 1, cptr_t, rptr_t>::type;
+  const plan_ptr_t rec = (plan_ptr_t)(p.plan2 + plan2_wg(w));
+  const plan_ptr_t segs = (plan_ptr_t)(p.plan2 + plan2_seg(p.G, p.kv));
   const int seg_lo = rec[0], nseg = rec[1];
   const bool live = kk0 + wk * 32 < p.K && c0 + wc * 32 < p.C;
   SPX_STAMP(0);
@@ -103,46 +106,44 @@
 #pragma unroll
       for (int b = 0; b < 2; ++b) acc[a][b] = f32x4{0.f, 0.f, 0.f, 0.f};
 
-    uint32_t wd = 0;
-    u32x4 dv[RA], fv[RA];
-    auto load_words = [&](int base) __attribute__((always_inline)) {
+    using Set0 = std::integral_constant<int, 0>;
+    using Set1 = std::integral_constant<int, 1>;
+    uint32_t wd[2] = {0u, 0u};
+    u32x4 dv[2][RA], fv[2][RA];
+    auto load_words = [&](int base, auto WSET) __attribute__((always_inline)) {
+      constexpr int W = decltype(WSET)::value;
       const int j = base + wl_row;
       if (identity) {
-        wd = static_cast<uint32_t>(j);
+        wd[W] = static_cast<uint32_t>(j);
       } else {
         const uint32_t vo = j < end ? static_cast<uint32_t>(j) * 4u + wl_list : kOob;
-        wd = __builtin_amdgcn_raw_buffer_load_b32(rW, vo, 0, SPX_AUX_TABLE);
+        wd[W] = __builtin_amdgcn_raw_buffer_load_b32(rW, vo, 0, SPX_AUX_TABLE);
       }
     };
-    auto load_rows = [&](int base) __attribute__((always_inline)) {
+    auto load_rows = [&](int base, auto SET, auto WSET) __attribute__((always_inline)) {
+      constexpr int S = decltype(SET)::value, W = decltype(WSET)::value;
+      int bp = rsub;
+      if constexpr (STAGES == 1) asm volatile("" : "+v"(bp));
 #pragma unroll
       for (int q = 0; q < RQ; ++q) {
         const uint32_t iq = static_cast<uint32_t>(
-            __builtin_amdgcn_ds_bpermute((q * W_ROWS + rsub) * 4, static_cast<int>(wd)));
+            __builtin_amdgcn_ds_bpermute((q * W_ROWS + bp) * 4, static_cast<int>(wd[W])));
         const uint32_t oq = static_cast<uint32_t>(
-            __builtin_amdgcn_ds_bpermute((32 + q * W_ROWS + rsub) * 4, static_cast<int>(wd)));
+            __builtin_amdgcn_ds_bpermute((32 + q * W_ROWS + bp) * 4, static_cast<int>(wd[W])));
         const bool ok = base + r0 + RSTEP * q < end;
-        dv[q] = __builtin_amdgcn_raw_buffer_load_b128(rD, ok ? (oq * rowD + dcol) | (dcol & kOob) : kOob, 0, 0);
-        fv[q] = __builtin_amdgcn_raw_buffer_load_b128(rF, ok ? (iq * rowF + fcol) | (fcol & kOob) : kOob, 0, 0);
+        dv[S][q] = __builtin_amdgcn_raw_buffer_load_b128(rD, ok ? (oq * rowD + dcol) | (dcol & kOob) : kOob, 0, 0);
+        fv[S][q] = __builtin_amdgcn_raw_buffer_load_b128(rF, ok ? (iq * rowF + fcol) | (fcol & kOob) : kOob, 0, 0);
       }
     };
-    load_words(begin);
-    load_rows(begin);
-    load_words(begin + kW2J);
-    if (si == 0) SPX_STAMP(1);
-    int stage = 0;
-    for (int base = begin; base < end; base += kW2J, stage ^= (STAGES - 1)) {
-      char *sD = smem + stage * (2 * TILE_B);
-      char *sF = sD + TILE_B;
-      if (STAGES == 1) __syncthreads();
+    auto write_rows = [&](char *sD, char *sF, auto SET) __attribute__((always_inline)) {
+      constexpr int S = decltype(SET)::value;
 #pragma unroll
       for (int q = 0; q < RQ; ++q) {
-        *reinterpret_cast<u32x4 *>(sD + lds_w[q]) = dv[q];
-        *reinterpret_cast<u32x4 *>(sF + lds_w[q]) = fv[q];
-      }
-      __syncthreads();
-      load_rows(base + kW2J);
-      load_words(base + 2 * kW2J);
+        *reinterpret_cast<u32x4 *>(sD + lds_w[q]) = dv[S][q];
+        *reinterpret_cast<u32x4 *>(sF + lds_w[q]) = fv[S][q];
+      }
+    };
+    auto chunk_mfma = [&](const char *sD, const char *sF) __attribute__((always_inline)) {
       if (live)
 #pragma unroll
       for (int ks = 0; ks < kW2J / 32; ++ks) {
@@ -157,20 +158,77 @@
 #pragma unroll
           for (int b = 0; b < 2; ++b) acc[a][b] = mfma16<BF16>(fa[a], fb[b], acc[a][b]);
       }
+    };
+    if constexpr (STAGES == 1) {
+      char *sD = smem, *sF = smem + TILE_B;
+      load_words(begin, Set0{});
+      load_words(begin + kW2J, Set1{});
+      load_rows(begin, Set0{}, Set0{});
+      __builtin_amdgcn_sched_barrier(0);
+      load_words(begin + 2 * kW2J, Set0{});
+      __builtin_amdgcn_sched_barrier(0);
+      load_rows(begin + kW2J, Set1{}, Set1{});
+      if (si == 0) SPX_STAMP(1);
+      auto chunk = [&](int base, auto SET) __attribute__((always_inline)) {
+        using Other = std::integral_constant<int, 1 - decltype(SET)::value>;
+        __syncthreads();
+        write_rows(sD, sF, SET);
+        __syncthreads();
+        load_words(base + 3 * kW2J, Other{});
+        __builtin_amdgcn_sched_barrier(0);
+        load_rows(base + 2 * kW2J, SET, SET);
+        chunk_mfma(sD, sF);
+      };
+      int base = begin;
+      for (; base + kW2J < end; base += 2 * kW2J) {
+        chunk(base, Set0{});
+        chunk(base + kW2J, Set1{});
+      }
+      if (base < end) chunk(base, Set0{});
+    } else {
+      load_words(begin, Set0{});
+      load_rows(begin, Set0{}, Set0{});
+      load_words(begin + kW2J, Set0{});
+      if (si == 0) SPX_STAMP(1);
+      int stage = 0;
+      for (int base = begin; base < end; base += kW2J, stage ^= (STAGES - 1)) {
+        char *sD = smem + stage * (2 * TILE_B);
+        char *sF = sD + TILE_B;
+        write_rows(sD, sF, Set0{});
+        __syncthreads();
+        load_rows(base + kW2J, Set0{}, Set0{});
+        load_words(base + 2 * kW2J, Set0{});
+        chunk_mfma(sD, sF);
+      }
     }
     if (si == nseg - 1) SPX_STAMP(4);
     float *dst = p.partial + (static_cast<size_t>(seg_lo + si) * ntile + tile) * (kWT * kWT);
-#pragma unroll
-    for (int a = 0; a < 2; ++a)
-#pragma unroll
-      for (int b = 0; b < 2; ++b)
-#pragma unroll
-        for (int e = 0; e < 4; ++e) {
-          const int kk = wk * 32 + a * 16 + lgrp * 4 + e;
-          const int c = wc * 32 + b * 16 + lrow;
-          if (SPX_AUX_OUT) __builtin_nontemporal_store(acc[a][b][e], &dst[kk * kWT + c]);
-          else dst[kk * kWT + c] = acc[a][b][e];
-        }
+    if constexpr (STAGES == 1) {
+      const __amdgpu_buffer_rsrc_t rP = make_rsrc(dst, kWT * kWT * 4);
+      const uint32_t o0 = static_cast<uint32_t>((wk * 32 + lgrp * 4) * kWT + wc * 32 + lrow) * 4u;
+#pragma unroll
+      for (int a = 0; a < 2; ++a)
+#pragma unroll
+        for (int b = 0; b < 2; ++b)
+#pragma unroll
+          for (int e = 0; e < 4; ++e) {
+            const float v = acc[a][b][e];
+            __builtin_amdgcn_raw_buffer_store_b32(__builtin_bit_cast(uint32_t, v), rP, o0,
+                                                  ((a * 16 + e) * kWT + b * 16) * 4, SPX_AUX_OUT);
+          }
+    } else {
+#pragma unroll
+      for (int a = 0; a < 2; ++a)
+#pragma unroll
+        for (int b = 0; b < 2; ++b)
+#pragma unroll
+          for (int e = 0; e < 4; ++e) {
+            const int kk = wk * 32 + a * 16 + lgrp * 4 + e;
+            const int c = wc * 32 + b * 16 + lrow;
+            if (SPX_AUX_OUT) __builtin_nontemporal_store(acc[a][b][e], &dst[kk * kWT + c]);
+            else dst[kk * kWT + c] = acc[a][b][e];
+          }
+    }
     __syncthreads();
   }
   SPX_STAMP(6);
@@ -296,7 +354,12 @@
                      identity_k, b_reverse, rest);
     p.xcd_rot = (rest.dbg & 0x100) ? 0 : (nw & 7);
     p.app_budget = kAppBudget;
-    igemm_v4_body<COUT, MB, DT, true, NKS, PK>(p, n_dgrad < 0 ? b - nw : b);
+    const int blk = n_dgrad < 0 ? b - nw : b;
+    if constexpr (COUT == 64 && (DT == 0 || DT == 1) && NKS == 2 && PK == 1) {
+      if ((b_reverse & kCentreFlag) && blk >= p.app_rows && centre_tile_body<COUT, MB, DT, true>(p, blk, p.app_rows))
+        return;
+    }
+    igemm_v4_body<COUT, MB, DT, true, NKS, PK>(p, blk);
   } else {
     if constexpr (DT == 3) wgrad_f32_body(wp, n_dgrad < 0 ? b : b - n_dgrad);
     else wgrad_tr_body<DT == 1, 1>(wp, n_dgrad < 0 ? b : b - n_dgrad);
@@ -321,12 +384,14 @@
   GemmParams pl = p;
   pl.lpt = p.tile_order && n_dgrad + n_wgrad_blocks > 1024;
   count_launch(kFamBwdFused);
+  const bool centre = centre_ok(p, DT, true);
+  if (centre) count_launch(kFamCentre);
 #define SPX_LAUNCH_BWD(NKSV, PKV)                                                                                  \
   do {                                                                                                               \
     count_inst<inst::bwd(COUT, MB, DT, NKSV, PKV)>();                                                                \
     hipLaunchKernelGGL((igemm_bwd_kernel<COUT, MB, DT, NKSV, PKV>), dim3(n_dgrad + n_wgrad_blocks), dim3(kThreads),  \
                        (bwd_smem_bytes<COUT, MB, DT>()), s, p.A, p.B, p.mask, p.argsort, p.pair, p.n_dst,           \
-                       p.n_src, p.CIN, p.kv, p.identity_k, v4_flags(pl), rr,                                        \
+                       p.n_src, p.CIN, p.kv, p.identity_k, v4_flags(pl) | (centre ? kCentreFlag : 0), rr,           \
                        wgrad_first ? ~n_wgrad_blocks : n_dgrad, q);                                                 \
   } while (0)
   const int pk = v4_pack(p, DT, DT == 3 ? 4 : 2, true);
diff --git a/spconv_amd/csrc/igemm_defs.h b/spconv_amd/csrc/igemm_defs.h
--- a/spconv_amd/csrc/igemm_defs.h
+++ b/spconv_amd/csrc/igemm_defs.h
@@ -46,6 +46,7 @@
   const uint32_t *mask_rows;
   int app_rows;
   int app_budget;
+  int sparse_seen;
   int dense_hint;
   float *stats;
   const int32_t *n_live;
diff --git a/spconv_amd/csrc/igemm_v4.h b/spconv_amd/csrc/igemm_v4.h
--- a/spconv_amd/csrc/igemm_v4.h
+++ b/spconv_amd/csrc/igemm_v4.h
@@ -163,6 +163,55 @@
 
 }
 
+template <int COUT, int DT>
+__device__ __forceinline__ void v4_bias(const GemmParams &p, float (&bv)[COUT / 4], int lgrp, int n0 = 0) {
+  constexpr bool BF16 = DT == 1, F32 = DT == 3;
+  constexpr int CPL = COUT / 4;
+#pragma unroll
+  for (int q = 0; q < CPL; ++q) bv[q] = 0.f;
+  if (p.bias) {
+#pragma unroll
+    for (int q = 0; q < CPL; ++q) {
+      if constexpr (F32) bv[q] = static_cast<const float *>(p.bias)[n0 + lgrp * CPL + q];
+      else bv[q] = to_float<BF16>(static_cast<const uint16_t *>(p.bias)[n0 + lgrp * CPL + q]);
+    }
+  }
+}
+
+template <int COUT, int MB, int DT>
+__device__ __forceinline__ void v4_store_rows(const GemmParams &p, const f32x4 (&acc)[COUT / 16][MB], const int (&grow)[MB],
+                                              const float (&bv)[COUT / 4], int lgrp, int ldo = COUT, int n0 = 0) {
+  constexpr bool BF16 = DT == 1, F32 = DT == 3;
+  constexpr int ES = F32 ? 4 : 2, NB = COUT / 16, CPL = NB * 4;
+  const bool plain = p.bias == nullptr && p.act == SPX_ACT_NONE;
+  const __amdgpu_buffer_rsrc_t rO = make_rsrc(p.out, static_cast<uint32_t>(p.n_dst) * (ldo * ES));
+#pragma unroll
+  for (int mb = 0; mb < MB; ++mb) {
+    uint32_t d[F32 ? CPL : CPL / 2];
+#pragma unroll
+    for (int nb = 0; nb < NB; ++nb) {
+#pragma unroll
+      for (int h = 0; h < 2; ++h) {
+        float v0 = acc[nb][mb][2 * h], v1 = acc[nb][mb][2 * h + 1];
+        if (!plain) {
+          v0 = apply_act(v0 + bv[nb * 4 + 2 * h], p.act, p.act_alpha);
+          v1 = apply_act(v1 + bv[nb * 4 + 2 * h + 1], p.act, p.act_alpha);
+        }
+        if constexpr (F32) {
+          d[nb * 4 + 2 * h] = __builtin_bit_cast(uint32_t, v0);
+          d[nb * 4 + 2 * h + 1] = __builtin_bit_cast(uint32_t, v1);
+        } else {
+          d[nb * 2 + h] = pack2<BF16>(v0, v1);
+        }
+      }
+    }
+    const uint32_t vo = grow[mb] < 0 ? kOob
+                                     : static_cast<uint32_t>(grow[mb]) * (ldo * ES) + (n0 + lgrp * CPL) * ES;
+    if (p.dbg & 0x400) store_dwords<(F32 ? CPL : CPL / 2)>(d, rO, vo);
+    else store_dwords<(F32 ? CPL : CPL / 2), 2>(d, rO, vo);
+  }
+}
+
 template <int COUT, int MB, int DT, bool BT, int NKS, int PK, bool WIDE>
 __device__ __forceinline__ void igemm_v4_body(const GemmParams &p, int block) {
   constexpr bool BF16 = DT == 1, I8 = DT == 2, F32 = DT == 3;
@@ -570,18 +619,8 @@
   SPX_STAMP(4);
 
   if constexpr (!I8) {
-    const bool plain = p.bias == nullptr && p.act == SPX_ACT_NONE;
-    const __amdgpu_buffer_rsrc_t rO = make_rsrc(p.out, static_cast<uint32_t>(p.n_dst) * (ldo * ES));
     float bv[CPL];
-#pragma unroll
-    for (int q = 0; q < CPL; ++q) bv[q] = 0.f;
-    if (p.bias) {
-#pragma unroll
-      for (int q = 0; q < CPL; ++q) {
-        if constexpr (F32) bv[q] = static_cast<const float *>(p.bias)[n0 + lgrp * CPL + q];
-        else bv[q] = to_float<BF16>(static_cast<const uint16_t *>(p.bias)[n0 + lgrp * CPL + q]);
-      }
-    }
+    v4_bias<COUT, DT>(p, bv, lgrp, n0);
     if (p.acc_mode) {
       const __amdgpu_buffer_rsrc_t rS = make_rsrc(p.acc, static_cast<uint32_t>(p.n_dst) * (ldo * 4));
 #pragma unroll
@@ -600,31 +639,7 @@
       }
       if (p.acc_mode & 2) return;
     }
-#pragma unroll
-    for (int mb = 0; mb < MB; ++mb) {
-      uint32_t d[F32 ? CPL : CPL / 2];
-#pragma unroll
-      for (int nb = 0; nb < NB; ++nb) {
-#pragma unroll
-        for (int h = 0; h < 2; ++h) {
-          float v0 = acc[nb][mb][2 * h], v1 = acc[nb][mb][2 * h + 1];
-          if (!plain) {
-            v0 = apply_act(v0 + bv[nb * 4 + 2 * h], p.act, p.act_alpha);
-            v1 = apply_act(v1 + bv[nb * 4 + 2 * h + 1], p.act, p.act_alpha);
-          }
-          if constexpr (F32) {
-            d[nb * 4 + 2 * h] = __builtin_bit_cast(uint32_t, v0);
-            d[nb * 4 + 2 * h + 1] = __builtin_bit_cast(uint32_t, v1);
-          } else {
-            d[nb * 2 + h] = pack2<BF16>(v0, v1);
-          }
-        }
-      }
-      const uint32_t vo = grow[mb] < 0 ? kOob
-                                       : static_cast<uint32_t>(grow[mb]) * (ldo * ES) + (n0 + lgrp * CPL) * ES;
-      if (p.dbg & 0x400) store_dwords<(F32 ? CPL : CPL / 2)>(d, rO, vo);
-      else store_dwords<(F32 ? CPL : CPL / 2), 2>(d, rO, vo);
-    }
+    v4_store_rows<COUT, MB, DT>(p, acc, grow, bv, lgrp, ldo, n0);
     if constexpr (!BT && !WIDE) {
       if (p.stats) {
         const int st_live = p.n_live ? *p.n_live : 0x7fffffff;
@@ -641,6 +656,126 @@
   asm volatile("s_waitcnt vmcnt(0)" ::: "memory");
   SPX_STAMP(7);
 #endif
+}
+
+template <int COUT, int MB, int DT, bool BT>
+__device__ __forceinline__ bool centre_tile_body(const GemmParams &p, int block, int napp) {
+  static_assert(DT == 0 || DT == 1, "16-bit operands");
+  constexpr int ES = 2, NB = COUT / 16, CPL = NB * 4, TM = 64 * MB;
+  constexpr int BROWS = !BT ? (COUT + 31) / 32 : 2 * ((COUT + 63) / 64);
+  static_assert(BROWS == 2, "one weight vector pair per thread");
+  extern __shared__ __attribute__((aligned(16))) char smem[];
+  SPX_STAMP(0);
+  typedef const int32_t __attribute__((address_space(4))) *cptr_t;
+  const int cls = *(cptr_t)(p.cls);
+  const int tid = threadIdx.x, lane = tid & 63, wave = tid >> 6;
+  const int lrow = lane & 15, lgrp = lane >> 4;
+  const int slot = tid & 7, r0 = tid >> 3;
+  const int ntiles = (p.n_dst + TM - 1) / TM;
+  const int bid = block - napp;
+  const int rot = (p.xcd_rot + napp) & 7;
+  const int tile = rot ? xcd_tile_rot(bid, ntiles, rot) : xcd_tile(bid, ntiles);
+  const uint32_t rowB = static_cast<uint32_t>(p.CIN) * ES;
+  const __amdgpu_buffer_rsrc_t rM = make_rsrc(p.mask, static_cast<uint32_t>(p.n_dst) * 4u);
+  const __amdgpu_buffer_rsrc_t rA = make_rsrc(p.A, static_cast<uint32_t>(p.n_src) * rowB);
+  int pos[MB];
+  uint32_t mraw[MB];
+  u32x4 areg[MB][2];
+#pragma unroll
+  for (int mb = 0; mb < MB; ++mb) {
+    const int t = tile * TM + (wave * MB + mb) * 16 + lrow;
+    pos[mb] = t < p.n_dst ? t : -1;
+    mraw[mb] = __builtin_amdgcn_raw_buffer_load_b32(rM, pos[mb] < 0 ? kOob : static_cast<uint32_t>(t) * 4u, 0,
+                                                    SPX_AUX_TABLE);
+  }
+#pragma unroll
+  for (int mb = 0; mb < MB; ++mb) {
+#pragma unroll
+    for (int ks = 0; ks < 2; ++ks) {
+      const uint32_t c = static_cast<uint32_t>(ks * 64 + lgrp * 16);
+      const uint32_t vo = (pos[mb] < 0 || c >= rowB) ? kOob : static_cast<uint32_t>(pos[mb]) * rowB + c;
+      areg[mb][ks] = __builtin_amdgcn_raw_buffer_load_b128(rA, vo, 0, 0);
+    }
+  }
+  u32x4 breg[BROWS];
+  {
+    const __amdgpu_buffer_rsrc_t rW = make_rsrc(p.B, static_cast<uint32_t>(p.COUT) * p.kv * rowB);
+    const int kb = p.b_reverse ? p.kv - 1 - p.identity_k : p.identity_k;
+    const uint32_t so = static_cast<uint32_t>(kb) * static_cast<uint32_t>(p.strideK) * ES;
+#pragma unroll
+    for (int j = 0; j < BROWS; ++j) {
+      uint32_t vo;
+      if constexpr (!BT) {
+        const int n = r0 + 32 * j;
+        vo = slot * 16u < rowB ? static_cast<uint32_t>(n) * static_cast<uint32_t>(p.strideN) * ES + slot * 16u : kOob;
+      } else {
+        const int d = 2 * r0 + j;
+        vo = d * ES < static_cast<int>(rowB)
+                 ? (static_cast<uint32_t>(d) * static_cast<uint32_t>(p.strideD) + slot * 8u) * ES : kOob;
+      }
+      breg[j] = __builtin_amdgcn_raw_buffer_load_b128(rW, vo, so, 0);
+    }
+  }
+  SPX_STAMP(1);
+  auto swzB = [](int row, int sl) __attribute__((always_inline)) {
+    const int x = ((row >> 1) & 1) | (((row / CPL) & 3) << 1);
+    return row * kRowBytes + ((sl ^ x) << 4);
+  };
+  if constexpr (!BT) {
+#pragma unroll
+    for (int j = 0; j < BROWS; ++j) *reinterpret_cast<u32x4 *>(smem + swzB(r0 + 32 * j, slot)) = breg[j];
+  } else {
+#pragma unroll
+    for (int e = 0; e < 8; ++e) {
+      const uint32_t ev = breg[0][e >> 1], od = breg[1][e >> 1];
+      const uint32_t v = (e & 1) ? __builtin_amdgcn_perm(od, ev, 0x07060302u) : __builtin_amdgcn_perm(od, ev, 0x05040100u);
+      *reinterpret_cast<uint32_t *>(smem + swzB(slot * 8 + e, r0 >> 2) + (r0 & 3) * 4) = v;
+    }
+  }
+  __syncthreads();
+  SPX_STAMP(2);
+  if (cls != 1) return false;
+  f32x4 acc[NB][MB];
+#pragma unroll
+  for (int nb = 0; nb < NB; ++nb)
+#pragma unroll
+    for (int mb = 0; mb < MB; ++mb) acc[nb][mb] = f32x4{0.f, 0.f, 0.f, 0.f};
+#pragma unroll
+  for (int ks = 0; ks < 2; ++ks) {
+#pragma unroll
+    for (int nb = 0; nb < NB; ++nb) {
+      const uint4 fa = *reinterpret_cast<const uint4 *>(
+          smem + swzB((lrow >> 2) * CPL + nb * 4 + (lrow & 3), ks * 4 + lgrp));
+#pragma unroll
+      for (int mb = 0; mb < MB; ++mb)
+        acc[nb][mb] = mfma_step<DT>(fa, __builtin_bit_cast(uint4, areg[mb][ks]), acc[nb][mb]);
+    }
+  }
+  SPX_STAMP(4);
+  int grow[MB];
+#pragma unroll
+  for (int mb = 0; mb < MB; ++mb) grow[mb] = mraw[mb] != 0u ? pos[mb] : -1;
+  float bv[CPL];
+  v4_bias<COUT, DT>(p, bv, lgrp);
+  v4_store_rows<COUT, MB, DT>(p, acc, grow, bv, lgrp);
+  SPX_STAMP(6);
+#ifdef SPX_TIMELINE
+  asm volatile("s_waitcnt vmcnt(0)" ::: "memory");
+  SPX_STAMP(7);
+#endif
+  return true;
+}
+
+template <int COUT, int MB, int DT, bool BT>
+__global__ void __launch_bounds__(kThreads, 4)
+igemm_centre_kernel(const void *argA, const void *argB, const uint32_t *arg_mask,
+                    const int32_t *arg_argsort, const int32_t *arg_pair, int n_dst, int n_src, int CIN,
+                    int kv, int identity_k, int b_reverse, GemmRest rest) {
+  GemmParams p;
+  unpack_gemm_args(p, argA, argB, arg_mask, arg_argsort, arg_pair, n_dst, n_src, CIN, kv, identity_k, b_reverse, rest);
+  const int block = static_cast<int>(blockIdx.x), napp = p.app_rows;
+  if (block >= napp && centre_tile_body<COUT, MB, DT, BT>(p, block, napp)) return;
+  igemm_v4_body<COUT, MB, DT, BT, 2, 1>(p, block);
 }
 
 template <int COUT, int MB, int DT = 0>
@@ -675,6 +810,15 @@
   const bool both = mode == 3 || (mode == 1 && fused_bwd);
   if (both) return rb <= 16 ? 32 : (rb <= 32 ? 16 : (rb <= 64 ? 8 : 1));
   return rb <= 16 ? 4 : (rb <= 32 ? 2 : 1);
+}
+
+constexpr int kCentreFlag = 1 << 13;
+inline bool centre_ok(const GemmParams &p, int DT, bool fused_bwd = false) {
+  if (!p.cls || !p.sparse_seen || (DT != 0 && DT != 1) || p.COUT != 64) return false;
+  if (p.identity_k < 0 || p.identity_k >= p.kv || p.kv > 32 || p.kbase != 0 || p.mask_words > 1 || p.acc_mode) return false;
+  if (p.CIN * 2 <= 64 || p.CIN * 2 > kRowBytes || v4_pack(p, DT, 2, fused_bwd) != 1) return false;
+  if (p.stats) return false;
+  return option_int("SPX_CENTRE", 1) != 0;
 }
 
 template <int COUT, int MB, int DT>
@@ -697,6 +841,23 @@
                        p.n_src, p.CIN, p.kv, p.identity_k, v4_flags(q), r);                            \
   } while (0)
   if (p.grid_out) *p.grid_out = (p.stats && DT != 2 && p.strideD == 1 && !p.acc_mode) ? napp + ntiles : 0;
+  if constexpr (COUT == 64 && (DT == 0 || DT == 1)) {
+    if (centre_ok(p, DT)) {
+      count_launch(kFamCentre);
+#define SPX_LAUNCH_CENTRE(BTV)                                                                                      \
+  do {                                                                                                                \
+    count_inst<inst::v4(COUT, MB, DT, BTV, 2, 1)>();                                                                  \
+    hipLaunchKernelGGL((igemm_centre_kernel<COUT, MB, DT, BTV>), dim3(napp + ntiles), dim3(kThreads),                 \
+                       (v4_smem_bytes<COUT, MB, DT>()), s, p.A, p.B, p.mask, p.argsort, p.pair, p.n_dst, p.n_src,    \
+                       p.CIN, p.kv, p.identity_k, v4_flags(q), r);                                                   \
+  } while (0)
+      if (p.strideD == 1) SPX_LAUNCH_CENTRE(false);
+      else SPX_LAUNCH_CENTRE(true);
+#undef SPX_LAUNCH_CENTRE
+      SPX_LAUNCH_CHECK();
+      return 0;
+    }
+  }
   if (DT == 2 || p.strideD == 1) {
     if constexpr (DT == 0 || DT == 1) {
       if (pk == 32) SPX_LAUNCH_V4(false, 2, 32);
diff --git a/spconv_amd/pytorch/_gemm.py b/spconv_amd/pytorch/_gemm.py
--- a/spconv_amd/pytorch/_gemm.py
+++ b/spconv_amd/pytorch/_gemm.py
@@ -12,7 +12,7 @@
 
 from spconv_amd import _lib
 from spconv_amd.pytorch._rulebook import (_MFMA_COUT, _ROWS_LAYOUT, Activation, _dtype_code, _int_repr, _on_device, _ptr,
-                                          _require_gpu, _stream, _with_dense_hint, _ws)
+                                          _require_gpu, _stream, _with_dense_hint, _with_sparse_seen, _ws)
 
 _OUT_CACHED = 0x100
 _TILE_ORDER = 0x200
@@ -185,7 +185,8 @@
         bias = bias.to(features.dtype).contiguous()
     f64 = features.dtype == torch.float64
     head = (features.data_ptr(), filters.data_ptr(), out.data_ptr(), _ptr(pair), _ptr(mask), _ptr(argsort),
-            int(tile_order) if f64 else _with_dense_hint(int(tile_order), argsort, mask), features.shape[0], n_out, C, K,
+            int(tile_order) if f64 else _with_sparse_seen(_with_dense_hint(int(tile_order), argsort, mask), argsort),
+            features.shape[0], n_out, C, K,
             kv, _dtype_code(features), identity_k)
     if f64:
         _lib.check(L.spx_igemm_fwd(*head, _ptr(bias), int(act_type), float(act_alpha), None, 0, _stream(features)))
@@ -225,8 +226,9 @@
     ws = None if code == _lib.DTYPE_F64 else _ws(max(L.spx_igemm_dgrad_ws_bytes(C, K, kv, code),
                                                      L.spx_igemm_acc_bytes(n_in, C, kv)), out_bp.device)
     _lib.check(L.spx_igemm_dgrad(out_bp.data_ptr(), filters.data_ptr(), din.data_ptr(), _ptr(pair),
-                                 _ptr(mask), _ptr(argsort), _with_dense_hint(int(tile_order), argsort, mask), out_bp.shape[0],
-                                 n_in, C, K, kv, code,
+                                 _ptr(mask), _ptr(argsort),
+                                 _with_sparse_seen(_with_dense_hint(int(tile_order), argsort, mask), argsort),
+                                 out_bp.shape[0], n_in, C, K, kv, code,
                                  int(subm), _ptr(ws), 0 if ws is None else ws.numel(), _stream(out_bp)))
     return din if C == C0 else din[:, :C0].contiguous()
 
diff --git a/spconv_amd/pytorch/_rulebook.py b/spconv_amd/pytorch/_rulebook.py
--- a/spconv_amd/pytorch/_rulebook.py
+++ b/spconv_amd/pytorch/_rulebook.py
@@ -287,6 +287,7 @@
 
 _ROWS_LAYOUT = 2
 _DENSE_HINT = 0x100
+_SPARSE_SEEN = 0x200
 _WS_MIN_ROWS = 98304
 _CLASS_SLOTS = 1024
 _class_ring = {}
@@ -318,9 +319,9 @@
     rb.sparse_class, rb.heavy_rows = (None if cls is None else bool(cls)), heavy
     carrier = rb.layout if rb.layout is not None else rb.mask_fwd
     if cls is None:
-        carrier._spx_dense = _pred_get(rb.pred_key)
+        carrier._spx_dense, carrier._spx_sparse = _pred_get(rb.pred_key), False
         return
-    carrier._spx_dense, carrier._spx_heavy = _dense_rule(cls, heavy, rb.n_out), heavy
+    carrier._spx_dense, carrier._spx_heavy, carrier._spx_sparse = _dense_rule(cls, heavy, rb.n_out), heavy, bool(cls)
     if predict:
         _predict(rb.pred_key, cls, heavy, rb.n_out)
 
@@ -394,6 +395,12 @@
     return tile_order
 
 
+def _with_sparse_seen(tile_order: int, argsort) -> int:
+    if (tile_order & 0xff) == _ROWS_LAYOUT and getattr(argsort, "_spx_sparse", False):
+        return tile_order | _SPARSE_SEEN
+    return tile_order
+
+
 def sparse_neighbourhoods(rb: Rulebook) -> bool:
     if rb.sparse_class is not None:
         return rb.sparse_class
diff --git a/spconv_amd/pytorch/ops.py b/spconv_amd/pytorch/ops.py
--- a/spconv_amd/pytorch/ops.py
+++ b/spconv_amd/pytorch/ops.py
@@ -13,7 +13,8 @@
 from spconv_amd.pytorch._rulebook import (
     _CLS0_ATTR, _DTYPES, _LAYOUT_MIN_ROWS, _MFMA_COUT, _ROWS_LAYOUT, _SORTED_MAX_SCRATCH, Activation, _build_conv,
     _build_subm, _cells, _dtype_code, _int_repr, _kv, _native_from_table, _on_device, _pred_get, _ptr, _rankmap_of,
-    _require_gpu, _set_class, _stream, _table_from_native, _with_dense_hint, _ws, attach_rank_map, attach_rulebook,
+    _require_gpu, _set_class, _stream, _table_from_native, _with_dense_hint, _with_sparse_seen, _ws, attach_rank_map,
+    attach_rulebook,
     get_conv_output_size, get_deconv_output_size, key_argsort, layout_views, mask_argsort, poll_class, rows_layout,
     rulebook_of, sort_rulebook, sparse_neighbourhoods, tables_of)
 from spconv_amd.pytorch._gemm import (
@@ -159,7 +160,8 @@
     dw = torch.empty_like(filters)
     ws = _ws(L.spx_igemm_wgrad_ws_bytes(native.shape[2], C, K, kv), features.device)
     args = (features.data_ptr(), out_bp.data_ptr(), filters.data_ptr(), din.data_ptr(), dw.data_ptr(), _ptr(table),
-            _ptr(mask), _ptr(argsort), int(tile_order), native.data_ptr(), num_per_loc.data_ptr(), _ptr(plan), n_in,
+            _ptr(mask), _ptr(argsort), _with_sparse_seen(int(tile_order), argsort), native.data_ptr(),
+            num_per_loc.data_ptr(), _ptr(plan), n_in,
             out_bp.shape[0], C, K, kv, _dtype_code(out_bp), int(subm), ws.data_ptr(), ws.numel(), _stream(out_bp))
     if st is not None:
         job = ctypes.create_string_buffer(_STAGE2_JOB_BYTES)
```

Measured after the change: 4.215 billion voxels/s (median of 4 runs). 2.4% higher.
